# fishmingyu/HyperGef

Measured on AMD Instinct MI355X. Metric: aggregated edges/sec (fused V->E->V aggregation), higher is better.
Workload: dtype f32; 1 GPU; cora-shape x1024 block-diagonal batch, F=32; op=H*H^T*X (aggr_proto), feat_len=32, variant=auto, resolved_variant=fused

## Files before the change

hypergef_amd/_lib.py:

```python
import ctypes
import os

_HERE = os.path.dirname(os.path.abspath(__file__))
LIB_PATH = os.environ.get("HG_AGGR_LIB") or os.path.join(_HERE, "lib", "libhgaggr.so")

HG_OK = 0
HG_ERR_INVALID = -1
HG_ERR_WORKSPACE = -4
HG_ERR_UNSUPPORTED = -5
HG_VARIANT_AUTO = 0
HG_VARIANT_PULL = 1
HG_VARIANT_PUSH_ATOMIC = 2
HG_VARIANT_FUSED = 3
HG_PLAN_HOST_ONLY = 1
HG_PLAN_NO_XCD_REMAP = 2
HG_PLAN_DFS_ORDER = 4
HG_PLAN_NO_HUB_PASS = 8
HG_PLAN_NO_ROW_STREAM = 16

VARIANTS = {"auto": HG_VARIANT_AUTO, "pull": HG_VARIANT_PULL, "push_atomic": HG_VARIANT_PUSH_ATOMIC,
            "fused": HG_VARIANT_FUSED}

SYMBOLS = (
    "hg_version", "hg_last_error", "hg_status_string", "hg_balance_schedule", "hg_mtx_read", "hg_free",
    "hg_plan_create_host", "hg_plan_create_device", "hg_plan_destroy", "hg_plan_get_info",
    "hg_plan_get_vertex_csr", "hg_plan_get_vertex_csr_device", "hg_plan_get_schedule", "hg_plan_prepare", "hg_plan_auto_variant", "hg_plan_bind_scales", "hg_plan_tune_f32",
    "hg_plan_workspace_bytes",
    "hg_aggr_fused_f32", "hg_aggr_fused_bf16", "hg_linear_pack_f32", "hg_linear_pack_ex_f32", "hg_linear_pack_floats", "hg_linear_rows_f32", "hg_linear_wgrad_workspace_bytes", "hg_linear_wgrad_f32", "hg_aggr_linear_workspace_bytes", "hg_aggr_linear_f32", "hg_aggr_linear_res_f32", "hg_aggr_linear_res_dev_f32",
    "hg_gather_rows_f32", "hg_aggr_push_groups_f32", "hg_gather_max_f32",
    "hg_scatter_record_f32",
    "hg_aggr_incidence_workspace_bytes", "hg_aggr_incidence_f32", "hg_incidence_dot_f32", "hg_plan_get_incidence_perm",
)


class HgError(RuntimeError):
    def __init__(self, status, message):
        super().__init__("libhgaggr: %s (status %d)" % (message, status))
        self.status = status


class PlanOpts(ctypes.Structure):
    _fields_ = [("short_max", ctypes.c_int32), ("split_len", ctypes.c_int32),
                ("panel_rows", ctypes.c_int32), ("panel_nnz", ctypes.c_int32),
                ("flags", ctypes.c_int32), ("t_big", ctypes.c_int32),
                ("fused_tile_bytes", ctypes.c_int32), ("fused_steps", ctypes.c_int32)]


class TuneInfo(ctypes.Structure):
    _fields_ = [("variant", ctypes.c_int32), ("pull_hop_kernels", ctypes.c_int32), ("us", ctypes.c_float * 10),
                ("reserved", ctypes.c_int32)]


class FusedInfo(ctypes.Structure):
    _fields_ = [("cap", ctypes.c_int32), ("t_big", ctypes.c_int32), ("vdeg_max", ctypes.c_int32),
                ("panels", ctypes.c_int32), ("n_mat", ctypes.c_int32), ("n_hub", ctypes.c_int32),
                ("slots", ctypes.c_int64), ("member_entries", ctypes.c_int64),
                ("n_split", ctypes.c_int32), ("fixups", ctypes.c_int32),
                ("hub_rounds", ctypes.c_int32), ("hub_workgroups", ctypes.c_int32),
                ("hub_entries", ctypes.c_int64), ("hub_pairs", ctypes.c_int64),
                ("partial_rows", ctypes.c_int64),
                ("record_words_max", ctypes.c_int32), ("stream_steps_max", ctypes.c_int32),
                ("lds_bytes", ctypes.c_int32), ("reserved", ctypes.c_int32)]

    def as_dict(self):
        return {name: getattr(self, name) for name, _ in self._fields_}


class PlanInfo(ctypes.Structure):
    _fields_ = [("N", ctypes.c_int32), ("M", ctypes.c_int32), ("nnz", ctypes.c_int64),
                ("short_max", ctypes.c_int32), ("split_len", ctypes.c_int32),
                ("panel_rows", ctypes.c_int32), ("panel_nnz", ctypes.c_int32),
                ("flags", ctypes.c_int32),
                ("panels", ctypes.c_int32 * 2), ("tasks", ctypes.c_int32 * 2),
                ("partials", ctypes.c_int32 * 2), ("fixups", ctypes.c_int32 * 2),
                ("max_len", ctypes.c_int32 * 2), ("device_bytes", ctypes.c_int64)]

    def as_dict(self):
        out = {}
        for name, _ in self._fields_:
            v = getattr(self, name)
            out[name] = list(v) if hasattr(v, "__len__") else v
        return out


_lib = None


def lib():
    global _lib
    if _lib is not None:
        return _lib
    if not os.path.exists(LIB_PATH):
        raise ImportError(
            "%s not found: build it with `python -c 'import __graft_entry__ as g; g.build()'` "
            "(or `make -C hypergef_amd/csrc`). There is no CPU fallback." % LIB_PATH)
    L = ctypes.CDLL(LIB_PATH)
    vp, i32, i64, sz = ctypes.c_void_p, ctypes.c_int32, ctypes.c_int64, ctypes.c_size_t
    L.hg_version.restype = ctypes.c_int
    L.hg_last_error.restype = ctypes.c_char_p
    L.hg_status_string.restype = ctypes.c_char_p
    L.hg_status_string.argtypes = [ctypes.c_int]
    L.hg_balance_schedule.restype = ctypes.c_int
    L.hg_balance_schedule.argtypes = [i32, i32, vp, ctypes.POINTER(i64), ctypes.POINTER(i64),
                                      vp, vp, vp, vp]
    L.hg_mtx_read.restype = ctypes.c_int
    L.hg_mtx_read.argtypes = [ctypes.c_char_p, ctypes.POINTER(i32), ctypes.POINTER(i32), ctypes.POINTER(i64),
                              ctypes.POINTER(ctypes.POINTER(i32)), ctypes.POINTER(ctypes.POINTER(i32)),
                              ctypes.POINTER(ctypes.POINTER(i32)), ctypes.POINTER(ctypes.POINTER(i32))]
    L.hg_free.restype = None
    L.hg_free.argtypes = [vp]
    L.hg_plan_create_host.restype = ctypes.c_int
    L.hg_plan_create_host.argtypes = [ctypes.POINTER(vp), i32, i32, vp, vp, ctypes.POINTER(PlanOpts)]
    L.hg_plan_create_device.restype = ctypes.c_int
    L.hg_plan_create_device.argtypes = [ctypes.POINTER(vp), i32, i32, i64, vp, vp,
                                        ctypes.POINTER(PlanOpts), vp]
    L.hg_plan_destroy.restype = None
    L.hg_plan_destroy.argtypes = [vp]
    L.hg_plan_get_info.restype = ctypes.c_int
    L.hg_plan_get_info.argtypes = [vp, ctypes.POINTER(PlanInfo)]
    L.hg_plan_get_vertex_csr.restype = ctypes.c_int
    L.hg_plan_get_vertex_csr.argtypes = [vp, vp, vp]
    L.hg_plan_get_vertex_csr_device.restype = ctypes.c_int
    L.hg_plan_get_vertex_csr_device.argtypes = [vp, ctypes.POINTER(vp), ctypes.POINTER(vp)]
    L.hg_plan_get_schedule.restype = ctypes.c_int
    L.hg_plan_get_schedule.argtypes = [vp, i32, vp, vp, vp]
    L.hg_plan_prepare.restype = ctypes.c_int
    L.hg_plan_prepare.argtypes = [vp, i32, ctypes.POINTER(FusedInfo)]
    L.hg_plan_tune_f32.restype = ctypes.c_int
    L.hg_plan_tune_f32.argtypes = [vp, i32, vp, vp, vp, vp, vp, vp, vp, vp, sz, i32, vp, ctypes.POINTER(TuneInfo)]
    L.hg_linear_pack_f32.restype = ctypes.c_int
    L.hg_linear_pack_f32.argtypes = [i32, i32, vp, vp, vp]
    L.hg_linear_pack_ex_f32.restype = ctypes.c_int
    L.hg_linear_pack_ex_f32.argtypes = [i32, i32, vp, vp, i32, vp]
    L.hg_linear_pack_floats.restype = sz
    L.hg_linear_pack_floats.argtypes = [i32, i32, i32]
    L.hg_linear_wgrad_workspace_bytes.restype = sz
    L.hg_linear_wgrad_workspace_bytes.argtypes = [i64, i32, i32]
    L.hg_linear_wgrad_f32.restype = ctypes.c_int
    L.hg_linear_wgrad_f32.argtypes = [i64, i32, i32, vp, vp, vp, vp, sz, vp]
    L.hg_linear_rows_f32.restype = ctypes.c_int
    L.hg_linear_rows_f32.argtypes = [i64, i32, i32, vp, vp, vp, vp]
    L.hg_aggr_linear_workspace_bytes.restype = sz
    L.hg_aggr_linear_workspace_bytes.argtypes = [vp, i32]
    L.hg_aggr_linear_f32.restype = ctypes.c_int
    L.hg_aggr_linear_f32.argtypes = [vp, i32, i32, vp, vp, vp, vp, vp, vp, vp, vp, vp, sz, i32, vp]
    L.hg_aggr_linear_res_f32.restype = ctypes.c_int
    L.hg_aggr_linear_res_f32.argtypes = [vp, i32, i32, vp, vp, vp, vp, vp, vp, vp, vp, ctypes.c_float, ctypes.c_float,
                                         i32, vp, vp, vp, sz, i32, vp]
    L.hg_aggr_linear_res_dev_f32.restype = ctypes.c_int
    L.hg_aggr_linear_res_dev_f32.argtypes = [vp, i32, i32, vp, vp, vp, vp, vp, vp, vp, vp, ctypes.c_float, vp,
                                             i32, vp, vp, vp, sz, i32, vp]
    L.hg_plan_bind_scales.restype = ctypes.c_int
    L.hg_plan_bind_scales.argtypes = [vp, i32, vp, vp, vp, vp]
    L.hg_plan_auto_variant.restype = ctypes.c_int
    L.hg_plan_auto_variant.argtypes = [vp, i32]
    L.hg_plan_workspace_bytes.restype = sz
    L.hg_plan_workspace_bytes.argtypes = [vp, i32]
    L.hg_aggr_fused_f32.restype = ctypes.c_int
    L.hg_aggr_fused_f32.argtypes = [vp, i32, vp, vp, vp, vp, vp, vp, vp, vp, sz, i32, vp]
    L.hg_aggr_fused_bf16.restype = ctypes.c_int
    L.hg_aggr_fused_bf16.argtypes = [vp, i32, vp, vp, vp, vp, vp, vp, vp, vp, sz, i32, vp]
    L.hg_gather_rows_f32.restype = ctypes.c_int
    L.hg_gather_rows_f32.argtypes = [vp, i32, i32, vp, vp, vp, vp, vp, vp, vp, sz, vp]
    L.hg_gather_max_f32.restype = ctypes.c_int
    L.hg_gather_max_f32.argtypes = [i32, i32, vp, vp, vp, vp, vp, vp, vp, vp]
    L.hg_scatter_record_f32.restype = ctypes.c_int
    L.hg_scatter_record_f32.argtypes = [i32, i32, i32, vp, vp, vp, vp, vp]
    if hasattr(L, "hg_aggr_incidence_f32"):
        L.hg_aggr_incidence_workspace_bytes.restype = sz
        L.hg_aggr_incidence_workspace_bytes.argtypes = [vp, i32]
        L.hg_aggr_incidence_f32.restype = ctypes.c_int
        L.hg_aggr_incidence_f32.argtypes = [vp, i32, vp, vp, vp, vp, vp, vp, vp, vp, vp, vp, vp, sz, vp]
        L.hg_incidence_dot_f32.restype = ctypes.c_int
        L.hg_incidence_dot_f32.argtypes = [vp, i32, vp, vp, vp, vp, vp, vp]
        L.hg_plan_get_incidence_perm.restype = ctypes.c_int
        L.hg_plan_get_incidence_perm.argtypes = [vp, vp]
    L.hg_aggr_push_groups_f32.restype = ctypes.c_int
    L.hg_aggr_push_groups_f32.argtypes = [i32, i32, i32, i64, vp, vp, vp, vp, vp, vp,
                                          vp, vp, vp, vp, vp, vp]
    _lib = L
    return L


def check(status):
    if status != HG_OK:
        msg = lib().hg_last_error()
        raise HgError(status, (msg or b"").decode() or lib().hg_status_string(status).decode())
```

hypergef_amd/csrc/hg_api.hip:

```cpp
#include <hip/hip_runtime.h>

#include <cstdio>
#include <cstring>
#include <algorithm>
#include <new>
#include <string>

#include "hg_kernels.h"

namespace {

int hip_fail(const char *what, hipError_t e) {
  hg::set_error(std::string(what) + ": " + hipGetErrorString(e));
  return HG_ERR_HIP;
}

#define HG_HIP(call)                                  \
  do {                                                \
    hipError_t e_ = (call);                           \
    if (e_ != hipSuccess) return hip_fail(#call, e_); \
  } while (0)

size_t round256(size_t x) { return (x + 255) & ~(size_t)255; }

bool aligned16(const void *p) { return (reinterpret_cast<uintptr_t>(p) & 15) == 0; }
bool aligned_lane(const void *p, bool bf16) { return (reinterpret_cast<uintptr_t>(p) & (bf16 ? 7 : 15)) == 0; }
bool rows_whole_64(const void *base, int32_t F, bool bf16 = false) {
  return ((int64_t)F * (bf16 ? 2 : 4)) % 64 == 0 && (reinterpret_cast<uintptr_t>(base) & 63) == 0;
}

int resolve_opts(const hg_plan_opts *in, hg::Opts &o) {
  if (in) {
    if (in->short_max > 0) o.short_max = in->short_max;
    if (in->split_len > 0) o.split_len = in->split_len;
    if (in->panel_rows > 0) {
      o.panel_rows = in->panel_rows;
      o.panel_rows_auto = false;
    }
    if (in->panel_nnz > 0) o.panel_nnz = in->panel_nnz;
    o.flags = in->flags;
    if (in->t_big > 0) o.t_big = in->t_big;
    if (in->fused_tile_bytes > 0) {
      o.fused_tile_bytes = in->fused_tile_bytes;
      o.fused_tile_auto = false;
    }
    if (in->fused_steps > 0) o.fused_steps = in->fused_steps;
  }
  if (o.short_max > o.panel_nnz || o.split_len < o.short_max || o.panel_rows > 4096 ||
      o.panel_nnz > 16384 || o.fused_tile_bytes > 131072) {
    hg::set_error("hg_plan_opts: need short_max <= panel_nnz <= 16384, split_len >= short_max, panel_rows <= 4096, fused_tile_bytes <= 131072");
    return HG_ERR_INVALID;
  }
  if ((size_t)(4 * o.panel_rows + 1 + o.panel_nnz) * sizeof(int32_t) > (size_t)160 * 1024) {
    hg::set_error("hg_plan_opts: panel_rows / panel_nnz need more than 160 KiB of LDS per workgroup");
    return HG_ERR_INVALID;
  }
  return HG_OK;
}

template <typename T>
int upload(const std::vector<T> &h, T **d, int64_t &bytes) {
  *d = nullptr;
  if (h.empty()) return HG_OK;
  const size_t n = h.size() * sizeof(T);
  hipError_t e = hipMalloc(reinterpret_cast<void **>(d), n);
  if (e != hipSuccess) {
    hg::set_error(std::string("hipMalloc(plan): ") + hipGetErrorString(e));
    return e == hipErrorOutOfMemory ? HG_ERR_NOMEM : HG_ERR_HIP;
  }
  HG_HIP(hipMemcpy(*d, h.data(), n, hipMemcpyHostToDevice));
  bytes += (int64_t)n;
  return HG_OK;
}

int sched_upload(hg::Sched &s, int64_t &bytes) {
  int rc;
  if ((rc = upload(s.panels, &s.d_panels, bytes)) != HG_OK) return rc;
  if ((rc = upload(s.tasks, &s.d_tasks, bytes)) != HG_OK) return rc;
  return upload(s.fixups, &s.d_fixups, bytes);
}

void sched_free(hg::Sched &s) {
  if (s.d_panels) (void)hipFree(s.d_panels);
  if (s.d_tasks) (void)hipFree(s.d_tasks);
  if (s.d_fixups) (void)hipFree(s.d_fixups);
  s.d_panels = nullptr;
  s.d_tasks = nullptr;
  s.d_fixups = nullptr;
}

int plan_upload(hg_plan *p) {
  HG_HIP(hipGetDevice(&p->device));
  int rc;
  if ((rc = upload(p->ptr_v, &p->d_ptr_v, p->device_bytes)) != HG_OK) return rc;
  if ((rc = upload(p->ind_v, &p->d_ind_v, p->device_bytes)) != HG_OK) return rc;
  for (int h = 0; h < 2; h++)
    if ((rc = sched_upload(p->sched[h], p->device_bytes)) != HG_OK) return rc;
  if (p->has_lat)
    for (int h = 0; h < 2; h++)
      if ((rc = sched_upload(p->sched_lat[h], p->device_bytes)) != HG_OK) return rc;
  return HG_OK;
}

int fused_upload(hg::FusedSched &f, int64_t &bytes) {
  int rc;
#define UP(v, d) if ((rc = upload(f.v, &f.d, bytes)) != HG_OK) return rc
  UP(prow, d_prow);
  UP(mat_ptr, d_mat_ptr);
  UP(mat_ind, d_mat_ind);
  UP(mat_eid, d_mat_eid);
  UP(rec, d_rec);
  UP(rec_tab, d_rec_tab);
  UP(eid_all, d_eid_all);
  UP(fixups, d_fixups);
  UP(hub.vslot0, hub.d_vslot0);
  UP(hub.rec, hub.d_rec);
  UP(hub.rec_tab, hub.d_rec_tab);
  UP(hub.wg_first, hub.d_wg_first);
  UP(mat_stream.rec, mat_stream.d_rec);
  UP(mat_stream.rec_tab, mat_stream.d_rec_tab);
  UP(mat_stream.fixups, mat_stream.d_fixups);
#undef UP
  return sched_upload(f.mat_sched, bytes);
}

void fused_free(hg::FusedSched &f) {
  void *ptrs[] = {f.d_prow, f.d_mat_ptr, f.d_mat_ind, f.d_mat_eid, f.d_rec, f.d_rec_tab, f.d_eid_all, f.d_bsA,
                  f.d_bsB, f.d_bsD, f.d_fixups, f.hub.d_vslot0, f.hub.d_rec, f.hub.d_rec_tab, f.hub.d_wg_first, f.mat_stream.d_rec, f.mat_stream.d_rec_tab,
                  f.mat_stream.d_fixups};
  for (void *q : ptrs)
    if (q) (void)hipFree(q);
  sched_free(f.mat_sched);
}

bool wide_rows_ok(const hg_plan *p, int32_t F) {
  return (F % 4 == 0 || F > 8) && p->N < (1 << 24) && p->M < (1 << 24) && F < (1 << 22) && (int64_t)p->N * F * 4 < ((int64_t)1 << 31) &&
         (int64_t)p->M * F * 4 < ((int64_t)1 << 31);
}
bool plan_vec4(const hg_plan *p, int32_t F) { return F % 4 == 0 || wide_rows_ok(p, F); }

void fused_caps(const hg_plan *p, int32_t F, bool vec4, int32_t &cap, int32_t &mem_cap, int32_t tile_bytes = 0) {
  const int row_bytes = hg::fused_tile_row_floats(F, vec4) * 4;
  const int c = std::max(16, std::min(256, (tile_bytes > 0 ? tile_bytes : p->opts.fused_tile_bytes) / row_bytes));
  cap = c / 16 * 16;
  mem_cap = cap * 4;
  if (p->opts.fused_steps > 0) {
    const int32_t ng = 256 / (hg::fused_tile_row_floats(F, vec4) / (vec4 ? 4 : 1));
    mem_cap = std::max(p->opts.t_big, std::min(mem_cap, p->opts.fused_steps * ng));
  }
}

double small_graph_cost(const hg::FusedSched &f) {
  int32_t max_rows = 0;
  for (const hg::FPanel &pn : f.panels) max_rows = std::max(max_rows, pn.nrows);
  const int launches = 1 + (f.n_mat > 0 ? 1 : 0) + (f.fixups.empty() ? 0 : 1);
  return 5.0 * launches + 0.08 * f.max_steps + 0.4 * ((max_rows + f.ng - 1) / std::max(1, f.ng));
}

bool lin_caps(const hg_plan *p, int32_t F, bool vec4, int32_t &cap, int32_t &mem_cap, int32_t &rows_cap) {
  if (!vec4 || F != 128 || !p->opts.fused_tile_auto || p->opts.fused_steps > 0 || p->nnz <= (1 << 18)) return false;
  const int pct = 150;
  fused_caps(p, F, vec4, cap, mem_cap);
  const int32_t ng = 256 / (hg::fused_tile_row_floats(F, vec4) / 4);
  rows_cap = std::min(cap, 4 * ng);
  cap = std::max(cap, (rows_cap * pct / 100 + 7) / 8 * 8);
  mem_cap = cap * 4;
  return true;
}

int get_fused(const hg_plan *cp, int32_t F, bool vec4, const hg::FusedSched **out, bool lin = false) {
  hg_plan *p = const_cast<hg_plan *>(cp);
  int32_t cap, mem_cap, rows_cap = 0;
  if (lin && !lin_caps(p, F, vec4, cap, mem_cap, rows_cap)) lin = false;
  if (!lin) fused_caps(p, F, vec4, cap, mem_cap);
  const int32_t row_floats = hg::fused_tile_row_floats(F, vec4);
  const int32_t ng = 256 / (row_floats / (vec4 ? 4 : 1));
  const bool allow_hub = vec4 && F % 4 == 0 && F >= 16 && p->N < (1 << 24) && p->M < (1 << 24) && (int64_t)p->N * F * 4 < ((int64_t)1 << 31) &&
                         (int64_t)p->M * F * 4 < ((int64_t)1 << 31);
  const int64_t key = ((((int64_t)cap * 1000000 + mem_cap) * 1000 + ng) * 2 + (allow_hub ? 1 : 0)) * 1024 + rows_cap;
  std::lock_guard<std::mutex> lock(p->fused_mu);
  auto it = p->fused.find(key);
  if (it == p->fused.end()) {
    hg::FusedSched f;
    try {
      hg::build_fused(p->N, p->M, p->ptr_t.data(), p->ind_t.data(), p->ptr_v.data(), p->ind_v.data(),
                      p->opts, cap, mem_cap, ng, row_floats, allow_hub, f, rows_cap);
      if (p->nnz <= (1 << 18)) {
        double best = small_graph_cost(f);
        const int32_t tiles[3] = {p->opts.fused_tile_bytes, p->opts.fused_tile_bytes / 2, p->opts.fused_tile_bytes / 4};
        for (int t = 0; t < (p->opts.fused_tile_auto ? 3 : 1); t++) {
          int32_t c2, m2;
          fused_caps(p, F, vec4, c2, m2, tiles[t]);
          if (t > 0 && c2 == cap) continue;
          for (int mode = 0; mode < 4; mode++) {
            if (t == 0 && mode == 0) continue;
            hg::Opts o = p->opts;
            if (mode == 1) {
              if (p->sched[0].max_len * 4 > m2 || p->sched[0].max_len <= o.t_big) continue;
              o.t_big = p->sched[0].max_len;
            } else if (mode >= 2) {
              o.slot_chunk = std::max(o.t_big, mode == 2 ? 8 : 16);
              if (p->sched[0].max_len <= o.slot_chunk || (mode == 3 && o.t_big >= 16)) continue;
            }
            hg::FusedSched alt;
            hg::build_fused(p->N, p->M, p->ptr_t.data(), p->ind_t.data(), p->ptr_v.data(), p->ind_v.data(), o, c2, m2,
                            ng, row_floats, allow_hub, alt);
            if (alt.invalid) continue;
            const double c = small_graph_cost(alt);
            if (c < best) {
              best = c;
              f = std::move(alt);
            }
          }
        }
        const int32_t lanes = row_floats / (vec4 ? 4 : 1);
        if (p->opts.fused_tile_auto && vec4 && F % 4 == 0 && (lanes == 8 || lanes == 16) && p->nnz <= 16384 && p->N <= 4096 &&
            wide_rows_ok(p, F)) {
          for (int32_t tile : {16384, 32768, 65536}) {
            int32_t c2, m2;
            fused_caps(p, F, vec4, c2, m2, tile);
            for (int mode = 1; mode < 4; mode++) {
              hg::Opts o = p->opts;
              if (mode == 1) {
                if (p->sched[0].max_len * 4 > m2) continue;
                o.t_big = std::max(o.t_big, p->sched[0].max_len);
              } else {
                o.slot_chunk = std::max(o.t_big, mode == 2 ? 8 : 16);
                if (p->sched[0].max_len <= o.slot_chunk) continue;
              }
              hg::FusedSched alt;
              hg::build_fused(p->N, p->M, p->ptr_t.data(), p->ind_t.data(), p->ptr_v.data(), p->ind_v.data(), o, c2, m2,
                              4 * ng, row_floats, false, alt);
              if (alt.invalid || alt.n_mat > 0 || !alt.fixups.empty()) continue;
              const double c = small_graph_cost(alt) + 0.3;
              if (c < best) {
                best = c;
                f = std::move(alt);
              }
            }
          }
        }
      }
    } catch (const std::bad_alloc &) {
      hg::set_error("fused schedule: host allocation failed");
      return HG_ERR_NOMEM;
    }
    for (const hg::FPanel &pn : f.panels) {
      if (pn.nrows <= 0 || pn.nrows > f.rows_cap || pn.nslots > f.cap || pn.npm > f.mem_cap ||
          pn.nvs > f.vslot_cap || pn.r0 < 0 || (size_t)(pn.r0 + pn.nrows) > f.prow.size()) {
        hg::set_error("fused schedule: internal error, panel exceeds its LDS budget");
        return HG_ERR_INVALID;
      }
    }
    const size_t lds_need = std::max((size_t)f.cap * (row_floats + 4) * 4 + (size_t)f.max_rec_words * 4 +
                                         (size_t)(2 * f.cap + f.rows_cap) * 4 + 16,
                                     f.hub.K > 0 ? hg::hub_pass_lds_bytes(f.hub.cap, row_floats, f.hub.max_rec_words) : 0);
    if (lds_need > (size_t)160 * 1024) {
      hg::set_error("fused schedule: fused_tile_bytes = " + std::to_string(p->opts.fused_tile_bytes) + " needs " +
                    std::to_string(lds_need) + " bytes of LDS per workgroup at this feature width (limit 163840)");
      return HG_ERR_INVALID;
    }
    int rc = (p->opts.flags & HG_PLAN_HOST_ONLY) ? HG_OK : fused_upload(f, p->device_bytes);
    if (rc != HG_OK) {
      fused_free(f);
      return rc;
    }
    it = p->fused.emplace(key, std::move(f)).first;
  }
  p->fused_by_width[((int64_t)F * 2 + (vec4 ? 1 : 0)) * 2 + (lin ? 1 : 0)] = &it->second;
  *out = &it->second;
  return HG_OK;
}

struct Carve {
  size_t xe, part[2], total;
};
Carve carve(const hg_plan *p, int32_t F) {
  Carve c;
  c.xe = 0;
  size_t off = round256((size_t)p->M * F * sizeof(float));
  for (int h = 0; h < 2; h++) {
    c.part[h] = off;
    off += round256((size_t)std::max(std::max(p->sched[h].nslots, p->sched_lat[h].nslots), p->stream_nslots[h]) * F * sizeof(float) + 16);
  }
  c.total = off;
  return c;
}
struct FusedCarve {
  size_t mat_part, part, total;
};
FusedCarve fused_carve(const hg::FusedSched &f, int32_t F) {
  FusedCarve c;
  c.mat_part = round256((size_t)f.n_mat * F * sizeof(float));
  c.part = c.mat_part + round256((size_t)std::max(f.mat_sched.nslots, f.mat_stream.nslots) * F * sizeof(float));
  c.total = c.part + round256((size_t)f.n_part * F * sizeof(float) + 16);
  return c;
}
size_t workspace_need(const hg_plan *cp, int32_t F, bool pull_only = false) {
  hg_plan *p = const_cast<hg_plan *>(cp);
  size_t need = carve(p, F).total;
  if (pull_only) return need;
  std::lock_guard<std::mutex> lock(p->fused_mu);
  for (const auto &kv : p->fused_by_width)
    if (kv.first / 4 == F) need = std::max(need, fused_carve(*kv.second, F).total);
  return need;
}

int pick_variant_uncached(const hg_plan *plan, int32_t F, bool vec4, int32_t *variant,
                          const hg::FusedSched **f);
int get_row_stream(const hg_plan *cp, int hop, int32_t ng, const hg::RowStream **out);

int pick_variant(const hg_plan *plan, int32_t F, bool vec4, int32_t *variant,
                 const hg::FusedSched **f) {
  hg_plan *mp = const_cast<hg_plan *>(plan);
  const int64_t key = (int64_t)F * 2 + (vec4 ? 1 : 0);
  {
    std::lock_guard<std::mutex> lock(mp->auto_mu);
    auto it = mp->auto_choice.find(key);
    if (it != mp->auto_choice.end()) {
      *variant = it->second;
      return *variant == HG_VARIANT_FUSED ? get_fused(plan, F, vec4, f) : HG_OK;
    }
  }
  int rc = pick_variant_uncached(plan, F, vec4, variant, f);
  if (rc == HG_OK) {
    std::lock_guard<std::mutex> lock(mp->auto_mu);
    mp->auto_choice[key] = *variant;
  }
  return rc;
}

int pick_variant_uncached(const hg_plan *plan, int32_t F, bool vec4, int32_t *variant,
                          const hg::FusedSched **f) {
  *variant = HG_VARIANT_PULL;
  const bool small = plan->nnz <= (1 << 18);
  if (!small && plan->small_nnz_frac < 0.2) return HG_OK;
  int32_t cap, mem_cap;
  fused_caps(plan, F, vec4, cap, mem_cap);
  if (small) {
    int64_t n_mat = 0, n_big = 0;
    hg::classify_fused(plan->N, plan->M, plan->ptr_t.data(), plan->ptr_v.data(), plan->ind_v.data(), plan->opts,
                       cap, mem_cap, &n_mat, &n_big);
    if (n_big > 0) return HG_OK;
  }
  int rc = get_fused(plan, F, vec4, f);
  if (rc != HG_OK) return rc;
  const hg::FusedSched &fs = **f;
  const int64_t mat_nnz = fs.mat_ptr.empty() ? 0 : fs.mat_ptr.back();
  if (small && (fs.n_mat > 0 || !fs.fixups.empty())) return HG_OK;
  const bool work_ok = small || fs.pmem_entries + fs.hub.stream_entries + mat_nnz <= 5 * plan->nnz;
  const bool pieces_ok = small || (int64_t)fs.n_split * 16 <= plan->N;
  if (work_ok && pieces_ok) *variant = HG_VARIANT_FUSED;
  return HG_OK;
}

int run_sched(const hg_plan *p, const hg::Sched &s, int32_t F, const int32_t *ptr,
              const int32_t *ind, const void *src, const float *scaleA, const float *scaleB,
              const int32_t *scale_map, const int32_t *dst_map, void *dst, float *partial,
              hipStream_t stream, bool nt_dst = false, bool src_bf16 = false, bool dst_bf16 = false,
              const float *w = nullptr, const int32_t *wperm = nullptr) {
  hg::WeightedGatherArgs a;
  a.nt_dst = nt_dst ? 1 : 0;
  a.w = w;
  a.wperm = wperm;
  a.scale_map = scale_map;
  a.dst_map = dst_map;
  a.ptr = ptr;
  a.ind = ind;
  a.src = src;
  a.dst = dst;
  a.scaleA = scaleA;
  a.scaleB = scaleB;
  a.partial = partial;
  a.panels = s.d_panels;
  a.tasks = s.d_tasks;
  a.npanels = (int32_t)s.panels.size();
  a.ntasks = (int32_t)s.tasks.size();
  a.n_task_blocks = (a.ntasks + 3) / 4;
  a.F = F;
  a.panel_rows = p->opts.panel_rows;
  a.panel_nnz = p->opts.panel_nnz;
  a.xcd_remap = (p->opts.flags & HG_PLAN_NO_XCD_REMAP) ? 0 : 1;
  const bool vec4 = (F % 4 == 0) && aligned_lane(src, src_bf16) && aligned_lane(dst, dst_bf16) && aligned16(partial);
  if (w && (src_bf16 || dst_bf16)) {
    hg::set_error("weighted row gather: fp32 rows only");
    return HG_ERR_UNSUPPORTED;
  }
  hipError_t e = w ? hg::launch_gather_weighted(a, (int)s.fixups.size(), s.n_fix_l1, s.d_fixups, vec4, stream)
                   : hg::launch_gather(a, (int)s.fixups.size(), s.n_fix_l1, s.d_fixups, vec4, stream, src_bf16, dst_bf16);
  if (e != hipSuccess) return hip_fail("gather_rows launch", e);
  return HG_OK;
}

int get_row_stream(const hg_plan *cp, int hop, int32_t ng, const hg::RowStream **out) {
  hg_plan *p = const_cast<hg_plan *>(cp);
  std::lock_guard<std::mutex> lock(p->stream_mu);
  const int64_t key = (int64_t)hop * 1024 + ng;
  auto it = p->row_streams.find(key);
  if (it == p->row_streams.end()) {
    hg::RowStream rs;
    try {
      if (hop == 0) hg::build_row_stream(p->M, p->ptr_t.data(), p->ind_t.data(), nullptr, ng, p->N, rs);
      else hg::build_row_stream(p->N, p->ptr_v.data(), p->ind_v.data(), nullptr, ng, p->M, rs);
    } catch (const std::bad_alloc &) {
      hg::set_error("row stream schedule: host allocation failed");
      return HG_ERR_NOMEM;
    }
    if (rs.nslots > p->stream_nslots[hop]) {
      hg::set_error("row stream schedule: internal error, more partial rows than the workspace layout reserves");
      return HG_ERR_INVALID;
    }
    int rc;
    if ((rc = upload(rs.rec, &rs.d_rec, p->device_bytes)) != HG_OK) return rc;
    if ((rc = upload(rs.rec_tab, &rs.d_rec_tab, p->device_bytes)) != HG_OK) return rc;
    if ((rc = upload(rs.fixups, &rs.d_fixups, p->device_bytes)) != HG_OK) return rc;
    it = p->row_streams.emplace(key, std::move(rs)).first;
  }
  *out = &it->second;
  return HG_OK;
}

int get_incidence_perm(const hg_plan *cp, bool upload_it, const int32_t **d_perm) {
  hg_plan *p = const_cast<hg_plan *>(cp);
  std::lock_guard<std::mutex> lock(p->perm_mu);
  if (!p->perm_built) {
    try {
      p->perm.assign((size_t)p->nnz, 0);
      std::vector<int32_t> cursor(p->ptr_v.begin(), p->ptr_v.end() - 1);
      for (int32_t e = 0; e < p->M; e++)
        for (int32_t q = p->ptr_t[e]; q < p->ptr_t[e + 1]; q++) p->perm[cursor[p->ind_t[q]]++] = q;
    } catch (const std::bad_alloc &) {
      hg::set_error("incidence permutation: host allocation failed");
      return HG_ERR_NOMEM;
    }
    p->perm_built = true;
  }
  if (upload_it && !p->d_perm && p->nnz > 0) {
    int rc = upload(p->perm, &p->d_perm, p->device_bytes);
    if (rc != HG_OK) {
      if (p->d_perm) (void)hipFree(p->d_perm);
      p->d_perm = nullptr;
      return rc;
    }
  }
  if (d_perm) *d_perm = p->d_perm;
  return HG_OK;
}

int run_hop(const hg_plan *p, int hop, int32_t F, const int32_t *ptr, const int32_t *ind,
            const void *src, const float *scaleA, const float *scaleB, void *dst,
            float *partial, hipStream_t stream, bool src_bf16 = false, bool dst_bf16 = false) {
  const bool lanes16 = F % 4 == 0 || F > 8;
  const int64_t nsrc = hop == 0 ? p->N : p->M, sb = nsrc * F * (src_bf16 ? 2 : 4);
  const bool nt_out = rows_whole_64(dst, F, dst_bf16) && (hop == 1 || (int64_t)p->M * F * 4 >= ((int64_t)192 << 20));
  int kind = 0;
  {
    hg_plan *mp = const_cast<hg_plan *>(p);
    std::lock_guard<std::mutex> lock(mp->auto_mu);
    auto it = mp->hop_kernel.find(F);
    if (it != mp->hop_kernel.end()) kind = hop == 0 ? it->second % 3 : (it->second / 3) % 3;
  }
  if (kind == 0 && lanes16 && F < (1 << 22) && nsrc < (1 << 24) && sb > 0 && sb < ((int64_t)1 << 31) && !(p->opts.flags & HG_PLAN_NO_ROW_STREAM)) {
    const int32_t ng = 256 / (hg::fused_tile_row_floats(F, true) / 4);
    const hg::RowStream *rs = nullptr;
    int rc = get_row_stream(p, hop, ng, &rs);
    if (rc != HG_OK) return rc;
    hg::StreamArgs sa;
    sa.rec = rs->d_rec;
    sa.rec_tab = rs->d_rec_tab;
    sa.nrec = (int32_t)rs->rec_tab.size();
    sa.ng = rs->ng;
    sa.cap = rs->cap;
    sa.max_rec_words = rs->max_rec_words;
    sa.src = src;
    sa.src_bytes = (int32_t)sb;
    sa.nrows_src = (int32_t)nsrc;
    sa.scaleA = scaleA;
    sa.scaleB = scaleB;
    sa.dst = dst;
    sa.partial = partial;
    sa.F = F;
    sa.xcd_remap = (p->opts.flags & HG_PLAN_NO_XCD_REMAP) ? 0 : 1;
    sa.nt_dst = nt_out;
    if (sa.nrec == 0) return HG_OK;
    if (hg::stream_rows_ok(sa, true)) {
      hipError_t e = hg::launch_stream_rows(sa, stream, src_bf16, dst_bf16);
      if (e == hipSuccess)
        e = hg::launch_fixups(rs->d_fixups, (int)rs->fixups.size(), rs->n_fix_l1, F, partial, dst, scaleA, scaleB,
                              nullptr, true, stream, nt_out, dst_bf16);
      if (e != hipSuccess) return hip_fail("stream_rows launch", e);
      return HG_OK;
    }
  }
  return run_sched(p, (kind == 2 && p->has_lat) ? p->sched_lat[hop] : p->sched[hop], F, ptr, ind, src, scaleA, scaleB,
                   nullptr, nullptr, dst, partial, stream, nt_out, src_bf16, dst_bf16);
}

enum { kSizeAny = 0, kSizePull = 1, kSizeLater = 2 };
int check_call(const hg_plan *plan, int32_t F, const void *workspace, size_t workspace_bytes, int size_mode = kSizeAny) {
  if (!plan) {
    hg::set_error("null plan");
    return HG_ERR_INVALID;
  }
  if (plan->opts.flags & HG_PLAN_HOST_ONLY) {
    hg::set_error("plan was built with HG_PLAN_HOST_ONLY and holds no device schedule");
    return HG_ERR_INVALID;
  }
  if (F <= 0) {
    hg::set_error("feature width must be positive");
    return HG_ERR_INVALID;
  }
  if ((int64_t)std::max(plan->N, plan->M) * F >= ((int64_t)1 << 40)) {
    hg::set_error("feature matrix too large");
    return HG_ERR_INVALID;
  }
  const size_t need = size_mode == kSizeLater ? 0 : workspace_need(plan, F, size_mode == kSizePull);
  if (need > 0 && (!workspace || workspace_bytes < need)) {
    hg::set_error("workspace too small: need " + std::to_string(need) + " bytes, got " +
                  std::to_string(workspace_bytes));
    return HG_ERR_WORKSPACE;
  }
  if (workspace && (reinterpret_cast<uintptr_t>(workspace) & 255)) {
    hg::set_error("workspace must be 256-byte aligned");
    return HG_ERR_INVALID;
  }
  return HG_OK;
}

int plan_build(hg_plan **out, int32_t N, int32_t M, const int32_t *csrptr_t,
               const int32_t *colind_t, const hg_plan_opts *opts) {
  if (!out) {
    hg::set_error("hg_plan_create: null output pointer");
    return HG_ERR_INVALID;
  }
  *out = nullptr;
  hg::Opts o;
  int rc = resolve_opts(opts, o);
  if (rc != HG_OK) return rc;
  if ((rc = hg::validate_csr(M, N, csrptr_t, colind_t)) != HG_OK) return rc;
  hg_plan *p = new (std::nothrow) hg_plan();
  if (!p) {
    hg::set_error("hg_plan_create: host allocation failed");
    return HG_ERR_NOMEM;
  }
  try {
    p->N = N;
    p->M = M;
    p->nnz = csrptr_t[M];
    p->opts = o;
    p->ptr_t.assign(csrptr_t, csrptr_t + M + 1);
    p->ind_t.assign(colind_t, colind_t + p->nnz);
    hg::transpose_csr(M, N, csrptr_t, colind_t, p->ptr_v, p->ind_v);
    hg::build_sched(M, csrptr_t, o, p->sched[0]);
    hg::build_sched(N, p->ptr_v.data(), o, p->sched[1]);
    if (p->nnz <= (1 << 18) && o.short_max > hg::kLatShortMax) {
      hg::Opts ol = o;
      ol.short_max = hg::kLatShortMax;
      hg::build_sched(M, csrptr_t, ol, p->sched_lat[0]);
      hg::build_sched(N, p->ptr_v.data(), ol, p->sched_lat[1]);
      p->has_lat = true;
    }
    int64_t small = 0;
    for (int32_t e = 0; e < M; e++) {
      const int32_t len = csrptr_t[e + 1] - csrptr_t[e];
      if (len <= o.t_big) small += len;
    }
    p->small_nnz_frac = p->nnz > 0 ? (double)small / (double)p->nnz : 0.0;
    for (int h = 0; h < 2; h++) {
      const std::vector<int32_t> &ptr = h ? p->ptr_v : p->ptr_t;
      int64_t ns = 0;
      for (size_t r = 0; r + 1 < ptr.size(); r++) {
        const int64_t len = ptr[r + 1] - ptr[r];
        if (len > hg::kRowStreamChunk) {
          const int64_t k = (len + hg::kRowStreamChunk - 1) / hg::kRowStreamChunk;
          ns += k;
          if (k > 32) {
            int64_t fan = 1;
            while (fan * fan < k) fan++;
            ns += (k + fan - 1) / fan;
          }
        }
      }
      p->stream_nslots[h] = (int32_t)std::min<int64_t>(ns, 0x7fffffff);
    }
  } catch (const std::bad_alloc &) {
    delete p;
    hg::set_error("hg_plan_create: host allocation failed");
    return HG_ERR_NOMEM;
  }
  if (!(o.flags & HG_PLAN_HOST_ONLY)) {
    rc = plan_upload(p);
    if (rc != HG_OK) {
      hg_plan_destroy(p);
      return rc;
    }
  }
  *out = p;
  return HG_OK;
}

}

extern "C" {

int hg_plan_create_host(hg_plan **out, int32_t N, int32_t M, const int32_t *csrptr_t_host,
                        const int32_t *colind_t_host, const hg_plan_opts *opts) {
  return plan_build(out, N, M, csrptr_t_host, colind_t_host, opts);
}

int hg_plan_create_device(hg_plan **out, int32_t N, int32_t M, int64_t nnz,
                          const int32_t *csrptr_t_dev, const int32_t *colind_t_dev,
                          const hg_plan_opts *opts, hg_stream_t stream) {
  if (!out || N < 0 || M < 0 || nnz < 0 || !csrptr_t_dev || (nnz > 0 && !colind_t_dev)) {
    hg::set_error("hg_plan_create_device: bad argument");
    return HG_ERR_INVALID;
  }
  hipStream_t s = static_cast<hipStream_t>(stream);
  std::vector<int32_t> ptr, ind;
  try {
    ptr.resize((size_t)M + 1);
    ind.resize((size_t)nnz);
  } catch (const std::bad_alloc &) {
    hg::set_error("hg_plan_create_device: host allocation failed");
    return HG_ERR_NOMEM;
  }
  HG_HIP(hipMemcpyAsync(ptr.data(), csrptr_t_dev, ptr.size() * sizeof(int32_t),
                        hipMemcpyDeviceToHost, s));
  if (nnz > 0)
    HG_HIP(hipMemcpyAsync(ind.data(), colind_t_dev, ind.size() * sizeof(int32_t),
                          hipMemcpyDeviceToHost, s));
  HG_HIP(hipStreamSynchronize(s));
  if (ptr[M] != nnz) {
    hg::set_error("hg_plan_create_device: csrptr_t[M] != nnz");
    return HG_ERR_INVALID;
  }
  return plan_build(out, N, M, ptr.data(), ind.data(), opts);
}

void hg_plan_destroy(hg_plan *p) {
  if (!p) return;
  if (p->d_ptr_v) (void)hipFree(p->d_ptr_v);
  if (p->d_ind_v) (void)hipFree(p->d_ind_v);
  for (int h = 0; h < 2; h++) sched_free(p->sched[h]);
  for (int h = 0; h < 2; h++) sched_free(p->sched_lat[h]);
  for (auto &kv : p->fused) fused_free(kv.second);
  for (auto &kv : p->row_streams) {
    void *ptrs[] = {kv.second.d_rec, kv.second.d_rec_tab, kv.second.d_fixups};
    for (void *q : ptrs)
      if (q) (void)hipFree(q);
  }
  if (p->d_perm) (void)hipFree(p->d_perm);
  delete p;
}

int hg_plan_get_info(const hg_plan *p, hg_plan_info *info) {
  if (!p || !info) {
    hg::set_error("hg_plan_get_info: null argument");
    return HG_ERR_INVALID;
  }
  std::memset(info, 0, sizeof(*info));
  info->N = p->N;
  info->M = p->M;
  info->nnz = p->nnz;
  info->short_max = p->opts.short_max;
  info->split_len = p->opts.split_len;
  info->panel_rows = p->opts.panel_rows;
  info->panel_nnz = p->opts.panel_nnz;
  info->flags = p->opts.flags;
  for (int h = 0; h < 2; h++) {
    info->panels[h] = (int32_t)p->sched[h].panels.size();
    info->tasks[h] = (int32_t)p->sched[h].tasks.size();
    info->partials[h] = p->sched[h].nslots;
    info->fixups[h] = (int32_t)p->sched[h].fixups.size();
    info->max_len[h] = p->sched[h].max_len;
  }
  info->device_bytes = p->device_bytes;
  return HG_OK;
}

int hg_plan_get_vertex_csr(const hg_plan *p, int32_t *ptr_v_host, int32_t *ind_v_host) {
  if (!p || !ptr_v_host || (p->nnz > 0 && !ind_v_host)) {
    hg::set_error("hg_plan_get_vertex_csr: null argument");
    return HG_ERR_INVALID;
  }
  std::memcpy(ptr_v_host, p->ptr_v.data(), p->ptr_v.size() * sizeof(int32_t));
  if (p->nnz > 0) std::memcpy(ind_v_host, p->ind_v.data(), p->ind_v.size() * sizeof(int32_t));
  return HG_OK;
}

int hg_plan_get_vertex_csr_device(const hg_plan *p, const int32_t **ptr_v_dev,
                                  const int32_t **ind_v_dev) {
  if (!p || !ptr_v_dev || !ind_v_dev || (p->opts.flags & HG_PLAN_HOST_ONLY)) {
    hg::set_error("hg_plan_get_vertex_csr_device: null argument or host-only plan");
    return HG_ERR_INVALID;
  }
  *ptr_v_dev = p->d_ptr_v;
  *ind_v_dev = p->d_ind_v;
  return HG_OK;
}

int hg_plan_get_schedule(const hg_plan *p, int32_t hop, int32_t *panels, int32_t *tasks,
                         int32_t *fixups) {
  if (!p || (hop != 0 && hop != 1)) {
    hg::set_error("hg_plan_get_schedule: bad argument");
    return HG_ERR_INVALID;
  }
  const hg::Sched &s = p->sched[hop];
  static_assert(sizeof(hg::Panel) == 16 && sizeof(hg::Task) == 16 && sizeof(hg::Fixup) == 16, "quad layout");
  if (panels && !s.panels.empty()) std::memcpy(panels, s.panels.data(), s.panels.size() * sizeof(hg::Panel));
  if (tasks && !s.tasks.empty()) std::memcpy(tasks, s.tasks.data(), s.tasks.size() * sizeof(hg::Task));
  if (fixups && !s.fixups.empty()) std::memcpy(fixups, s.fixups.data(), s.fixups.size() * sizeof(hg::Fixup));
  return HG_OK;
}

static int gather_bound_scales(hg::FusedSched *f, const float *degE, const float *degV, const float *W, hipStream_t stream) {
  const size_t ns = f->eid_all.size(), nr = f->prow.size();
  if (!f->d_bsA && ns > 0) {
    HG_HIP(hipMalloc(reinterpret_cast<void **>(&f->d_bsA), ns * sizeof(float)));
    HG_HIP(hipMalloc(reinterpret_cast<void **>(&f->d_bsB), ns * sizeof(float)));
  }
  if (!f->d_bsD && nr > 0) HG_HIP(hipMalloc(reinterpret_cast<void **>(&f->d_bsD), nr * sizeof(float)));
  hipError_t e = hg::launch_bind_scales((int64_t)ns, f->d_eid_all, degE, W, f->d_bsA, f->d_bsB, (int64_t)nr,
                                        f->d_prow, degV, f->d_bsD, stream);
  if (e != hipSuccess) return hip_fail("bind_scales launch", e);
  return HG_OK;
}

int hg_plan_bind_scales(const hg_plan *cp, int32_t F, const float *degE, const float *degV,
                        const float *W, hg_stream_t stream) {
  if (!cp || F <= 0 || (cp->opts.flags & HG_PLAN_HOST_ONLY)) {
    hg::set_error("hg_plan_bind_scales: bad argument or host-only plan");
    return HG_ERR_INVALID;
  }
  const hg::FusedSched *cf = nullptr;
  int rc = get_fused(cp, F, plan_vec4(cp, F), &cf);
  if (rc != HG_OK) return rc;
  hg::FusedSched *f = const_cast<hg::FusedSched *>(cf);
  std::lock_guard<std::mutex> lock(const_cast<hg_plan *>(cp)->fused_mu);
  for (const auto &kv : cp->fused_by_width)
    if (kv.first / 4 == F && (kv.first & 1) && kv.second != cf) {
      hg::FusedSched *fl = const_cast<hg::FusedSched *>(kv.second);
      fl->bound_degE = fl->bound_W = fl->bound_degV = nullptr;
      fl->bound_W_is_one = false;
    }
  if (!degE && !degV && !W) {
    f->bound_degE = f->bound_W = f->bound_degV = nullptr;
    f->bound_W_is_one = false;
    return HG_OK;
  }
  if ((rc = gather_bound_scales(f, degE, degV, W, static_cast<hipStream_t>(stream))) != HG_OK) return rc;
  bool w_one = false;
  if (W && cp->M > 0) {
    int32_t *d_flag = nullptr, h_flag = 1;
    HG_HIP(hipMalloc(reinterpret_cast<void **>(&d_flag), sizeof(int32_t)));
    hipStream_t st = static_cast<hipStream_t>(stream);
    hipError_t e2 = hipMemcpyAsync(d_flag, &h_flag, sizeof(int32_t), hipMemcpyHostToDevice, st);
    if (e2 == hipSuccess) e2 = hg::launch_all_ones(cp->M, W, d_flag, st);
    if (e2 == hipSuccess) e2 = hipMemcpyAsync(&h_flag, d_flag, sizeof(int32_t), hipMemcpyDeviceToHost, st);
    if (e2 == hipSuccess) e2 = hipStreamSynchronize(st);
    (void)hipFree(d_flag);
    if (e2 != hipSuccess) return hip_fail("bind_scales: all-ones check", e2);
    w_one = h_flag != 0;
  }
  f->bound_degE = degE;
  f->bound_W = W;
  f->bound_degV = degV;
  f->bound_W_is_one = w_one;
  return HG_OK;
}

int hg_plan_auto_variant(const hg_plan *p, int32_t F) {
  if (!p || F <= 0) {
    hg::set_error("hg_plan_auto_variant: bad argument");
    return HG_ERR_INVALID;
  }
  int32_t variant = HG_VARIANT_PULL;
  const hg::FusedSched *f = nullptr;
  int rc = pick_variant(p, F, plan_vec4(p, F), &variant, &f);
  return rc != HG_OK ? rc : variant;
}

int hg_plan_prepare(const hg_plan *p, int32_t F, hg_fused_info *info) {
  if (!p || F <= 0) {
    hg::set_error("hg_plan_prepare: bad argument");
    return HG_ERR_INVALID;
  }
  const hg::FusedSched *f = nullptr;
  int rc = get_fused(p, F, plan_vec4(p, F), &f);
  if (rc != HG_OK) return rc;
  if (!(p->opts.flags & (HG_PLAN_HOST_ONLY | HG_PLAN_NO_ROW_STREAM)) && (F % 4 == 0 || F > 8)) {
    const int32_t ng = 256 / (hg::fused_tile_row_floats(F, true) / 4);
    for (int hop = 0; hop < 2; hop++) {
      const int64_t nsrc = hop == 0 ? p->N : p->M;
      if (nsrc >= (1 << 24) || nsrc * F * 4 >= ((int64_t)1 << 31)) continue;
      const hg::RowStream *rs = nullptr;
      if ((rc = get_row_stream(p, hop, ng, &rs)) != HG_OK) return rc;
    }
  }
  if (info) {
    info->cap = f->cap;
    info->t_big = f->t_big;
    info->vdeg_max = f->vdeg_max;
    info->panels = (int32_t)f->panels.size();
    info->n_mat = f->n_mat;
    info->n_hub = f->hub.K;
    info->member_entries = f->pmem_entries;
    int64_t slots = 0;
    for (const auto &pn : f->panels) slots += pn.nslots;
    info->slots = slots;
    info->n_split = f->n_split;
    info->fixups = (int32_t)f->fixups.size();
    info->hub_rounds = (int32_t)f->hub.rec_tab.size();
    info->hub_workgroups = f->hub.K > 0 ? f->hub.nwg : 0;
    info->hub_entries = f->hub.stream_entries;
    info->hub_pairs = f->hub.pairs;
    info->partial_rows = f->n_part;
    info->record_words_max = f->max_rec_words;
    info->stream_steps_max = f->max_steps;
    info->lds_bytes = (int32_t)((size_t)f->cap * hg::fused_tile_row_floats(F, plan_vec4(p, F)) * 4 + (size_t)f->max_rec_words * 4 + 16);
    info->reserved = 0;
  }
  return HG_OK;
}

__attribute__((visibility("default"))) int hg_debug_fused_shape(const hg_plan *p, int32_t F, int32_t lin, int64_t *out9) {
  const hg::FusedSched *f = nullptr;
  int rc = get_fused(p, F, plan_vec4(p, F), &f, lin != 0);
  if (rc != HG_OK) return rc;
  int64_t rows = 0, padded = 0, slots = 0;
  for (const auto &pn : f->panels) {
    rows += pn.nrows;
    padded += (pn.nrows + 15) / 16 * 16;
    slots += pn.nslots;
  }
  const int64_t v[9] = {(int64_t)f->panels.size(), rows, padded, f->pmem_entries, slots, f->cap, f->rows_cap, f->n_mat,
                        f->stream_entries / std::max(1, f->ng) * 100000 + f->max_rec_words};
  for (int i = 0; i < 9; i++) out9[i] = v[i];
  return HG_OK;
}

size_t hg_plan_workspace_bytes(const hg_plan *p, int32_t F) {
  if (!p || F <= 0) return 0;
  int32_t variant = HG_VARIANT_PULL;
  const hg::FusedSched *f = nullptr;
  (void)pick_variant(p, F, plan_vec4(p, F), &variant, &f);
  return workspace_need(p, F);
}

int hg_gather_rows_f32(const hg_plan *plan, int32_t hop, int32_t F, const int32_t *csrptr_t,
                       const int32_t *colind_t, const float *src, const float *scaleA,
                       const float *scaleB, float *dst, void *workspace, size_t workspace_bytes,
                       hg_stream_t stream) {
  int rc = check_call(plan, F, workspace, workspace_bytes, kSizePull);
  if (rc != HG_OK) return rc;
  if ((hop != 0 && hop != 1) || !src || !dst || (hop == 0 && (!csrptr_t || (plan->nnz > 0 && !colind_t)))) {
    hg::set_error("hg_gather_rows_f32: bad argument");
    return HG_ERR_INVALID;
  }
  const Carve c = carve(plan, F);
  float *partial = reinterpret_cast<float *>(static_cast<char *>(workspace) + c.part[hop]);
  const int32_t *ptr = hop == 0 ? csrptr_t : plan->d_ptr_v;
  const int32_t *ind = hop == 0 ? colind_t : plan->d_ind_v;
  return run_hop(plan, hop, F, ptr, ind, src, scaleA, scaleB, dst, partial,
                 static_cast<hipStream_t>(stream));
}

int hg_aggr_push_groups_f32(int32_t N, int32_t M, int32_t F, int64_t n_group,
                            const int32_t *group_key, const int32_t *group_row,
                            const int32_t *group_st, const int32_t *group_ed,
                            const int32_t *csrptr_t, const int32_t *colind_t, const float *X,
                            const float *degE, const float *degV, const float *W, float *Y,
                            hg_stream_t stream) {
  if (N < 0 || M < 0 || F <= 0 || n_group < 0 || !X || !Y || !colind_t) {
    hg::set_error("hg_aggr_push_groups_f32: bad argument");
    return HG_ERR_INVALID;
  }
  if (group_key ? (!group_row || !group_st || !group_ed) : (!csrptr_t || n_group != M)) {
    hg::set_error("hg_aggr_push_groups_f32: need all four group arrays, or csrptr_t with n_group == M");
    return HG_ERR_INVALID;
  }
  hipStream_t s = static_cast<hipStream_t>(stream);
  HG_HIP(hipMemsetAsync(Y, 0, (size_t)N * F * sizeof(float), s));
  hg::PushArgs a;
  a.n_group = n_group;
  a.group_key = group_key;
  a.group_row = group_row;
  a.group_st = group_st;
  a.group_ed = group_ed;
  a.csrptr_t = csrptr_t;
  a.colind_t = colind_t;
  a.X = X;
  a.degE = degE;
  a.degV = degV;
  a.W = W;
  a.Y = Y;
  a.F = F;
  hipError_t e = hg::launch_push(a, s);
  if (e != hipSuccess) return hip_fail("push_groups launch", e);
  return HG_OK;
}

int hg_gather_max_f32(int32_t M, int32_t F, const int32_t *csrptr_t, const int32_t *colind_t,
                      const float *X, const float *degE, const float *W, float *Xe, int32_t *record,
                      hg_stream_t stream) {
  if (M < 0 || F <= 0 || !csrptr_t || !X || !Xe || !record || (int64_t)M * F >= ((int64_t)1 << 39)) {
    hg::set_error("hg_gather_max_f32: bad argument");
    return HG_ERR_INVALID;
  }
  hipError_t e = hg::launch_gather_max(M, F, csrptr_t, colind_t, X, degE, W, Xe, record,
                                       static_cast<hipStream_t>(stream));
  if (e != hipSuccess) return hip_fail("gather_max launch", e);
  return HG_OK;
}

int hg_scatter_record_f32(int32_t N, int32_t M, int32_t F, const float *T, const int32_t *record,
                          const float *degV, float *Y, hg_stream_t stream) {
  if (N < 0 || M < 0 || F <= 0 || !T || !record || !Y) {
    hg::set_error("hg_scatter_record_f32: bad argument");
    return HG_ERR_INVALID;
  }
  hipStream_t s = static_cast<hipStream_t>(stream);
  HG_HIP(hipMemsetAsync(Y, 0, (size_t)N * F * sizeof(float), s));
  hipError_t e = hg::launch_scatter_record(M, F, T, record, degV, Y, s);
  if (e != hipSuccess) return hip_fail("scatter_record launch", e);
  return HG_OK;
}

struct LinReq {
  const float *Wlin;
  int32_t F_out;
  float *Y;
  bool done;
  hg::LinEpilogue epi;
};

static int aggr_impl(const hg_plan *plan, int32_t F, const int32_t *csrptr_t,
                     const int32_t *colind_t, const void *X, const float *degE,
                     const float *degV, const float *W, void *Y, void *workspace,
                     size_t workspace_bytes, int32_t variant, hg_stream_t stream, LinReq *lin, bool bf16 = false) {
  const char *fn = bf16 ? "hg_aggr_fused_bf16" : "hg_aggr_fused_f32";
  if (variant == HG_VARIANT_PUSH_ATOMIC) {
    if (!plan) {
      hg::set_error("null plan");
      return HG_ERR_INVALID;
    }
    if (bf16) {
      hg::set_error("hg_aggr_fused_bf16: the push kernels are fp32 only");
      return HG_ERR_UNSUPPORTED;
    }
    return hg_aggr_push_groups_f32(plan->N, plan->M, F, plan->M, nullptr, nullptr, nullptr, nullptr,
                                   csrptr_t, colind_t, static_cast<const float *>(X), degE, degV, W,
                                   static_cast<float *>(Y), stream);
  }
  if (variant != HG_VARIANT_AUTO && variant != HG_VARIANT_PULL && variant != HG_VARIANT_FUSED) {
    hg::set_error(std::string(fn) + ": unknown variant");
    return HG_ERR_UNSUPPORTED;
  }
  int rc = check_call(plan, F, workspace, workspace_bytes, kSizeLater);
  if (rc != HG_OK) return rc;
  if (!csrptr_t || (plan->nnz > 0 && !colind_t) || !X || !Y) {
    hg::set_error(std::string(fn) + ": null array");
    return HG_ERR_INVALID;
  }
  if (bf16 && (lin || F % 4 != 0 || !aligned_lane(X, true) || !aligned_lane(Y, true))) {
    hg::set_error("hg_aggr_fused_bf16: F must be a multiple of 4 and X, Y 8-byte aligned");
    return HG_ERR_UNSUPPORTED;
  }
  hipStream_t s = static_cast<hipStream_t>(stream);
  const Carve c = carve(plan, F);
  char *ws = static_cast<char *>(workspace);
  float *Xe = reinterpret_cast<float *>(ws + c.xe);
  const bool aligned = (F % 4 == 0) && aligned_lane(X, bf16) && aligned_lane(Y, bf16) && aligned16(Xe);
  const bool vec4 = aligned || wide_rows_ok(plan, F);
  const hg::FusedSched *f = nullptr;
  if (variant == HG_VARIANT_AUTO) {
    if ((rc = pick_variant(plan, F, vec4, &variant, &f)) != HG_OK) return rc;
  }
  if (variant == HG_VARIANT_FUSED) {
    if (!f && (rc = get_fused(plan, F, vec4, &f)) != HG_OK) return rc;
    if (lin && aligned && f->fixups.empty()) {
      const hg::FusedSched *fl = nullptr;
      if ((rc = get_fused(plan, F, vec4, &fl, true)) != HG_OK) return rc;
      if (fl != f && fl->fixups.empty()) {
        const bool dflt_bound = (degE || degV || W) && f->bound_degE == degE && f->bound_W == W && f->bound_degV == degV;
        if (dflt_bound && !(fl->bound_degE == degE && fl->bound_W == W && fl->bound_degV == degV)) {
          hg::FusedSched *m = const_cast<hg::FusedSched *>(fl);
          std::lock_guard<std::mutex> lock(const_cast<hg_plan *>(plan)->fused_mu);
          if ((rc = gather_bound_scales(m, degE, degV, W, s)) != HG_OK) return rc;
          (void)hipStreamSynchronize(s);
          m->bound_degE = degE;
          m->bound_W = W;
          m->bound_degV = degV;
          m->bound_W_is_one = f->bound_W_is_one;
        }
        f = fl;
      }
    }
    const FusedCarve fc = fused_carve(*f, F);
    if (fc.total > 0 && (!workspace || fc.total > workspace_bytes)) {
      hg::set_error("workspace too small for the fused schedule: need " + std::to_string(fc.total) + " bytes, got " +
                    std::to_string(workspace_bytes) +
                    " (hg_plan_workspace_bytes covers it once hg_plan_prepare has built the schedule)");
      return HG_ERR_WORKSPACE;
    }
    float *partial = reinterpret_cast<float *>(ws + fc.part);
    const bool bound = (degE || degV || W) && f->bound_degE == degE && f->bound_W == W && f->bound_degV == degV;
    if (bound && W && f->bound_W_is_one) W = nullptr;
    const int64_t xb = (int64_t)plan->N * F * (bf16 ? 2 : 4), mb = (int64_t)f->n_mat * F * 4;
    const int32_t x_bytes = xb < ((int64_t)1 << 31) ? (int32_t)xb : 0;
    const int32_t mat_bytes = mb < ((int64_t)1 << 31) ? (int32_t)mb : 0;
    if (f->n_mat > 0) {
      hg::StreamArgs sa;
      sa.rec = f->mat_stream.d_rec;
      sa.rec_tab = f->mat_stream.d_rec_tab;
      sa.nrec = (int32_t)f->mat_stream.rec_tab.size();
      sa.ng = f->mat_stream.ng;
      sa.cap = f->mat_stream.cap;
      sa.max_rec_words = f->mat_stream.max_rec_words;
      sa.src = X;
      sa.src_bytes = x_bytes;
      sa.nrows_src = plan->N;
      sa.scaleA = degE;
      sa.scaleB = W;
      sa.dst = Xe;
      sa.partial = reinterpret_cast<float *>(ws + fc.mat_part);
      sa.F = F;
      sa.xcd_remap = (plan->opts.flags & HG_PLAN_NO_XCD_REMAP) ? 0 : 1;
      if (hg::stream_rows_ok(sa, vec4)) {
        hipError_t e = hg::launch_stream_rows(sa, s, bf16, false);
        if (e == hipSuccess)
          e = hg::launch_fixups(f->mat_stream.d_fixups, (int)f->mat_stream.fixups.size(), f->mat_stream.n_fix_l1, F,
                                sa.partial, Xe, degE, W, f->d_mat_eid, vec4, s);
        if (e != hipSuccess) return hip_fail("stream_rows launch", e);
      } else {
        rc = run_sched(plan, f->mat_sched, F, f->d_mat_ptr, f->d_mat_ind, X, degE, W, f->d_mat_eid,
                       nullptr, Xe, reinterpret_cast<float *>(ws + fc.mat_part), s, false, bf16);
        if (rc != HG_OK) return rc;
      }
    }
    if (f->hub.K > 0) {
      hg::HubArgs h;
      h.rec = f->hub.d_rec;
      h.rec_tab = f->hub.d_rec_tab;
      h.wg_first = f->hub.d_wg_first;
      h.vslot0 = f->hub.d_vslot0;
      h.nwg = f->hub.nwg;
      h.ng = f->hub.ng;
      h.cap = f->hub.cap;
      h.max_rec_words = f->hub.max_rec_words;
      h.X = X;
      h.Xe_mat = f->n_mat > 0 ? Xe : nullptr;
      h.degE = degE;
      h.W = W;
      h.partial = partial;
      h.F = F;
      h.x_bytes = x_bytes;
      h.mat_bytes = mat_bytes;
      h.nrows_x = plan->N;
      h.nrows_mat = f->n_mat;
      h.n_heavy = f->hub.n_heavy;
      for (int q = 0; q < hg::kHubHeavy; q++) h.hslot0[q] = f->hub.hslot0[q];
      hipError_t e = hg::launch_hub_pass(h, vec4, s, bf16);
      if (e != hipSuccess) return hip_fail("hub_pass launch", e);
    }
    hg::FusedArgs a;
    a.npanels = (int32_t)f->panels.size();
    a.X = X;
    a.Xe_mat = f->n_mat > 0 ? Xe : nullptr;
    a.degE = degE;
    a.W = W;
    a.degV = degV;
    a.Y = Y;
    a.partial = partial;
    a.F = F;
    a.cap = f->cap;
    a.rows_cap = f->rows_cap;
    a.xcd_remap = (plan->opts.flags & HG_PLAN_NO_XCD_REMAP) ? 0 : 1;
    a.rec = f->d_rec;
    a.rec_tab = f->d_rec_tab;
    a.eid_all = f->d_eid_all;
    a.max_rec_words = f->max_rec_words;
    a.ng = f->ng;
    a.x_bytes = x_bytes;
    a.mat_bytes = mat_bytes;
    a.nrows_x = plan->N;
    a.nrows_mat = f->n_mat;
    a.y_nt = rows_whole_64(Y, F, bf16);
    a.reverse_runs = f->n_mat > 0 && !f->mat_ptr.empty() && (int64_t)f->mat_ptr.back() * 4 >= plan->nnz;
    a.bsA = bound ? f->d_bsA : nullptr;
    a.bsB = bound ? f->d_bsB : nullptr;
    a.bsD = bound ? f->d_bsD : nullptr;
    if (lin && f->fixups.empty() && aligned) {
      a.Wlin = lin->Wlin;
      a.F_out = lin->F_out;
      a.epi = lin->epi;
      if (hg::fused_linear_ok(a)) {
        a.Y = lin->Y;
        lin->done = true;
      } else {
        a.Wlin = nullptr;
      }
    }
    hipError_t e = hg::launch_fused(a, vec4, s, bf16);
    if (e != hipSuccess) return hip_fail("fused_panel launch", e);
    if (!f->fixups.empty()) {
      e = hg::launch_fixups(f->d_fixups, (int)f->fixups.size(), f->n_fix_l1, F, partial, Y, degV, nullptr, nullptr, vec4, s,
                            rows_whole_64(Y, F, bf16), bf16);
      if (e != hipSuccess) return hip_fail("fixup launch", e);
    }
    return HG_OK;
  }
  if (c.total > 0 && (!workspace || workspace_bytes < c.total)) {
    hg::set_error("workspace too small: need " + std::to_string(c.total) + " bytes, got " + std::to_string(workspace_bytes));
    return HG_ERR_WORKSPACE;
  }
  rc = run_hop(plan, 0, F, csrptr_t, colind_t, X, degE, W, Xe,
               reinterpret_cast<float *>(ws + c.part[0]), s, bf16, false);
  if (rc != HG_OK) return rc;
  return run_hop(plan, 1, F, plan->d_ptr_v, plan->d_ind_v, Xe, degV, nullptr, Y,
                 reinterpret_cast<float *>(ws + c.part[1]), s, false, bf16);
}

int hg_aggr_fused_f32(const hg_plan *plan, int32_t F, const int32_t *csrptr_t,
                      const int32_t *colind_t, const float *X, const float *degE,
                      const float *degV, const float *W, float *Y, void *workspace,
                      size_t workspace_bytes, int32_t variant, hg_stream_t stream) {
  return aggr_impl(plan, F, csrptr_t, colind_t, X, degE, degV, W, Y, workspace, workspace_bytes, variant,
                   stream, nullptr);
}

int hg_aggr_fused_bf16(const hg_plan *plan, int32_t F, const int32_t *csrptr_t,
                       const int32_t *colind_t, const uint16_t *X, const float *degE,
                       const float *degV, const float *W, uint16_t *Y, void *workspace,
                       size_t workspace_bytes, int32_t variant, hg_stream_t stream) {
  if (variant == HG_VARIANT_PUSH_ATOMIC) {
    hg::set_error("hg_aggr_fused_bf16: HG_VARIANT_PUSH_ATOMIC is fp32 only");
    return HG_ERR_UNSUPPORTED;
  }
  return aggr_impl(plan, F, csrptr_t, colind_t, X, degE, degV, W, Y, workspace, workspace_bytes, variant,
                   stream, nullptr, true);
}

int hg_plan_tune_f32(const hg_plan *plan, int32_t F, const int32_t *csrptr_t, const int32_t *colind_t,
                     const float *X, const float *degE, const float *degV, const float *W, float *Y,
                     void *workspace, size_t workspace_bytes, int32_t iters, hg_stream_t stream,
                     hg_tune_info *info) {
  int rc = check_call(plan, F, workspace, workspace_bytes);
// ... 321 lines not shown
```

hypergef_amd/csrc/hg_fused.cpp:

```cpp
#include <algorithm>
#include <numeric>

#include "hg_internal.h"

namespace hg {

void pack_records(FusedSched &f, int32_t ng, int32_t idle);
static void build_hub_pass(int32_t N, int32_t M, const int32_t *ptr_t, const int32_t *ind_t, const int32_t *ptr_v,
                           const std::vector<uint8_t> &is_mat, const std::vector<int32_t> &mat_id,
                           const std::vector<int32_t> &hub_of, const std::vector<int32_t> &parts,
                           int32_t t_big, FusedSched &f, std::vector<Fixup> &finals);

void classify_fused(int32_t N, int32_t M, const int32_t *ptr_t, const int32_t *ptr_v, const int32_t *ind_v,
                    const Opts &o, int32_t cap, int32_t mem_cap, int64_t *n_mat, int64_t *n_big) {
  (void)ind_v;
  const int32_t t_big = std::max(1, std::min(o.t_big, mem_cap));
  const int32_t vdeg_max = std::max(1, std::min(std::min(cap, cap * 2), mem_cap / t_big));
  *n_mat = 0;
  for (int32_t e = 0; e < M; e++)
    if (ptr_t[e + 1] - ptr_t[e] > t_big) (*n_mat)++;
  *n_big = 0;
  for (int32_t v = 0; v < N; v++)
    if (ptr_v[v + 1] - ptr_v[v] > vdeg_max) (*n_big)++;
}

static void hub_geometry(int32_t ng_panel, int32_t row_floats, int32_t tile_bytes, HubPass &h) {
  h.bs = 1024;
  h.ng = ng_panel * 4;
  h.R = kHubRows;
  h.cap = std::max(16, std::min(1024, tile_bytes / (row_floats * 4))) / 16 * 16;
  h.cap = std::max(h.cap, (h.ng + 15) / 16 * 16);
  h.mem_cap = std::min(h.cap * 4, 16 * h.ng);
  h.pair_cap = std::max(h.ng * h.R, std::min(h.cap * 8, 8192));
}

constexpr int32_t kHubRecWords = 6144;
static int32_t hub_rec_bound(const HubPass &h, int32_t entries, int32_t longest, int32_t nslots, int32_t npairs) {
  return 16 + h.ng + ((entries + h.ng - 1) / h.ng + longest + 1) * h.ng + nslots + (h.ng * h.R + 1) / 2 + (npairs + 1) / 2 + 4;
}

struct SlotRange {
  int32_t m0, m1;
  uint32_t hmask;
};
struct PackedStream {
  int32_t steps = 0, steps_x = 0;
  std::vector<int32_t> stream, newid, gslots;
};
static void pack_stream(const std::vector<SlotRange> &slots, const int32_t *mem, int32_t ng, int32_t idle_x,
                        int32_t idle_m, uint32_t row_mask, PackedStream &out) {
  const int32_t ns = (int32_t)slots.size();
  std::vector<int32_t> order_x, mats;
  for (int32_t k = 0; k < ns; k++) {
    const bool mat = slots[k].m1 - slots[k].m0 == 1 && ((uint32_t)mem[slots[k].m0] & 0x80000000u);
    (mat ? mats : order_x).push_back(k);
  }
  std::stable_sort(order_x.begin(), order_x.end(), [&](int32_t a, int32_t b) {
    return (slots[a].m1 - slots[a].m0) > (slots[b].m1 - slots[b].m0);
  });
  std::vector<int32_t> load((size_t)ng, 0);
  std::vector<std::vector<int32_t>> members((size_t)ng), mmembers((size_t)ng);
  for (int32_t k : order_x) {
    int32_t best = 0;
    for (int32_t g = 1; g < ng; g++)
      if (load[g] < load[best]) best = g;
    members[best].push_back(k);
    load[best] += slots[k].m1 - slots[k].m0;
  }
  out.steps_x = 0;
  for (int32_t g = 0; g < ng; g++) out.steps_x = std::max(out.steps_x, load[g]);
  for (size_t i = 0; i < mats.size(); i++) mmembers[i % (size_t)ng].push_back(mats[i]);
  const int32_t mat_steps = ((int32_t)mats.size() + ng - 1) / ng;
  out.steps = out.steps_x + mat_steps;
  out.stream.assign((size_t)out.steps * ng, idle_x);
  for (size_t i = (size_t)out.steps_x * ng; i < out.stream.size(); i++) out.stream[i] = idle_m;
  out.newid.assign((size_t)ns, 0);
  out.gslots.assign((size_t)ng, 0);
  int32_t next = 0;
  auto emit = [&](int32_t g, int32_t k, int32_t &s) {
    out.newid[k] = next++;
    for (int32_t p = slots[k].m0; p < slots[k].m1; p++, s++) {
      const uint32_t w = (uint32_t)mem[p];
      const uint32_t mat = (w & 0x80000000u) ? 0x40000000u : 0u;
      const uint32_t last = (p + 1 == slots[k].m1) ? (0x80000000u | (slots[k].hmask << 24)) : 0u;
      out.stream[(size_t)s * ng + g] = (int32_t)((w & row_mask) | mat | last);
    }
  };
  for (int32_t g = 0; g < ng; g++) {
    out.gslots[g] = next;
    int32_t s = 0;
    for (int32_t k : members[g]) emit(g, k, s);
    s = out.steps_x;
    for (int32_t k : mmembers[g]) emit(g, k, s);
  }
}

void build_fused(int32_t N, int32_t M, const int32_t *ptr_t, const int32_t *ind_t,
                 const int32_t *ptr_v, const int32_t *ind_v, const Opts &o, int32_t cap,
                 int32_t mem_cap, int32_t ng, int32_t row_floats, bool allow_hub, FusedSched &f,
                 int32_t rows_cap) {
  f = FusedSched();
  f.cap = cap;
  f.rows_cap = rows_cap > 0 ? std::min(rows_cap, cap) : cap;
  f.mem_cap = mem_cap;
  f.vslot_cap = cap * 2;
  f.t_big = std::max(1, std::min(o.t_big, f.mem_cap));
  f.vdeg_max = std::max(1, std::min(std::min(cap, f.vslot_cap), f.mem_cap / f.t_big));
  const int64_t nnz = ptr_t[M];

  const int32_t chunk = o.slot_chunk > 0 ? std::max(o.slot_chunk, f.t_big) : 0;
  auto nsub = [&](int32_t e) { return chunk > 0 ? std::max(1, (ptr_t[e + 1] - ptr_t[e] + chunk - 1) / chunk) : 1; };
  std::vector<uint8_t> is_mat((size_t)M, 0);
  std::vector<int32_t> mat_id((size_t)M, -1);
  f.mat_ptr.push_back(0);
  for (int32_t e = 0; e < M; e++)
    if (chunk == 0 && ptr_t[e + 1] - ptr_t[e] > f.t_big) {
      is_mat[e] = 1;
      mat_id[e] = f.n_mat++;
      f.mat_eid.push_back(e);
      f.mat_ind.insert(f.mat_ind.end(), ind_t + ptr_t[e], ind_t + ptr_t[e + 1]);
      f.mat_ptr.push_back((int32_t)f.mat_ind.size());
    }
  build_sched(f.n_mat, f.mat_ptr.data(), o, f.mat_sched);
  if (allow_hub) build_row_stream(f.n_mat, f.mat_ptr.data(), f.mat_ind.data(), f.mat_eid.data(), ng, N, f.mat_stream);

  std::vector<uint8_t> big((size_t)N, 0);
  std::vector<int32_t> cand;
  for (int32_t v = 0; v < N; v++) {
    int64_t w = ptr_v[v + 1] - ptr_v[v];
    if (chunk > 0) {
      w = 0;
      for (int32_t p = ptr_v[v]; p < ptr_v[v + 1]; p++) w += nsub(ind_v[p]);
      if (w > std::min(f.vdeg_max, f.mem_cap / chunk)) {
        f.invalid = true;
        return;
      }
    }
    if (w > f.vdeg_max) {
      big[v] = 2;
      cand.push_back(v);
    }
  }
  std::vector<int32_t> hub_of((size_t)N, -1), parts;
  HubPass &hp = f.hub;
  hub_geometry(ng, row_floats, o.hub_tile_bytes, hp);
  const int32_t kHubMinDeg = o.hub_min_deg;
  allow_hub = allow_hub && hub_rec_bound(hp, f.t_big, f.t_big, 1, hp.ng * hp.R) <= kHubRecWords;
  if (allow_hub && !(o.flags & HG_PLAN_NO_HUB_PASS) && nnz >= o.hub_min_nnz && !cand.empty()) {
    auto deg = [&](int32_t v) { return ptr_v[v + 1] - ptr_v[v]; };
    std::stable_sort(cand.begin(), cand.end(), [&](int32_t a, int32_t b) { return deg(a) > deg(b); });
    const int32_t vmax = hp.ng * hp.R;
    int64_t top = 0;
    for (size_t i = 0; i < cand.size() && (int32_t)i < vmax && deg(cand[i]) >= kHubMinDeg; i++) top += deg(cand[i]);
    if (top * 5 >= nnz) {
      auto listed_twice = [&](int32_t v) {
        for (int32_t p = ptr_v[v] + 1; p < ptr_v[v + 1]; p++)
          if (ind_v[p] == ind_v[p - 1]) return true;
        return false;
      };
      int64_t heavy_sum = 0;
      for (size_t i = 0; i < cand.size() && hp.n_heavy < kHubHeavy && deg(cand[i]) >= kHubMinDeg &&
                         (int64_t)deg(cand[i]) * 512 >= nnz; i++) {
        if (listed_twice(cand[i])) continue;
        heavy_sum += deg(cand[i]);
        std::rotate(cand.begin() + hp.n_heavy, cand.begin() + i, cand.begin() + i + 1);
        hp.n_heavy++;
      }
      const int64_t wmax = std::max<int64_t>(1, (top - heavy_sum) / (2 * (int64_t)hp.ng));
      int32_t nv = 0;
      for (size_t i = 0; i < cand.size() && deg(cand[i]) >= kHubMinDeg; i++) {
        const bool heavy = (int32_t)i < hp.n_heavy;
        const int32_t p = heavy ? 0 : (int32_t)std::min<int64_t>(64, (deg(cand[i]) + wmax - 1) / wmax);
        if (nv + p > vmax) break;
        nv += p;
        hub_of[cand[i]] = hp.K++;
        hp.vid.push_back(cand[i]);
        parts.push_back(p);
        big[cand[i]] = 1;
      }
      hp.nv = nv;
    }
  }

  std::vector<int32_t> order;
  order.reserve((size_t)N);
  {
    std::vector<uint8_t> vis((size_t)N, 0), seen((size_t)M, 0);
    struct Frame {
      int32_t v, ep, up;
    };
    std::vector<Frame> st;
    for (int32_t root = 0; root < N; root++) {
      if (vis[root] || big[root]) continue;
      vis[root] = 1;
      st.push_back(Frame{root, ptr_v[root], -1});
      while (!st.empty()) {
        Frame &fr = st.back();
        bool descended = false;
        while (!descended && fr.ep < ptr_v[fr.v + 1]) {
          const int32_t e = ind_v[fr.ep];
          if (fr.up < 0) {
            if (seen[e] || is_mat[e]) {
              fr.ep++;
              continue;
            }
            seen[e] = 1;
            fr.up = ptr_t[e];
          }
          while (fr.up < ptr_t[e + 1]) {
            const int32_t u = ind_t[fr.up++];
            if (!vis[u] && !big[u]) {
              vis[u] = 1;
              st.push_back(Frame{u, ptr_v[u], -1});
              descended = true;
              break;
            }
          }
          if (!descended) {
            fr.ep++;
            fr.up = -1;
          }
        }
        if (!descended) {
          order.push_back(st.back().v);
          st.pop_back();
        }
      }
    }
  }

  std::vector<int32_t> stamp((size_t)M, -1), slot_of((size_t)M, 0);
  FPanel cur{};
  auto open_panel = [&]() {
    cur = FPanel{};
    cur.r0 = (int32_t)f.prow.size();
    cur.sbase = (int32_t)f.soff.size();
    cur.pm0 = (int32_t)f.pmem.size();
    cur.eid0 = (int32_t)f.slot_eid.size();
    cur.v0 = (int32_t)f.pvs.size();
    f.soff.push_back(0);
  };
  auto close_panel = [&]() {
    cur.nrows = (int32_t)f.prow.size() - cur.r0;
    if (cur.nrows > 0) {
      cur.npm = (int32_t)f.pmem.size() - cur.pm0;
      cur.nvs = (int32_t)f.pvs.size() - cur.v0;
      f.panels.push_back(cur);
    } else {
      f.soff.pop_back();
    }
  };
  struct Cand {
    float frac;
    int32_t shared, v;
    bool operator<(const Cand &o) const {
      return frac != o.frac ? frac < o.frac : (shared != o.shared ? shared < o.shared : v > o.v);
    }
  };
  const bool greedy = !(o.flags & HG_PLAN_DFS_ORDER);
  std::vector<Cand> heap;
  std::vector<int32_t> score(greedy ? (size_t)N : 0, 0), touched;
  std::vector<uint8_t> done(greedy ? (size_t)N : 0, 0);
  size_t next_in_order = 0;
  auto reset_candidates = [&]() {
    for (const int32_t u : touched) score[u] = 0;
    touched.clear();
    heap.clear();
  };
  auto next_vertex = [&]() -> int32_t {
    if (greedy) {
      while (!heap.empty()) {
        std::pop_heap(heap.begin(), heap.end());
        const Cand c = heap.back();
        heap.pop_back();
        if (!done[c.v] && score[c.v] == c.shared) return c.v;
      }
      while (next_in_order < order.size() && done[order[next_in_order]]) next_in_order++;
    }
    return next_in_order < order.size() ? order[next_in_order++] : -1;
  };
  auto add_row = [&](int32_t v, int32_t p0, int32_t p1, int32_t dest, bool feed_greedy) {
    int32_t pid = (int32_t)f.panels.size();
    int32_t new_slots = 0, new_mem = 0, deg = 0;
    for (int32_t p = p0; p < p1; p++) {
      const int32_t e = ind_v[p];
      deg += nsub(e);
      if (stamp[e] != pid) {
        new_slots += nsub(e);
        new_mem += is_mat[e] ? 1 : (ptr_t[e + 1] - ptr_t[e]);
      }
    }
    const int32_t rows = (int32_t)f.prow.size() - cur.r0;
    const int32_t cur_mem = (int32_t)f.pmem.size() - cur.pm0;
    const int32_t cur_vs = (int32_t)f.pvs.size() - cur.v0;
    if (rows > 0 && (rows == f.rows_cap || cur.nslots + new_slots > f.cap ||
                     cur_mem + new_mem > f.mem_cap || cur_vs + deg > f.vslot_cap)) {
      close_panel();
      open_panel();
// ... 367 lines not shown
```

hypergef_amd/csrc/hg_internal.h:

```cpp
#pragma once
#include <cstdint>
#include <map>
#include <mutex>
#include <string>
#include <vector>

#include "hg_aggr.h"

namespace hg {

struct Panel {
  int32_t row0, nrows, nnz0, nnz_cnt;
};

struct Task {
  int32_t row, beg, end, slot;
};

struct Fixup {
  int32_t row, first, count, pad;
};

struct Sched {
  int32_t nrows = 0;
  int32_t max_len = 0;
  std::vector<Panel> panels;
  std::vector<Task> tasks;
  std::vector<Fixup> fixups;
  int32_t n_fix_l1 = 0;
  int32_t nslots = 0;
  Panel *d_panels = nullptr;
  Task *d_tasks = nullptr;
  Fixup *d_fixups = nullptr;
};

struct FPanel {
  int32_t r0, nrows, sbase, nslots, pm0, npm, eid0, v0, nvs, pad0, pad1, pad2;
};

struct FRec {
  int64_t off;
  int32_t len;
  int32_t off_prow, pad;
  int32_t nrows, nslots;
  int32_t slot_base, row_base;
};

constexpr int kHubRows = 12;
constexpr int kHubChunk = 4;
constexpr int kHubHeavy = 4;

struct HubRec {
  int64_t off;
  int32_t len;
  int32_t nslots, off_eid;
  int32_t pad;
};

struct HubPass {
  int32_t K = 0;
  int32_t n_heavy = 0;
  int32_t hslot0[kHubHeavy] = {};
  int32_t nv = 0;
  int32_t bs = 1024, ng = 0, R = kHubRows;
  int32_t cap = 0, mem_cap = 0, pair_cap = 0;
  int32_t nwg = 0;
  int32_t max_rec_words = 0, max_steps = 0;
  int64_t stream_entries = 0;
  int64_t pairs = 0;
  std::vector<int32_t> vid;
  std::vector<int32_t> vslot0;
  std::vector<int32_t> rec;
  std::vector<HubRec> rec_tab;
  std::vector<int32_t> wg_first;
  int32_t *d_vslot0 = nullptr, *d_rec = nullptr, *d_wg_first = nullptr;
  HubRec *d_rec_tab = nullptr;
};

constexpr int kLatShortMax = 8;
constexpr int kRowStreamChunk = 64;

struct SRec {
  int64_t off;
  int32_t len, nslots, off_sidx, pad;
};
struct RowStream {
  int32_t ng = 0, cap = 0, max_rec_words = 0, max_steps = 0;
  int32_t nslots = 0;
  int64_t entries = 0;
  std::vector<int32_t> rec;
  std::vector<SRec> rec_tab;
  std::vector<Fixup> fixups;
  int32_t n_fix_l1 = 0;
  int32_t *d_rec = nullptr;
  SRec *d_rec_tab = nullptr;
  Fixup *d_fixups = nullptr;
};

struct FusedSched {
  int32_t cap = 0;
  int32_t rows_cap = 0;
  int32_t mem_cap = 0;
  int32_t vslot_cap = 0;
  int32_t t_big = 0;
  int32_t vdeg_max = 0;
  int32_t n_mat = 0;
  int32_t n_split = 0;
  bool invalid = false;
  std::vector<FPanel> panels;
  std::vector<int32_t> soff, pmem, slot_eid;
  std::vector<int32_t> prow, pend;
  std::vector<uint16_t> pvs;
  std::vector<int32_t> mat_ptr, mat_ind, mat_eid;
  Sched mat_sched;
  RowStream mat_stream;
  HubPass hub;
  int32_t n_part = 0;
  std::vector<Fixup> fixups;
  int32_t n_fix_l1 = 0;
  Fixup *d_fixups = nullptr;
  int32_t *d_prow = nullptr;
  int32_t *d_mat_ptr = nullptr, *d_mat_ind = nullptr, *d_mat_eid = nullptr;
  int64_t pmem_entries = 0;
  int32_t ng = 0;
  std::vector<int32_t> rec;
  std::vector<FRec> rec_tab;
  int32_t max_rec_words = 0;
  int32_t max_steps = 0;
  int64_t stream_entries = 0;
  int32_t *d_rec = nullptr;
  FRec *d_rec_tab = nullptr;
  std::vector<int32_t> eid_all;
  int32_t *d_eid_all = nullptr;
  float *d_bsA = nullptr, *d_bsB = nullptr, *d_bsD = nullptr;
  const float *bound_degE = nullptr, *bound_W = nullptr, *bound_degV = nullptr;
  bool bound_W_is_one = false;
};

struct Opts {
  int32_t short_max = 32;
  int32_t split_len = 512;
  int32_t panel_rows = 128;
  bool panel_rows_auto = true;
  int32_t panel_nnz = 1024;
  int32_t flags = 0;
  int32_t t_big = 8;
  int32_t fused_tile_bytes = 16384;
  bool fused_tile_auto = true;
  int32_t slot_chunk = 0;
  int32_t fused_steps = 0;
  int64_t hub_min_nnz = 1 << 20;
  int32_t hub_min_deg = 256;
  int32_t hub_tile_bytes = 80 * 1024;
};

void set_error(const std::string &msg);

int balance_schedule(int32_t nrow, int32_t ngs, const int32_t *csrptr,
                     int64_t *n_key, int64_t *n_group, int32_t *key,
                     int32_t *row, int32_t *st, int32_t *ed);
int validate_csr(int32_t nrows, int32_t ncols, const int32_t *ptr,
                 const int32_t *ind);
void transpose_csr(int32_t nrows, int32_t ncols, const int32_t *ptr,
                   const int32_t *ind, std::vector<int32_t> &t_ptr,
                   std::vector<int32_t> &t_ind);
void build_sched(int32_t nrows, const int32_t *ptr, const Opts &o, Sched &s);
void classify_fused(int32_t N, int32_t M, const int32_t *ptr_t, const int32_t *ptr_v, const int32_t *ind_v,
                    const Opts &o, int32_t cap, int32_t mem_cap, int64_t *n_mat, int64_t *n_big);
void build_fused(int32_t N, int32_t M, const int32_t *ptr_t, const int32_t *ind_t,
                 const int32_t *ptr_v, const int32_t *ind_v, const Opts &o, int32_t cap,
                 int32_t mem_cap, int32_t ng, int32_t row_floats, bool allow_hub, FusedSched &f,
                 int32_t rows_cap = 0);
void build_row_stream(int32_t nrows, const int32_t *ptr, const int32_t *ind, const int32_t *scale_index,
                      int32_t ng, int32_t idle, RowStream &rs);
void add_fixups(int32_t row, int32_t first, int32_t count, int32_t &nslots, std::vector<Fixup> &level1,
                std::vector<Fixup> &finals);

}

struct hg_plan {
  int32_t N = 0, M = 0;
  int64_t nnz = 0;
  hg::Opts opts;
  std::vector<int32_t> ptr_t, ind_t;
  std::vector<int32_t> ptr_v, ind_v;
  int32_t *d_ptr_v = nullptr, *d_ind_v = nullptr;
  hg::Sched sched[2];
  hg::Sched sched_lat[2];
  bool has_lat = false;
  std::map<int64_t, hg::FusedSched> fused;
  std::map<int64_t, const hg::FusedSched *> fused_by_width;
  std::mutex fused_mu;
  std::map<int64_t, hg::RowStream> row_streams;
  std::mutex stream_mu;
  int32_t stream_nslots[2] = {0, 0};
  std::map<int64_t, int32_t> auto_choice;
  std::map<int32_t, int32_t> hop_kernel;
  std::mutex auto_mu;
  std::vector<int32_t> perm;
  bool perm_built = false;
  int32_t *d_perm = nullptr;
  std::mutex perm_mu;
  double small_nnz_frac = 0.0;
  int64_t device_bytes = 0;
  int device = -1;
};
```

hypergef_amd/csrc/hg_kernels.h:

```cpp
#pragma once
#include <hip/hip_runtime.h>

#include <algorithm>

#include "hg_internal.h"

namespace hg {

struct bf16 {
  uint16_t bits;
};

struct GatherArgs {
  const int32_t *ptr;
  const int32_t *ind;
  const void *src;
  void *dst;
  const float *scaleA;
  const float *scaleB;
  float *partial;
  const int32_t *scale_map;
  const int32_t *dst_map;
  const Panel *panels;
  const Task *tasks;
  int32_t npanels, ntasks, n_task_blocks;
  int32_t F;
  int32_t panel_rows, panel_nnz;
  int32_t xcd_remap;
  int32_t nt_dst = 0;
};

struct WeightedGatherArgs : GatherArgs {
  const float *w = nullptr;
  const int32_t *wperm = nullptr;
};

struct LinEpilogue {
  const float *R = nullptr;
  float ca = 1.f, cb = 0.f;
  const float *cb_dev = nullptr;
  int32_t relu = 0;
  float *T_out = nullptr;
  const void *wsplit = nullptr;
};

struct FusedArgs {
  int32_t npanels;
  const int32_t *rec;
  const FRec *rec_tab;
  const int32_t *eid_all;
  int32_t max_rec_words;
  int32_t ng;
  int32_t cap, rows_cap;
  int32_t dv_regs = 0;
  const void *X;
  const float *Xe_mat, *degE, *W, *degV;
  const float *bsA, *bsB, *bsD;
  void *Y;
  float *partial = nullptr;
  int32_t F;
  int32_t xcd_remap;
  int32_t x_bytes;
  int32_t mat_bytes;
  int32_t nrows_x;
  int32_t nrows_mat = 0;
  int32_t y_nt = 0;
  int32_t reverse_runs = 0;
  const float *Wlin = nullptr;
  int32_t F_out = 0;
  LinEpilogue epi;
};

struct LinearArgs {
  const float *T;
  const float *Wlin;
  const int32_t *rowmap;
  float *Y;
  int64_t nrows;
  int32_t F_in, F_out;
  LinEpilogue epi;
};

struct HubArgs {
  const int32_t *rec;
  const HubRec *rec_tab;
  const int32_t *wg_first;
  const int32_t *vslot0;
  int32_t nwg, ng, cap, max_rec_words;
  const void *X;
  const float *Xe_mat, *degE, *W;
  float *partial;
  int32_t F;
  int32_t x_bytes, mat_bytes, nrows_x, nrows_mat;
  int32_t n_heavy = 0;
  int32_t hslot0[kHubHeavy] = {};
};

struct StreamArgs {
  const int32_t *rec;
  const SRec *rec_tab;
  int32_t nrec, ng, cap, max_rec_words;
  const void *src;
  int32_t src_bytes, nrows_src;
  const float *scaleA, *scaleB;
  void *dst;
  float *partial;
  int32_t F, xcd_remap;
  int32_t nt_dst = 0;
};

struct PushArgs {
  int64_t n_group;
  const int32_t *group_key, *group_row, *group_st, *group_ed;
  const int32_t *csrptr_t, *colind_t;
  const float *X, *degE, *degV, *W;
  float *Y;
  int32_t F;
};

hipError_t launch_gather(const GatherArgs &a, int nfix, int nfix_l1, const Fixup *fixups, bool vec4,
                         hipStream_t stream, bool src_bf16 = false, bool dst_bf16 = false);
hipError_t launch_gather_weighted(const WeightedGatherArgs &a, int nfix, int nfix_l1, const Fixup *fixups, bool vec4,
                                  hipStream_t stream);
hipError_t launch_incidence_dot(int32_t M, int64_t nnz, int32_t F, const int32_t *ptr, const int32_t *ind, const float *A,
                                const float *B, float *out, bool vec4, hipStream_t stream);
hipError_t launch_fused(const FusedArgs &a, bool vec4, hipStream_t stream, bool xy_bf16 = false);
hipError_t launch_hub_pass(const HubArgs &a, bool vec4, hipStream_t stream, bool x_bf16 = false);
size_t hub_pass_lds_bytes(int32_t cap, int32_t row_floats, int32_t max_rec_words);
hipError_t launch_fixups(const Fixup *fixups, int nfix, int nfix_l1, int32_t F, float *partial, void *Y,
                         const float *scaleA, const float *scaleB, const int32_t *scale_map, bool vec4,
                         hipStream_t stream, bool nt_dst = false, bool Y_bf16 = false);
bool stream_rows_ok(const StreamArgs &a, bool vec4);
hipError_t launch_stream_rows(const StreamArgs &a, hipStream_t stream, bool src_bf16 = false, bool dst_bf16 = false);
bool fused_linear_ok(const FusedArgs &a);
hipError_t launch_linear(const LinearArgs &a, hipStream_t stream);
int wgrad_parts(int64_t nrows, int32_t Fa, int32_t Fb);
bool wgrad_shape_ok(int32_t Fa, int32_t Fb);
hipError_t launch_wgrad(int64_t nrows, int32_t Fa, int32_t Fb, const float *A, const float *B, float *C,
                        float *partial, hipStream_t stream);
hipError_t launch_linear_pack(int32_t F_out, int32_t F_in, const float *Wlin, float *wfrag, hipStream_t stream);
hipError_t launch_linear_pack_split(int32_t F_out, int32_t F_in, const float *Wlin, void *wsplit, hipStream_t stream);
int fused_tile_row_floats(int F, bool vec4);
hipError_t launch_push(const PushArgs &a, hipStream_t stream);
hipError_t launch_bind_scales(int64_t nslots, const int32_t *eid_all, const float *degE, const float *W,
                              float *bsA, float *bsB, int64_t nrows, const int32_t *prow, const float *degV,
                              float *bsD, hipStream_t stream);
hipError_t launch_all_ones(int64_t n, const float *W, int32_t *flag, hipStream_t stream);
hipError_t launch_gather_max(int32_t M, int32_t F, const int32_t *ptr, const int32_t *ind, const float *X,
                             const float *degE, const float *W, float *Xe, int32_t *record,
                             hipStream_t stream);
hipError_t launch_scatter_record(int32_t M, int32_t F, const float *T, const int32_t *record,
                                 const float *degV, float *Y, hipStream_t stream);

}
```

hypergef_amd/csrc/hg_kernels.hip:

```cpp
#include <hip/hip_runtime.h>

#include <atomic>
#include <type_traits>

#include "hg_kernels.h"

namespace hg {

constexpr int kRowsWaves = 7;
template <int VEC> struct Vec;
template <> struct Vec<1> {
  float x;
  __device__ __forceinline__ static Vec zero() { return Vec{0.f}; }
  __device__ __forceinline__ static Vec load(const float *p) { return Vec{*p}; }
  __device__ __forceinline__ static Vec load_buf(__amdgpu_buffer_rsrc_t r, unsigned off) {
    return Vec{__builtin_bit_cast(float, __builtin_amdgcn_raw_buffer_load_b32(r, off, 0, 0))};
  }
  __device__ __forceinline__ static Vec loadu(const float *p) { return Vec{*p}; }
  __device__ __forceinline__ void store(float *p) const { *p = x; }
  __device__ __forceinline__ void store_n(float *p, int) const { *p = x; }
  __device__ __forceinline__ void store_n_nt(float *p, int) const { __builtin_nontemporal_store(x, p); }
  __device__ __forceinline__ void add(const Vec &o) { x += o.x; }
  __device__ __forceinline__ void fma(const Vec &o, float s) { x = __builtin_fmaf(o.x, s, x); }
  __device__ __forceinline__ void mul(float s) { x *= s; }
  __device__ __forceinline__ void xor_reduce(int off) { x += __shfl_xor(x, off, 64); }
};
template <> struct Vec<4> {
  float4 v;
  __device__ __forceinline__ static Vec zero() { return Vec{make_float4(0.f, 0.f, 0.f, 0.f)}; }
  __device__ __forceinline__ static Vec load(const float *p) {
    return Vec{*reinterpret_cast<const float4 *>(p)};
  }
  __device__ __forceinline__ static Vec load_buf(__amdgpu_buffer_rsrc_t r, unsigned off) {
    typedef unsigned u4 __attribute__((ext_vector_type(4)));
    return Vec{__builtin_bit_cast(float4, (u4)__builtin_amdgcn_raw_buffer_load_b128(r, off, 0, 0))};
  }
  __device__ __forceinline__ void store(float *p) const { *reinterpret_cast<float4 *>(p) = v; }
  typedef float f4u __attribute__((ext_vector_type(4), aligned(4)));
  __device__ __forceinline__ static Vec loadu(const float *p) {
    const f4u t = *reinterpret_cast<const f4u *>(p);
    return Vec{make_float4(t.x, t.y, t.z, t.w)};
  }
  __device__ __forceinline__ void storeu(float *p) const { *reinterpret_cast<f4u *>(p) = f4u{v.x, v.y, v.z, v.w}; }
  __device__ __forceinline__ void store_n(float *p, int n) const {
    if (n >= 4) {
      storeu(p);
    } else {
      p[0] = v.x;
      if (n > 1) p[1] = v.y;
      if (n > 2) p[2] = v.z;
    }
  }
  __device__ __forceinline__ void store_nt(float *p) const {
    typedef float f4 __attribute__((ext_vector_type(4)));
    __builtin_nontemporal_store(f4{v.x, v.y, v.z, v.w}, reinterpret_cast<f4 *>(p));
  }
  __device__ __forceinline__ void store_n_nt(float *p, int n) const {
    if (n >= 4) {
      __builtin_nontemporal_store(f4u{v.x, v.y, v.z, v.w}, reinterpret_cast<f4u *>(p));
    } else {
      __builtin_nontemporal_store(v.x, p);
      if (n > 1) __builtin_nontemporal_store(v.y, p + 1);
      if (n > 2) __builtin_nontemporal_store(v.z, p + 2);
    }
  }
  __device__ __forceinline__ void add(const Vec &o) {
    v.x += o.v.x; v.y += o.v.y; v.z += o.v.z; v.w += o.v.w;
  }
  __device__ __forceinline__ void fma(const Vec &o, float s) {
    v.x = __builtin_fmaf(o.v.x, s, v.x); v.y = __builtin_fmaf(o.v.y, s, v.y);
    v.z = __builtin_fmaf(o.v.z, s, v.z); v.w = __builtin_fmaf(o.v.w, s, v.w);
  }
  __device__ __forceinline__ void mul(float s) { v.x *= s; v.y *= s; v.z *= s; v.w *= s; }
  __device__ __forceinline__ void xor_reduce(int off) {
    v.x += __shfl_xor(v.x, off, 64); v.y += __shfl_xor(v.y, off, 64);
    v.z += __shfl_xor(v.z, off, 64); v.w += __shfl_xor(v.w, off, 64);
  }
};

template <typename T, int VEC> struct Rows {
  using V = Vec<VEC>;
  __device__ __forceinline__ static V load(const float *p) { return V::load(p); }
  __device__ __forceinline__ static V load_buf(__amdgpu_buffer_rsrc_t r, unsigned off) { return V::load_buf(r, off); }
  __device__ __forceinline__ static void store(const V &v, float *p) { v.store(p); }
  __device__ __forceinline__ static void store_n(const V &v, float *p, int n) { v.store_n(p, n); }
  __device__ __forceinline__ static void store_n_nt(const V &v, float *p, int n) { v.store_n_nt(p, n); }
};
template <> struct Rows<bf16, 4> {
  using V = Vec<4>;
  typedef unsigned u2 __attribute__((ext_vector_type(2)));
  __device__ __forceinline__ static V widen(u2 u) {
    return V{make_float4(__uint_as_float(u.x << 16), __uint_as_float(u.x & 0xffff0000u), __uint_as_float(u.y << 16),
                         __uint_as_float(u.y & 0xffff0000u))};
  }
  __device__ __forceinline__ static unsigned pack(float lo, float hi) {
    return (unsigned)__builtin_bit_cast(uint16_t, (__bf16)lo) | ((unsigned)__builtin_bit_cast(uint16_t, (__bf16)hi) << 16);
  }
  __device__ __forceinline__ static u2 narrow(const V &v) { return u2{pack(v.v.x, v.v.y), pack(v.v.z, v.v.w)}; }
  __device__ __forceinline__ static V load(const bf16 *p) { return widen(*reinterpret_cast<const u2 *>(p)); }
  __device__ __forceinline__ static V load_buf(__amdgpu_buffer_rsrc_t r, unsigned off) {
    return widen(__builtin_amdgcn_raw_buffer_load_b64(r, off, 0, 0));
  }
  __device__ __forceinline__ static void store(const V &v, bf16 *p) { *reinterpret_cast<u2 *>(p) = narrow(v); }
  __device__ __forceinline__ static void store_n(const V &v, bf16 *p, int) { store(v, p); }
  __device__ __forceinline__ static void store_n_nt(const V &v, bf16 *p, int) {
    __builtin_nontemporal_store(narrow(v), reinterpret_cast<u2 *>(p));
  }
};

template <int LPR, int VEC, typename TS = float, typename TD = float, bool WT = false>
__global__ __launch_bounds__(256) void gather_rows_kernel(const std::conditional_t<WT, WeightedGatherArgs, GatherArgs> a) {
  constexpr int U = 4;
  constexpr int G = 64 / LPR;
  constexpr int NG = 256 / LPR;
  using V = Vec<VEC>;
  using RS = Rows<TS, VEC>;
  using RD = Rows<TD, VEC>;
  extern __shared__ int32_t smem[];
  const TS *src = static_cast<const TS *>(a.src);
  TD *dst = static_cast<TD *>(a.dst);

  const int tid = threadIdx.x;
  const int gl = tid & (LPR - 1);
  const int col = (blockIdx.y * LPR + gl) * VEC;
  const bool col_ok = col < a.F;
  const int64_t F = a.F;
  int b = blockIdx.x;

  if (b < a.n_task_blocks) {
    const int t = __builtin_amdgcn_readfirstlane(b * 4 + (tid >> 6));
    if (t >= a.ntasks) return;
    const Task tk = a.tasks[t];
    const int g = (tid & 63) / LPR;
    V acc = V::zero();
    for (int p = tk.beg + g; p < tk.end; p += G * U) {
      V v[U];
      float wv[U];
#pragma unroll
      for (int k = 0; k < U; k++) {
        const int q = p + k * G;
        const bool ok = col_ok && q < tk.end;
        const int64_t idx = ok ? a.ind[q] : 0;
        if constexpr (WT) wv[k] = ok ? a.w[a.wperm ? a.wperm[q] : q] : 0.f;
        v[k] = ok ? RS::load(src + idx * F + col) : V::zero();
      }
#pragma unroll
      for (int k = 0; k < U; k++) {
        if constexpr (WT) acc.fma(v[k], wv[k]);
        else acc.add(v[k]);
      }
    }
#pragma unroll
    for (int off = LPR; off < 64; off <<= 1) acc.xor_reduce(off);
    if (g == 0 && col_ok) {
      if (tk.slot < 0) {
        const int srow = a.scale_map ? a.scale_map[tk.row] : tk.row;
        const int64_t drow = a.dst_map ? a.dst_map[tk.row] : tk.row;
        if (a.scaleA) acc.mul(a.scaleA[srow]);
        if (a.scaleB) acc.mul(a.scaleB[srow]);
        if (a.nt_dst) RD::store_n_nt(acc, dst + drow * F + col, VEC);
        else RD::store(acc, dst + drow * F + col);
      } else {
        acc.store(a.partial + (int64_t)tk.slot * F + col);
      }
    }
    return;
  }

  b -= a.n_task_blocks;
  if (a.xcd_remap) {
    const int x = b & 7, i = b >> 3;
    const int cpx = a.npanels >> 3, rem = a.npanels & 7;
    b = x * cpx + (x < rem ? x : rem) + i;
  }
  const Panel pn = a.panels[b];
  int32_t *sptr = smem;
  float *sA = reinterpret_cast<float *>(smem + a.panel_rows + 1);
  float *sB = sA + a.panel_rows;
  int32_t *sdst = reinterpret_cast<int32_t *>(sB + a.panel_rows);
  int32_t *sind = sdst + a.panel_rows;

  for (int i = tid; i <= pn.nrows; i += 256) sptr[i] = a.ptr[pn.row0 + i] - pn.nnz0;
  for (int i = tid; i < pn.nrows; i += 256) {
    const int srow = a.scale_map ? a.scale_map[pn.row0 + i] : pn.row0 + i;
    if (a.scaleA) sA[i] = a.scaleA[srow];
    if (a.scaleB) sB[i] = a.scaleB[srow];
    if (a.dst_map) sdst[i] = a.dst_map[pn.row0 + i];
  }
  for (int i = tid; i < pn.nnz_cnt; i += 256) sind[i] = a.ind[pn.nnz0 + i];
  float *sw = reinterpret_cast<float *>(sind + a.panel_nnz);
  if constexpr (WT) {
    for (int i = tid; i < pn.nnz_cnt; i += 256) {
      const int q = pn.nnz0 + i;
      sw[i] = a.w[a.wperm ? a.wperm[q] : q];
    }
  }
  __syncthreads();

  const int g = tid / LPR;
  const int rpg = (pn.nrows + NG - 1) / NG;
  int r = min(g * rpg, pn.nrows);
  const int re = min(r + rpg, pn.nrows);
  if (r >= re) return;

  auto flush = [&](int row, V acc) {
    if (sptr[row + 1] > sptr[row]) {
      if (a.scaleA) acc.mul(sA[row]);
      if (a.scaleB) acc.mul(sB[row]);
    }
    const int64_t drow = a.dst_map ? sdst[row] : pn.row0 + row;
    if (col_ok) {
      if (a.nt_dst) RD::store_n_nt(acc, dst + drow * F + col, VEC);
      else RD::store(acc, dst + drow * F + col);
    }
  };

  int pos = sptr[r];
  const int stop = sptr[re];
  int row_end = sptr[r + 1];
  V acc = V::zero();

  auto issue = [&](int p0, int n, V(&v)[U]) {
#pragma unroll
    for (int k = 0; k < U; k++) {
      const int64_t idx = sind[p0 + min(k, n - 1)];
      v[k] = col_ok ? RS::load(src + idx * F + col) : V::zero();
    }
  };
  auto consume = [&](int p0, int n, const V(&v)[U]) {
#pragma unroll
    for (int k = 0; k < U; k++) {
      if (k < n) {
        while (row_end <= p0 + k) {
          flush(r, acc);
// ... 654 lines not shown
  for (int j = 0; j < NL; j++) {
    const int i = threadIdx.x + j * 256, r = i / (K / 4), c = (i % (K / 4)) * 4;
    *reinterpret_cast<float4 *>(t + r * LD + c) = v[j];
  }
  __syncthreads();
  panel_times_wt<KSTEPS>(t, nrows, a.F_out, a.Wlin, a.rowmap ? a.rowmap + row0 : nullptr, row0, a.Y,
                         threadIdx.x, bv, a.epi.relu);
}

template <int TA, int TB>
__global__ __launch_bounds__(256) __attribute__((amdgpu_waves_per_eu(TA * TB >= 16 ? 3 : TA * TB >= 8 ? 4 : 1, 8))) void wgrad_kernel(const float *A, const float *B, float *partial, int64_t N,
                                                    int64_t rows_per_wg, int lda, int ldb, int nbb, int nblocks, int nparts) {
  constexpr int FA = TA * 16, FB = TB * 16;
  int part = blockIdx.x, blk = 0;
  if (nblocks > 1) {
    const int xcd = blockIdx.x & 7, k = blockIdx.x >> 3;
    blk = k % nblocks;
    part = (k / nblocks) * 8 + xcd;
  }
  A += (blk / nbb) * FA;
  B += (blk % nbb) * FB;
  __shared__ float red[FA * FB];
  const int lane = threadIdx.x & 63, wave = threadIdx.x >> 6;
  const int kk = lane >> 4, c = lane & 15;
  const int64_t wg0 = min(N, (int64_t)part * rows_per_wg);
  const int64_t wg1 = min(N, wg0 + rows_per_wg);
  const int64_t per_wave = (rows_per_wg / 4 + 3) & ~(int64_t)3;
  const int64_t r0 = min(wg1, wg0 + wave * per_wave), r1 = min(wg1, r0 + per_wave);
  hg_f4 acc[TA][TB];
#pragma unroll
  for (int i = 0; i < TA; i++)
#pragma unroll
    for (int j = 0; j < TB; j++) acc[i][j] = hg_f4{0.f, 0.f, 0.f, 0.f};
  float a0[TA], b0[TB], a1[TA], b1[TB];
  auto load = [&](int64_t n, float (&a)[TA], float (&b)[TB]) {
    const int64_t row = min(n + kk, r1 - 1);
    typedef float f4u __attribute__((ext_vector_type(4), aligned(4)));
    typedef float f2u __attribute__((ext_vector_type(2), aligned(4)));
    auto fetch = [&](const float *p, auto &dst, auto nt) {
      constexpr int T = decltype(nt)::value;
      if constexpr (T % 4 == 0) {
#pragma unroll
        for (int q = 0; q < T / 4; q++) {
          const f4u v = *reinterpret_cast<const f4u *>(p + 4 * q);
          dst[4 * q] = v.x; dst[4 * q + 1] = v.y; dst[4 * q + 2] = v.z; dst[4 * q + 3] = v.w;
        }
      } else if constexpr (T == 2) {
        const f2u v = *reinterpret_cast<const f2u *>(p);
        dst[0] = v.x; dst[1] = v.y;
      } else {
#pragma unroll
        for (int q = 0; q < T; q++) dst[q] = p[q];
      }
    };
    fetch(A + row * lda + c * TA, a, std::integral_constant<int, TA>{});
    fetch(B + row * ldb + c * TB, b, std::integral_constant<int, TB>{});
  };
  auto step = [&](const float (&a)[TA], const float (&b)[TB]) {
#pragma unroll
    for (int i = 0; i < TA; i++)
#pragma unroll
      for (int j = 0; j < TB; j++)
        acc[i][j] = __builtin_amdgcn_mfma_f32_16x16x4f32(a[i], b[j], acc[i][j], 0, 0, 0);
  };
  float a2[TA], b2[TB];
  if (r0 < r1) {
    const int64_t rfull = r0 + ((r1 - r0) & ~(int64_t)3);
    load(r0, a0, b0);
    load(r0 + 4, a1, b1);
    int64_t n = r0;
    for (; n + 12 <= rfull; n += 12) {
      load(n + 8, a2, b2);
      __builtin_amdgcn_sched_barrier(0);
      step(a0, b0);
      __builtin_amdgcn_sched_barrier(0);
      load(n + 12, a0, b0);
      __builtin_amdgcn_sched_barrier(0);
      step(a1, b1);
      __builtin_amdgcn_sched_barrier(0);
      load(n + 16, a1, b1);
      __builtin_amdgcn_sched_barrier(0);
      step(a2, b2);
      __builtin_amdgcn_sched_barrier(0);
    }
    auto tail = [&](float (&a)[TA], float (&b)[TB], int64_t at) {
      if (at >= r1) return;
      const bool ok = at + kk < r1;
#pragma unroll
      for (int i = 0; i < TA; i++) a[i] = ok ? a[i] : 0.f;
#pragma unroll
      for (int j = 0; j < TB; j++) b[j] = ok ? b[j] : 0.f;
      step(a, b);
    };
    if (n + 8 <= rfull) {
      load(n + 8, a2, b2);
      step(a0, b0);
      step(a1, b1);
      tail(a2, b2, n + 8);
    } else if (n + 4 <= rfull) {
      step(a0, b0);
      tail(a1, b1, n + 4);
    } else {
      tail(a0, b0, n);
    }
  }
  for (int w = 0; w < 4; w++) {
    if (wave == w) {
#pragma unroll
      for (int i = 0; i < TA; i++)
#pragma unroll
        for (int j = 0; j < TB; j++)
#pragma unroll
          for (int q = 0; q < 4; q++) {
            float *d = red + (TA * (4 * kk + q) + i) * FB + TB * c + j;
            *d = w == 0 ? acc[i][j][q] : *d + acc[i][j][q];
          }
    }
    __syncthreads();
  }
  float *out = partial + ((int64_t)blk * nparts + part) * FA * FB;
  for (int i = threadIdx.x; i < FA * FB; i += 256) out[i] = red[i];
}

__global__ __launch_bounds__(256) void wgrad_reduce_kernel(const float *partial, int nparts, int n, float *out, int fa, int fb, int ldc, int nbb) {
  const int i = blockIdx.x * 256 + threadIdx.x;
  if (i >= n) return;
  const int c = blockIdx.y, nchunks = gridDim.y, z = blockIdx.z;
  partial += (int64_t)z * nparts * n;
  float s = 0.f;
  for (int p = c; p < nparts; p += nchunks) s += partial[(int64_t)p * n + i];
  if (fb > 0) out[(int64_t)((z / nbb) * fa + i / fb) * ldc + (z % nbb) * fb + (i % fb)] = s;
  else out[((int64_t)z * nchunks + c) * n + i] = s;
}

constexpr int kLinWaves8 = 8, kLinWaves16 = 6, kLinWaves32 = 5, kLinWavesStaged = 8;
constexpr int kLinWavesStaged32 = 6;
constexpr int kLinU32 = 12;
typedef unsigned hg_u4 __attribute__((ext_vector_type(4)));
typedef int hg_i4 __attribute__((ext_vector_type(4)));

__host__ __device__ inline int lin_tile_floats(int cap, int rows_cap, int tw) {
  const int rows16 = (rows_cap + 15) / 16 * 16;
  const int a = cap * tw, b = rows16 * (tw + 4);
  return a > b ? a : b;
}

template <int LPR, int VEC, int U, bool FAST, bool MAT, bool SCALED, bool LIN = false, int BS = 256, bool LINW = true, bool SPLIT = false,
          typename T = float>
__global__ __launch_bounds__(BS) __attribute__((amdgpu_waves_per_eu(LIN ? (!LINW ? (LPR >= 32 ? kLinWavesStaged32 : kLinWavesStaged) : LPR >= 32 ? kLinWaves32 : LPR == 16 ? kLinWaves16 : kLinWaves8) : 1, 8))) void fused_packed_kernel(const FusedArgs a) {
  static_assert(!LIN || BS == 256, "the linear epilogue is written for four waves");
  static_assert(!SPLIT || (LIN && !LINW && LPR == 32 && VEC == 4), "bf16x6 matrix phase: K = 128 staged instances");
  static_assert(!LIN || std::is_same_v<T, float>, "the linear epilogue takes fp32 rows");
  constexpr bool XF32 = std::is_same_v<T, float>;
  constexpr int NG = BS / LPR;
  constexpr int TW = LPR * VEC;
  using V = Vec<VEC>;
  using RX = Rows<T, VEC>;
  extern __shared__ int32_t smem[];
  const int64_t F = a.F;
  const int tid = threadIdx.x;
  const int gl = tid & (LPR - 1);
  const int lcol = gl * VEC;
  const int col = blockIdx.y * TW + lcol;
  const bool col_ok = col < a.F;
  int b = blockIdx.x;
  if (a.xcd_remap) {
    const int x = b & 7;
    int i = b >> 3;
    const int cpx = a.npanels >> 3, rem = a.npanels & 7;
    if (MAT && a.reverse_runs) i = cpx + (x < rem ? 1 : 0) - 1 - i;
    b = x * cpx + (x < rem ? x : rem) + i;
  }

  float *tile = reinterpret_cast<float *>(smem);
  int32_t *rec = smem + (LIN ? lin_tile_floats(a.cap, a.rows_cap, TW) : a.cap * TW);
  float *sA = reinterpret_cast<float *>(rec + a.max_rec_words);
  float *sB = sA + (a.degE ? a.cap : 0);
  float *sdeg = sB + (a.W ? a.cap : 0);

  const FRec rt = a.rec_tab[b];
  const int32_t *grec = a.rec + rt.off;
  const int g = tid / LPR;
  const bool dv_regs = SCALED && a.dv_regs != 0;
  [[maybe_unused]] float dv[4] = {1.f, 1.f, 1.f, 1.f};
  if constexpr (SCALED) {
    if (dv_regs) {
      const int rpg0 = (rt.nrows + NG - 1) / NG;
      const int q0 = min(g * rpg0, rt.nrows), q1 = min(q0 + rpg0, rt.nrows);
#pragma unroll
      for (int i = 0; i < 4; i++)
        if (q0 + i < q1) dv[i] = a.bsD[rt.row_base + q0 + i];
    }
  }

  const int nrec4 = rt.len >> 2;
  const hg_i4 *grec4 = reinterpret_cast<const hg_i4 *>(grec);
  const bool bound_e = SCALED && a.bsA && (a.degE || a.W) && rt.nslots > 0, bound_v = a.degV && !dv_regs && a.bsD && rt.nrows > 0;
  const bool pre = bound_e || bound_v;
  if (pre) {
    const hg_i4 rv = grec4[min(tid, nrec4 - 1)];
    float va = 1.f, vb = 1.f, vd = 1.f;
    if (bound_e) {
      const int64_t si = rt.slot_base + min(tid, rt.nslots - 1);
      if (a.degE) va = a.bsA[si];
      if (a.W) vb = a.bsB[si];
    }
    if (bound_v) vd = a.bsD[rt.row_base + min(tid, rt.nrows - 1)];
    if (tid < nrec4) reinterpret_cast<hg_i4 *>(rec)[tid] = rv;
    if (bound_e && tid < rt.nslots) {
      if (a.degE) sA[tid] = va;
      if (a.W) sB[tid] = vb;
    }
    if (bound_v && tid < rt.nrows) sdeg[tid] = vd;
  }
  for (int i = pre ? tid + BS : tid; i < nrec4; i += BS)
    reinterpret_cast<hg_i4 *>(rec)[i] = grec4[i];
  if (a.degE || a.W)
    for (int i = bound_e ? tid + BS : tid; i < rt.nslots; i += BS) {
      if (a.bsA) {
        if (a.degE) sA[i] = a.bsA[rt.slot_base + i];
        if (a.W) sB[i] = a.bsB[rt.slot_base + i];
      } else {
        const int e = a.eid_all[rt.slot_base + i];
        if (a.degE) sA[i] = e >= 0 ? a.degE[e] : 1.f;
        if (a.W) sB[i] = e >= 0 ? a.W[e] : 1.f;
      }
    }
  if (a.degV && !dv_regs)
    for (int i = bound_v ? tid + BS : tid; i < rt.nrows; i += BS) {
      if (a.bsD) {
        sdeg[i] = a.bsD[rt.row_base + i];
      } else {
        const int pr = grec[rt.off_prow + i];
        sdeg[i] = pr < 0 ? 1.f : a.degV[pr];
      }
    }
  __syncthreads();
  const int steps = rec[0], nrows = rec[1];
  const int32_t *gbase = rec + rec[4];
  const int32_t *stream = rec + rec[5];
  const uint16_t *pend = reinterpret_cast<const uint16_t *>(rec + rec[6]);
  const int32_t *prow = rec + rec[7];
  const uint16_t *pvs = reinterpret_cast<const uint16_t *>(rec + rec[9]);

  {
    [[maybe_unused]] int slot = gbase[g];
    float *tp = tile + gbase[g] * TW + lcol;
    V acc = V::zero();
    [[maybe_unused]] const unsigned row_bytes = (unsigned)a.F * 4u;
    [[maybe_unused]] const unsigned col_off = col_ok ? (unsigned)col * 4u : 0x80000000u;
    [[maybe_unused]] const unsigned xrow_bytes = (unsigned)a.F * (unsigned)sizeof(T);
    [[maybe_unused]] const unsigned xcol_off = col_ok ? (unsigned)col * (unsigned)sizeof(T) : 0x80000000u;
    [[maybe_unused]] const T *X = static_cast<const T *>(a.X);
    [[maybe_unused]] __amdgpu_buffer_rsrc_t rx, rm;
    if constexpr (FAST) {
      rx = __builtin_amdgcn_make_buffer_rsrc(const_cast<void *>(a.X), 0, a.x_bytes, 0x00020000);
      rm = __builtin_amdgcn_make_buffer_rsrc(const_cast<void *>(a.Xe_mat ? static_cast<const void *>(a.Xe_mat) : a.X), 0,
                                             a.Xe_mat ? a.mat_bytes : 0, 0x00020000);
    }
    auto block = [&](const int s0, const int send, auto full, auto matph) {
      constexpr bool FULL = decltype(full)::value;
      constexpr bool MATPH = decltype(matph)::value;
      const int idle = MATPH ? a.nrows_mat : a.nrows_x;
      int ent[U];
#pragma unroll
      for (int j = 0; j < U; j++) ent[j] = (FULL || s0 + j < send) ? stream[(s0 + j) * NG + g] : idle;
      V v[U];
#pragma unroll
      for (int j = 0; j < U; j++) {
        if (!FULL && s0 + j >= send) {
          v[j] = V::zero();
          continue;
        }
        if constexpr (FAST && !XF32 && !MATPH) {
          v[j] = RX::load_buf(rx, __umul24((unsigned)ent[j], xrow_bytes) + xcol_off);
        } else if constexpr (FAST) {
          const unsigned off = __umul24((unsigned)ent[j], row_bytes) + col_off;
          v[j] = V::load_buf(MATPH ? rm : rx, off);
        } else if constexpr (!XF32 && !MATPH) {
          const bool on = col_ok && ent[j] != idle;
          const int64_t idx = ent[j] & 0x3fffffff;
          v[j] = on ? RX::load(X + idx * F + col) : V::zero();
        } else {
          const bool on = col_ok && ent[j] != idle;
          const int64_t idx = ent[j] & 0x3fffffff;
          const float *base = MATPH ? a.Xe_mat : static_cast<const float *>(a.X);
          v[j] = on ? V::load(base + idx * F + col) : V::zero();
        }
      }
#pragma unroll
      for (int j = 0; j < U; j++) {
        acc.add(v[j]);
        if (ent[j] < 0) {
          if constexpr (SCALED) {
            if (a.degE) acc.mul(sA[slot]);
            if (a.W) acc.mul(sB[slot]);
            slot++;
          }
          acc.store(tp);
          tp += TW;
          acc = V::zero();
        }
      }
    };
    const int steps_x = MAT ? rec[8] : steps;
    if constexpr (MAT && FAST && ((LIN && !LINW && LPR >= 32) || (!LIN && VEC == 4 && BS == 256))) {
      auto mixed = [&](const int s0, auto full) {
        constexpr bool FULL = decltype(full)::value;
        int ent[U];
#pragma unroll
        for (int j = 0; j < U; j++) ent[j] = (FULL || s0 + j < steps) ? stream[(s0 + j) * NG + g] : 0;
        V v[U];
#pragma unroll
        for (int j = 0; j < U; j++) {
          if (!FULL && s0 + j >= steps) {
            v[j] = V::zero();
            continue;
          }
          const unsigned off = __umul24((unsigned)ent[j], row_bytes) + col_off;
          if (s0 + j >= steps_x) v[j] = V::load_buf(rm, off);
          else if constexpr (XF32) v[j] = V::load_buf(rx, off);
          else v[j] = RX::load_buf(rx, __umul24((unsigned)ent[j], xrow_bytes) + xcol_off);
        }
#pragma unroll
        for (int j = 0; j < U; j++) {
          acc.add(v[j]);
          if (ent[j] < 0) {
            if constexpr (SCALED) {
              if (a.degE) acc.mul(sA[slot]);
              if (a.W) acc.mul(sB[slot]);
              slot++;
            }
            acc.store(tp);
            tp += TW;
            acc = V::zero();
          }
        }
      };
      int s0 = 0;
      for (; s0 + U <= steps; s0 += U) mixed(s0, std::true_type{});
      if (s0 < steps) mixed(s0, std::false_type{});
    } else {
      int s0 = 0;
      for (; s0 + U <= steps_x; s0 += U) block(s0, steps_x, std::true_type{}, std::false_type{});
      if (s0 < steps_x) block(s0, steps_x, std::false_type{}, std::false_type{});
      if constexpr (MAT) {
        for (s0 = steps_x; s0 + U <= steps; s0 += U) block(s0, steps, std::true_type{}, std::true_type{});
        if (s0 < steps) block(s0, steps, std::false_type{}, std::true_type{});
      }
    }
  }
  __syncthreads();
  if constexpr (LIN) {
    [[maybe_unused]] float bv[BPre<TW / 4>::N];
    [[maybe_unused]] SplitB bsp[kSplitDepth];
    const LinSplit sp = lin_split(tid >> 6, a.F_out >> 4);
    if constexpr (SPLIT) {
      if (sp.active) {
#pragma unroll
        for (int t = 0; t < kSplitDepth; t++)
          bsp[t] = load_bsplit_step(static_cast<const uint4 *>(a.epi.wsplit), sp, a.F_out >> 4, a.F_out > 64 ? 2 : 1, t, tid & 63);
      }
    }
    const int rpg = (nrows + NG - 1) / NG;
    const int r0 = min(g * rpg, nrows), r1 = min(r0 + rpg, nrows);
    V rr[4];
    if (a.epi.R) {
#pragma unroll
      for (int i = 0; i < 4; i++) rr[i] = V::load(a.epi.R + (int64_t)prow[min(r0 + i, nrows - 1)] * F + col);
    }
    V outr[4];
#pragma unroll
    for (int i = 0; i < 4; i++) {
      outr[i] = V::zero();
      const int r = r0 + i;
      if (r < r1) {
        const int pb = r ? pend[r - 1] : 0, pe = pend[r];
        for (int p = pb; p < pe; p++) outr[i].add(V::load(tile + (int)pvs[p] * TW + lcol));
        if (a.degV && pe > pb) outr[i].mul(dv_regs ? dv[i] : sdeg[r]);
      }
    }
    if (a.epi.R || a.epi.ca != 1.f) {
      const float cb = a.epi.cb_dev ? *a.epi.cb_dev : a.epi.cb;
#pragma unroll
      for (int i = 0; i < 4; i++)
        if (r0 + i < r1) {
          outr[i].mul(a.epi.ca);
          if (a.epi.R) {
            rr[i].mul(cb);
            outr[i].add(rr[i]);
          }
        }
    }
    if constexpr (SPLIT) {
      const int pstride = split_plane_bytes(a.rows_cap);
      if (a.epi.T_out) {
#pragma unroll
        for (int i = 0; i < 4; i++)
          if (r0 + i < r1) outr[i].store(a.epi.T_out + (int64_t)prow[r0 + i] * TW + lcol);
      }
      __syncthreads();
#pragma unroll
      for (int i = 0; i < 4; i++)
        if (r0 + i < r1) split_store_row(reinterpret_cast<char *>(tile), pstride, r0 + i, lcol, outr[i].v);
      __syncthreads();
      if (a.F_out > 64) panel_times_wt_split<2>(tile, pstride, nrows, a.F_out, static_cast<const uint4 *>(a.epi.wsplit), prow, static_cast<float *>(a.Y), tid, bsp, a.epi.relu);
      else panel_times_wt_split<1>(tile, pstride, nrows, a.F_out, static_cast<const uint4 *>(a.epi.wsplit), prow, static_cast<float *>(a.Y), tid, bsp, a.epi.relu);
      return;
    }
    if (sp.active) load_bfrag_pre<TW / 4>(a.Wlin, sp.nt_first, tid & 63, bv);
    __syncthreads();
#pragma unroll
    for (int i = 0; i < 4; i++)
      if (r0 + i < r1) outr[i].store(tile + (r0 + i) * (TW + 4) + lcol);
    __syncthreads();
    if (a.epi.T_out) {
      constexpr int q = TW >> 2;
      for (int i = tid; i < nrows * q; i += 256) {
        const int r = i / q, c = (i - r * q) * 4;
        *reinterpret_cast<float4 *>(a.epi.T_out + (int64_t)prow[r] * TW + c) =
            *reinterpret_cast<const float4 *>(tile + r * (TW + 4) + c);
      }
    }
    panel_times_wt<TW / 4, LINW>(tile, nrows, a.F_out, a.Wlin, prow, 0, static_cast<float *>(a.Y), tid, bv, a.epi.relu);
    return;
  } else {
    const int rpg = (nrows + NG - 1) / NG;
    const int r0 = min(g * rpg, nrows), r1 = min(r0 + rpg, nrows);
    auto row = [&](const int r, const float dscale) {
      V acc = V::zero();
      const int pb = r ? pend[r - 1] : 0, pe = pend[r];
      for (int p = pb; p < pe; p++) acc.add(V::load(tile + (int)pvs[p] * TW + lcol));
      if (a.degV && pe > pb) acc.mul(dv_regs ? dscale : sdeg[r]);
      if (col_ok) {
        const int pr = prow[r];
        if constexpr (XF32) {
          float *dst = (pr < 0 ? a.partial + (int64_t)(pr & 0x7fffffff) * F : static_cast<float *>(a.Y) + (int64_t)pr * F) + col;
          if (a.y_nt && pr >= 0) acc.store_n_nt(dst, a.F - col);
          else acc.store_n(dst, a.F - col);
        } else {
          if (pr < 0) {
            acc.store_n(a.partial + (int64_t)(pr & 0x7fffffff) * F + col, a.F - col);
          } else {
            T *y = static_cast<T *>(a.Y) + (int64_t)pr * F + col;
            if (a.y_nt) RX::store_n_nt(acc, y, a.F - col);
            else RX::store_n(acc, y, a.F - col);
          }
        }
      }
    };
    if (SCALED && dv_regs) {
#pragma unroll
      for (int i = 0; i < 4; i++)
        if (r0 + i < r1) row(r0 + i, dv[i]);
    } else {
      for (int r = r0; r < r1; r++) row(r, 1.f);
    }
  }
}
// ... 341 lines not shown

constexpr size_t kLdsMax = 160 * 1024;
template <auto Kern, int BLOCK = 256, typename Args>
static hipError_t launch_lds(dim3 grid, size_t lds, hipStream_t stream, const Args &a) {
  static std::atomic<size_t> granted{64 * 1024};
  if (lds > kLdsMax) return hipErrorInvalidValue;
  if (lds > granted.load(std::memory_order_relaxed)) {
    hipError_t e = hipFuncSetAttribute(reinterpret_cast<const void *>(Kern),
                                       hipFuncAttributeMaxDynamicSharedMemorySize, (int)kLdsMax);
    if (e != hipSuccess) return e;
    granted.store(kLdsMax, std::memory_order_relaxed);
  }
  hipLaunchKernelGGL(Kern, grid, dim3(BLOCK), lds, stream, a);
  return hipGetLastError();
}

template <int LPR, int VEC, typename TD = float>
static hipError_t launch_fixups_t(const GatherArgs &a, int nfix, int nfix_l1, const Fixup *fixups, hipStream_t stream) {
  const int col_tiles = (a.F + LPR * VEC - 1) / (LPR * VEC);
  const int per_block = 256 / LPR;
  if (nfix_l1 > 0)
    hipLaunchKernelGGL((fixup_rows_kernel<LPR, VEC, TD>), dim3((nfix_l1 + per_block - 1) / per_block, col_tiles),
                       dim3(256), 0, stream, a, fixups, nfix_l1);
  if (nfix > nfix_l1)
    hipLaunchKernelGGL((fixup_rows_kernel<LPR, VEC, TD>),
                       dim3((nfix - nfix_l1 + per_block - 1) / per_block, col_tiles), dim3(256), 0, stream, a,
                       fixups + nfix_l1, nfix - nfix_l1);
  return hipGetLastError();
}

template <int LPR, int VEC, typename TS = float, typename TD = float, bool WT = false>
static hipError_t launch_gather_t(const std::conditional_t<WT, WeightedGatherArgs, GatherArgs> &a, int nfix, int nfix_l1,
                                  const Fixup *fixups, hipStream_t stream) {
  const int col_tiles = (a.F + LPR * VEC - 1) / (LPR * VEC);
  const int nblocks = a.n_task_blocks + a.npanels;
  if (nblocks > 0) {
    const size_t lds = (size_t)(4 * a.panel_rows + 1 + (WT ? 2 : 1) * a.panel_nnz) * sizeof(int32_t);
    const dim3 grid(nblocks, col_tiles);
    const hipError_t e = launch_lds<gather_rows_kernel<LPR, VEC, TS, TD, WT>>(grid, lds, stream, a);
    if (e != hipSuccess) return e;
  }
  return launch_fixups_t<LPR, VEC, TD>(a, nfix, nfix_l1, fixups, stream);
}

hipError_t launch_gather(const GatherArgs &a, int nfix, int nfix_l1, const Fixup *fixups, bool vec4,
                         hipStream_t stream, bool src_bf16, bool dst_bf16) {
  const int lanes = vec4 ? a.F / 4 : a.F;
  const int lpr = std::min(64, next_pow2(std::max(lanes, 1)));
  if ((src_bf16 || dst_bf16) && (!vec4 || (src_bf16 && dst_bf16))) return hipErrorInvalidValue;
#define HG_CASE(L)                                                                                       \
  case L:                                                                                                \
    if (src_bf16) return launch_gather_t<L, 4, bf16, float>(a, nfix, nfix_l1, fixups, stream);            \
    if (dst_bf16) return launch_gather_t<L, 4, float, bf16>(a, nfix, nfix_l1, fixups, stream);            \
    return vec4 ? launch_gather_t<L, 4>(a, nfix, nfix_l1, fixups, stream)                                \
                : launch_gather_t<L, 1>(a, nfix, nfix_l1, fixups, stream);
  switch (lpr) {
    HG_CASE(1)
    HG_CASE(2)
    HG_CASE(4)
    HG_CASE(8)
    HG_CASE(16)
    HG_CASE(32)
    HG_CASE(64)
  }
#undef HG_CASE
  return hipErrorInvalidValue;
}

hipError_t launch_gather_weighted(const WeightedGatherArgs &a, int nfix, int nfix_l1, const Fixup *fixups, bool vec4,
                                  hipStream_t stream) {
  if (!a.w) return hipErrorInvalidValue;
  const int lanes = vec4 ? a.F / 4 : a.F;
  const int lpr = std::min(64, next_pow2(std::max(lanes, 1)));
#define HG_CASE(L)                                                                                     \
  case L:                                                                                              \
    return vec4 ? launch_gather_t<L, 4, float, float, true>(a, nfix, nfix_l1, fixups, stream)          \
                : launch_gather_t<L, 1, float, float, true>(a, nfix, nfix_l1, fixups, stream);
  switch (lpr) {
    HG_CASE(1)
    HG_CASE(2)
    HG_CASE(4)
    HG_CASE(8)
    HG_CASE(16)
    HG_CASE(32)
    HG_CASE(64)
  }
#undef HG_CASE
  return hipErrorInvalidValue;
}

hipError_t launch_incidence_dot(int32_t M, int64_t nnz, int32_t F, const int32_t *ptr, const int32_t *ind, const float *A,
                                const float *B, float *out, bool vec4, hipStream_t stream) {
  if (nnz == 0) return hipSuccess;
  if (M <= 0 || F <= 0 || (vec4 && F % 4)) return hipErrorInvalidValue;
  const int lanes = vec4 ? F / 4 : F;
  const int lpr = std::min(64, next_pow2(std::max(lanes, 1)));
  const int64_t per_block = (int64_t)(256 / lpr) * kDotRun;
  const int64_t nblocks = (nnz + per_block - 1) / per_block;
  if (nblocks > 0x7fffffff) return hipErrorInvalidValue;
#define HG_CASE(L)                                                                                                   \
  case L:                                                                                                            \
    if (vec4) hipLaunchKernelGGL((incidence_dot_kernel<L, 4>), dim3((unsigned)nblocks), dim3(256), 0, stream, ptr, ind, M, \
                                 nnz, F, A, B, out);                                                                 \
    else hipLaunchKernelGGL((incidence_dot_kernel<L, 1>), dim3((unsigned)nblocks), dim3(256), 0, stream, ptr, ind, M,   \
                            nnz, F, A, B, out);                                                                      \
    return hipGetLastError();
  switch (lpr) {
    HG_CASE(1)
    HG_CASE(2)
    HG_CASE(4)
    HG_CASE(8)
    HG_CASE(16)
    HG_CASE(32)
    HG_CASE(64)
  }
#undef HG_CASE
  return hipErrorInvalidValue;
}

hipError_t launch_fixups(const Fixup *fixups, int nfix, int nfix_l1, int32_t F, float *partial, void *Y,
                         const float *scaleA, const float *scaleB, const int32_t *scale_map, bool vec4,
                         hipStream_t stream, bool nt_dst, bool Y_bf16) {
  if (nfix == 0) return hipSuccess;
  if (Y_bf16 && (!vec4 || (F & 3))) return hipErrorInvalidValue;
  GatherArgs a{};
  a.nt_dst = nt_dst ? 1 : 0;
  a.F = F;
  a.partial = partial;
  a.dst = Y;
  a.scaleA = scaleA;
  a.scaleB = scaleB;
  a.scale_map = scale_map;
  const int lanes = vec4 ? (F + 3) / 4 : F;
  const int lpr = std::min(64, next_pow2(std::max(lanes, 1)));
#define HG_CASE(L)                                                                      \
  case L:                                                                               \
    if (Y_bf16) return launch_fixups_t<L, 4, bf16>(a, nfix, nfix_l1, fixups, stream);   \
    return vec4 ? launch_fixups_t<L, 4>(a, nfix, nfix_l1, fixups, stream) : launch_fixups_t<L, 1>(a, nfix, nfix_l1, fixups, stream);
  switch (lpr) {
    HG_CASE(1)
    HG_CASE(2)
    HG_CASE(4)
    HG_CASE(8)
    HG_CASE(16)
    HG_CASE(32)
    HG_CASE(64)
  }
#undef HG_CASE
  return hipErrorInvalidValue;
}

bool stream_rows_ok(const StreamArgs &a, bool vec4) {
  return vec4 && a.nrec > 0 && a.src_bytes > 0 && a.nrows_src < (1 << 24) && a.F < (1 << 22) &&
         a.ng == 256 / (fused_tile_row_floats(a.F, true) / 4) &&
         (size_t)a.max_rec_words * 4 + (size_t)2 * a.cap * 4 <= kLdsMax;
}

template <int LPR>
static hipError_t launch_stream_t(const StreamArgs &a, hipStream_t stream, bool src_bf16, bool dst_bf16) {
  constexpr int TW = LPR * 4;
  const dim3 grid(a.nrec, (a.F + TW - 1) / TW);
  const size_t lds = (size_t)a.max_rec_words * 4 + (size_t)2 * a.cap * 4;
  if (src_bf16) return launch_lds<stream_rows_kernel<LPR, 4, 8, bf16, float>>(grid, lds, stream, a);
  if (dst_bf16) return launch_lds<stream_rows_kernel<LPR, 4, 8, float, bf16>>(grid, lds, stream, a);
  return launch_lds<stream_rows_kernel<LPR, 4, 8>>(grid, lds, stream, a);
}

hipError_t launch_stream_rows(const StreamArgs &a, hipStream_t stream, bool src_bf16, bool dst_bf16) {
  if (a.nrec == 0) return hipSuccess;
  if ((src_bf16 && dst_bf16) || ((src_bf16 || dst_bf16) && (a.F & 3))) return hipErrorInvalidValue;
  switch (fused_tile_row_floats(a.F, true) / 4) {
    case 1: return launch_stream_t<1>(a, stream, src_bf16, dst_bf16);
    case 2: return launch_stream_t<2>(a, stream, src_bf16, dst_bf16);
    case 4: return launch_stream_t<4>(a, stream, src_bf16, dst_bf16);
    case 8: return launch_stream_t<8>(a, stream, src_bf16, dst_bf16);
    case 16: return launch_stream_t<16>(a, stream, src_bf16, dst_bf16);
    case 32: return launch_stream_t<32>(a, stream, src_bf16, dst_bf16);
    case 64: return launch_stream_t<64>(a, stream, src_bf16, dst_bf16);
  }
  return hipErrorInvalidValue;
}

size_t hub_pass_lds_bytes(int32_t cap, int32_t row_floats, int32_t max_rec_words) {
  return (size_t)(cap + 1) * row_floats * 4 + (size_t)2 * max_rec_words * 4 + (size_t)2 * cap * 4 + 16;
}

template <int LPR, typename T>
static hipError_t launch_hub_t(const HubArgs &a, hipStream_t stream) {
  constexpr int TW = LPR * 4;
  if (a.ng != 1024 / LPR) return hipErrorInvalidValue;
  const bool fast = a.x_bytes > 0 && a.nrows_x < (1 << 24) && a.F < (1 << 22) &&
                    (!a.Xe_mat || (a.mat_bytes > 0 && a.nrows_mat < (1 << 24)));
  if (!fast) return hipErrorInvalidValue;
  const dim3 grid(a.nwg, (a.F + TW - 1) / TW);
  const size_t lds = hub_pass_lds_bytes(a.cap, TW, a.max_rec_words);
  if (a.cap < 1024 / LPR) return hipErrorInvalidValue;
  const int spec = (a.Xe_mat ? 1 : 0) | ((a.degE || a.W) ? 2 : 0) | (a.n_heavy > 0 ? 4 : 0);
#define HG_HUB(M, S, H) return launch_lds<hub_pass_kernel<LPR, 4, 4, M, S, H, T>, 1024>(grid, lds, stream, a)
  switch (spec) {
    case 0: HG_HUB(false, false, false);
    case 1: HG_HUB(true, false, false);
    case 2: HG_HUB(false, true, false);
    case 3: HG_HUB(true, true, false);
    case 4: HG_HUB(false, false, true);
    case 5: HG_HUB(true, false, true);
    case 6: HG_HUB(false, true, true);
    default: HG_HUB(true, true, true);
  }
#undef HG_HUB
}

hipError_t launch_hub_pass(const HubArgs &a, bool vec4, hipStream_t stream, bool x_bf16) {
  if (a.nwg == 0) return hipSuccess;
  if (!vec4) return hipErrorInvalidValue;
  if (x_bf16 && (a.F & 3)) return hipErrorInvalidValue;
  const int lpr = fused_tile_row_floats(a.F, true) / 4;
#define HG_CASE(L) \
  case L: return x_bf16 ? launch_hub_t<L, bf16>(a, stream) : launch_hub_t<L, float>(a, stream);
  switch (lpr) {
    HG_CASE(4)
    HG_CASE(8)
    HG_CASE(16)
    HG_CASE(32)
    HG_CASE(64)
  }
#undef HG_CASE
  return hipErrorInvalidValue;
}

static size_t fused_scale_floats(const FusedArgs &a) {
  return (size_t)(a.degE ? a.cap : 0) + (size_t)(a.W ? a.cap : 0) + (size_t)((a.degV && !a.dv_regs) ? a.rows_cap : 0);
}
static int fused_dv_regs(const FusedArgs &a, int ng, size_t lds_without_scales, int max_wgs) {
  if (!((a.degE || a.W) && a.degV && a.bsD && a.rows_cap <= 4 * ng)) return 0;
  const size_t common = lds_without_scales + ((size_t)(a.degE ? a.cap : 0) + (size_t)(a.W ? a.cap : 0)) * 4;
  const size_t with = common + (size_t)a.rows_cap * 4;
  const int fit_with = (int)std::min<size_t>((size_t)max_wgs, kLdsMax / with);
  const int fit_without = (int)std::min<size_t>((size_t)max_wgs, kLdsMax / common);
  return fit_without > fit_with ? 1 : 0;
}

template <int LPR, int VEC, typename T = float>
static hipError_t launch_fused_t(const FusedArgs &a, hipStream_t stream) {
  if (a.npanels == 0) return hipSuccess;
  constexpr int TW = LPR * VEC;
  constexpr bool XF32 = std::is_same_v<T, float>;
  if constexpr (VEC == 4 && (LPR == 8 || LPR == 16)) {
    if (a.ng == 1024 / LPR) {
      const bool fast = a.x_bytes > 0 && a.nrows_x < (1 << 24) && a.F < (1 << 22) && (a.F & 3) == 0;
      if (!fast || a.Wlin || a.Xe_mat) return hipErrorInvalidValue;
      const dim3 grid(a.npanels, (a.F + TW - 1) / TW);
      const size_t lds = (size_t)a.cap * TW * 4 + (size_t)a.max_rec_words * 4 + fused_scale_floats(a) * 4 + 16;
      if (a.degE || a.W) return launch_lds<fused_packed_kernel<LPR, VEC, 8, true, false, true, false, 1024, true, false, T>, 1024>(grid, lds, stream, a);
      return launch_lds<fused_packed_kernel<LPR, VEC, 8, true, false, false, false, 1024, true, false, T>, 1024>(grid, lds, stream, a);
    }
  }
  if (a.ng != 256 / LPR) return hipErrorInvalidValue;
  const int col_tiles = (a.F + TW - 1) / TW;
  FusedArgs ad = a;
  const dim3 grid(a.npanels, col_tiles);
  ad.dv_regs = a.Wlin ? 0 : fused_dv_regs(a, 256 / LPR, (size_t)a.cap * TW * 4 + (size_t)a.max_rec_words * 4 + 16, 8);
  const size_t lds_p = (size_t)a.cap * TW * 4 + (size_t)a.max_rec_words * 4 + fused_scale_floats(ad) * 4 + 16;
  if constexpr (VEC == 4) {
    const bool fast = a.x_bytes > 0 && a.nrows_x < (1 << 24) && a.F < (1 << 22) &&
                      (!a.Xe_mat || (a.mat_bytes > 0 && a.nrows_mat < (1 << 24)));
    if (a.Wlin) {
      if constexpr (XF32 && (TW == 32 || TW == 64 || TW == 128)) {
        if (!fast || a.F != TW || a.rows_cap > 4 * (256 / LPR) || (a.F_out & 15)) return hipErrorInvalidValue;
        const size_t lds_l = lds_p - (size_t)a.cap * TW * 4 + (size_t)lin_tile_floats(a.cap, a.rows_cap, TW) * 4;
        const int spec = (a.Xe_mat ? 1 : 0) | ((a.degE || a.W) ? 2 : 0);
        const int nt_all = a.F_out >> 4, nwr = nt_all >= 3 ? 1 : 4 / nt_all;
        const bool staged = a.F_out <= TW && (((a.rows_cap + 15) >> 4) + nwr - 1) / nwr <= (a.F_out > 64 ? 2 : 4);
        constexpr int UL = LPR >= 32 ? kLinU32 : 8;
        bool split = false;
        if constexpr (TW == 128) {
          const int ps = split_plane_bytes(a.rows_cap), tile_b = lin_tile_floats(a.cap, a.rows_cap, TW) * 4;
          split = a.epi.wsplit && staged && a.rows_cap > 0 && a.rows_cap <= 32 && 3 * ps <= tile_b && 2 * ps + 32 * 256 <= (int)lds_l;
        }
        if (!split) ad.epi.wsplit = nullptr;
#define HG_PKL(M, S)                                                                                                          \
  if constexpr (TW == 128)                                                                                                    \
    if (split) return launch_lds<fused_packed_kernel<LPR, VEC, UL, true, M, S, true, 256, false, true>>(grid, lds_l, stream, ad); \
  return staged ? launch_lds<fused_packed_kernel<LPR, VEC, UL, true, M, S, true, 256, false>>(grid, lds_l, stream, ad) \
                : launch_lds<fused_packed_kernel<LPR, VEC, 8, true, M, S, true, 256, true>>(grid, lds_l, stream, ad)
        switch (spec) {
          case 0: HG_PKL(false, false);
          case 1: HG_PKL(true, false);
          case 2: HG_PKL(false, true);
          default: HG_PKL(true, true);
        }
#undef HG_PKL
      } else {
        return hipErrorInvalidValue;
      }
    }
    if (fast) {
      const bool u16 = a.npanels <= 512;
      const int spec = (a.Xe_mat ? 1 : 0) | ((a.degE || a.W) ? 2 : 0);
#define HG_PK(UU, M, S) return launch_lds<fused_packed_kernel<LPR, VEC, UU, true, M, S, false, 256, true, false, T>>(grid, lds_p, stream, ad)
      if (u16) {
        switch (spec) {
          case 0: HG_PK(16, false, false);
          case 1: HG_PK(16, true, false);
          case 2: HG_PK(16, false, true);
          default: HG_PK(16, true, true);
        }
      } else {
        switch (spec) {
          case 0: HG_PK(8, false, false);
          case 1: HG_PK(8, true, false);
          case 2: HG_PK(8, false, true);
          default: HG_PK(8, true, true);
        }
      }
#undef HG_PK
    }
    if (a.F & 3) return hipErrorInvalidValue;
  }
  if (a.Wlin) return hipErrorInvalidValue;
  if constexpr (XF32 && VEC == 1 && LPR >= 8) {
    const bool fast = a.x_bytes > 0 && a.nrows_x < (1 << 24) && a.F < (1 << 22) &&
                      (!a.Xe_mat || (a.mat_bytes > 0 && a.nrows_mat < (1 << 24)));
    if (fast) {
      if (!a.Xe_mat && !a.degE && !a.W)
        return launch_lds<fused_packed_kernel<LPR, VEC, 8, true, false, false>>(grid, lds_p, stream, ad);
      return launch_lds<fused_packed_kernel<LPR, VEC, 8, true, true, true>>(grid, lds_p, stream, ad);
    }
  }
  return launch_lds<fused_packed_kernel<LPR, VEC, 8, false, true, true, false, 256, true, false, T>>(grid, lds_p, stream, ad);
}

hipError_t launch_linear_pack_split(int32_t F_out, int32_t F_in, const float *Wlin, void *wsplit, hipStream_t stream) {
  if (F_out <= 0 || F_in != 128 || (F_out & 15)) return hipErrorInvalidValue;
  const int64_t n = (int64_t)(F_out >> 4) * (F_in >> 5) * 64;
  hipLaunchKernelGGL(linear_pack_split_kernel, dim3((unsigned)((n + 255) / 256)), dim3(256), 0, stream, F_out, F_in, Wlin,
                     static_cast<uint4 *>(wsplit));
  return hipGetLastError();
}

hipError_t launch_linear_pack(int32_t F_out, int32_t F_in, const float *Wlin, float *wfrag, hipStream_t stream) {
  if (F_out <= 0 || F_in <= 0 || (F_out & 15) || (F_in & 15)) return hipErrorInvalidValue;
  const int64_t n = (int64_t)F_out * F_in;
  hipLaunchKernelGGL(linear_pack_kernel, dim3((unsigned)((n + 255) / 256)), dim3(256), 0, stream, F_out, F_in,
                     Wlin, wfrag);
  return hipGetLastError();
}

bool wgrad_blocked(int32_t Fa, int32_t Fb) { return (Fa / 16) * (Fb / 16) > 16; }
bool wgrad_shape_ok(int32_t Fa, int32_t Fb) {
  if (Fa <= 0 || Fb <= 0 || (Fa & 15) || (Fb & 15)) return false;
  if (!wgrad_blocked(Fa, Fb)) return true;
  return (Fa % 64) == 0 && (Fb % 64) == 0 && Fa <= 512 && Fb <= 512;
}
int wgrad_parts(int64_t nrows, int32_t Fa, int32_t Fb) {
  const bool blocked = wgrad_blocked(Fa, Fb);
  if (blocked) Fa = Fb = 64;
  const int tiles = (Fa / 16) * (Fb / 16);
  const int64_t cap = tiles <= 4 ? 2048 : (tiles <= 8 ? 1024 : 768);
  const int n = (int)std::max<int64_t>(1, std::min<int64_t>(cap, (nrows + 63) / 64));
  return blocked ? (n + 7) / 8 * 8 : n;
}

hipError_t launch_wgrad(int64_t nrows, int32_t Fa, int32_t Fb, const float *A, const float *B, float *C,
                        float *partial, hipStream_t stream) {
  if (!wgrad_shape_ok(Fa, Fb)) return hipErrorInvalidValue;
  const bool blocked = wgrad_blocked(Fa, Fb);
  const int32_t Ba = blocked ? 64 : Fa, Bb = blocked ? 64 : Fb;
  const int nba = Fa / Ba, nbb = Fb / Bb, nblocks = nba * nbb;
  const int nparts = wgrad_parts(nrows, Fa, Fb);
  int64_t rows_per_wg = (nrows + nparts - 1) / nparts;
  rows_per_wg = (rows_per_wg + 15) & ~(int64_t)15;
#define HG_WG(TA_, TB_)                                                                                          \
  if (Ba == 16 * TA_ && Bb == 16 * TB_) {                                                                        \
    hipLaunchKernelGGL((wgrad_kernel<TA_, TB_>), dim3(nparts * nblocks), dim3(256), 0, stream, A, B, partial, nrows, rows_per_wg, Fa, Fb, nbb, nblocks, nparts); \
  } else
  HG_WG(1, 1) HG_WG(1, 2) HG_WG(2, 1) HG_WG(2, 2) HG_WG(1, 4) HG_WG(4, 1) HG_WG(2, 4) HG_WG(4, 2) HG_WG(4, 4)
  HG_WG(1, 8) HG_WG(8, 1) HG_WG(2, 8) HG_WG(8, 2) HG_WG(1, 3) HG_WG(3, 1) HG_WG(3, 3) HG_WG(3, 4) HG_WG(4, 3)
  HG_WG(2, 3) HG_WG(3, 2) { return hipErrorInvalidValue; }
#undef HG_WG
  hipError_t e = hipGetLastError();
  if (e != hipSuccess) return e;
  const int n = Ba * Bb;
  const int mid = nparts > 64 ? 32 : 1;
  float *p2 = partial + (int64_t)nblocks * nparts * n;
  if (mid > 1) {
    hipLaunchKernelGGL(wgrad_reduce_kernel, dim3((n + 255) / 256, mid, nblocks), dim3(256), 0, stream, partial, nparts, n, p2, 0, 0, 0, nbb);
    hipLaunchKernelGGL(wgrad_reduce_kernel, dim3((n + 255) / 256, 1, nblocks), dim3(256), 0, stream, p2, mid, n, C, Ba, Bb, Fb, nbb);
  } else {
    hipLaunchKernelGGL(wgrad_reduce_kernel, dim3((n + 255) / 256, 1, nblocks), dim3(256), 0, stream, partial, nparts, n, C, Ba, Bb, Fb, nbb);
  }
  return hipGetLastError();
}

bool fused_linear_ok(const FusedArgs &a) {
  const int lpr = a.F / 4;
  return (a.F == 32 || a.F == 64 || a.F == 128) && a.F_out > 0 && (a.F_out & 15) == 0 && a.x_bytes > 0 && a.nrows_x < (1 << 24) &&
         (!a.Xe_mat || (a.mat_bytes > 0 && a.nrows_mat < (1 << 24))) &&
         a.ng == 256 / lpr && a.rows_cap <= 4 * (256 / lpr) && a.rows_cap <= a.cap;
}

hipError_t launch_linear(const LinearArgs &a, hipStream_t stream) {
  if (a.nrows == 0) return hipSuccess;
  if ((a.F_out & 15) || a.F_out <= 0) return hipErrorInvalidValue;
  const int R = a.F_in >= 128 ? 32 : 64;
  const int64_t nb = (a.nrows + R - 1) / R;
  if (nb > 0x7fffffffLL) return hipErrorInvalidValue;
  const dim3 grid((unsigned)nb), block(256);
  switch (a.F_in) {
    case 32: hipLaunchKernelGGL((linear_rows_kernel<8>), grid, block, 0, stream, a); break;
    case 64: hipLaunchKernelGGL((linear_rows_kernel<16>), grid, block, 0, stream, a); break;
    case 128: hipLaunchKernelGGL((linear_rows_kernel<32>), grid, block, 0, stream, a); break;
    default: return hipErrorInvalidValue;
  }
  return hipGetLastError();
}


int fused_tile_row_floats(int F, bool vec4);

hipError_t launch_fused(const FusedArgs &a, bool vec4, hipStream_t stream, bool xy_bf16) {
  const int lpr = fused_tile_row_floats(a.F, vec4) / (vec4 ? 4 : 1);
  if (xy_bf16 && (!vec4 || a.Wlin || (a.F & 3))) return hipErrorInvalidValue;
#define HG_CASE(L)                                              \
  case L:                                                       \
    if (xy_bf16) return launch_fused_t<L, 4, bf16>(a, stream);   \
    return vec4 ? launch_fused_t<L, 4>(a, stream) : launch_fused_t<L, 1>(a, stream);
  switch (lpr) {
    HG_CASE(1)
    HG_CASE(2)
    HG_CASE(4)
    HG_CASE(8)
    HG_CASE(16)
    HG_CASE(32)
    HG_CASE(64)
  }
#undef HG_CASE
  return hipErrorInvalidValue;
}

int fused_tile_row_floats(int F, bool vec4) {
  const int lanes = vec4 ? (F + 3) / 4 : F;
  return std::min(64, next_pow2(std::max(lanes, 1))) * (vec4 ? 4 : 1);
}

hipError_t launch_push(const PushArgs &a, hipStream_t stream) {
  const int lpr = std::min(64, next_pow2(std::max(a.F, 1)));
  const int per_block = 256 / lpr;
  const int col_tiles = (a.F + lpr - 1) / lpr;
  const int64_t nblocks = (a.n_group + per_block - 1) / per_block;
  if (nblocks == 0) return hipSuccess;
  if (nblocks > 0x7fffffffLL) return hipErrorInvalidValue;
#define HG_CASE(L)                                                                              \
  case L:                                                                                       \
    hipLaunchKernelGGL((push_tasks_kernel<L>), dim3((unsigned)nblocks, col_tiles), dim3(256), 0, \
                       stream, a);                                                              \
    break;
  switch (lpr) {
    HG_CASE(1)
    HG_CASE(2)
    HG_CASE(4)
    HG_CASE(8)
    HG_CASE(16)
    HG_CASE(32)
    HG_CASE(64)
  }
#undef HG_CASE
  return hipGetLastError();
}

__global__ __launch_bounds__(256) void gather_max_kernel(int32_t M, int32_t F, const int32_t *ptr,
                                                         const int32_t *ind, const float *X,
                                                         const float *degE, const float *W, float *Xe,
                                                         int32_t *record) {
  const int64_t t = (int64_t)blockIdx.x * 256 + threadIdx.x;
  if (t >= (int64_t)M * F) return;
  const int32_t e = (int32_t)(t / F), k = (int32_t)(t % F);
  float best = -1e5f;
  int32_t who = 0;
  for (int32_t p = ptr[e]; p < ptr[e + 1]; p++) {
    const int32_t u = ind[p];
    const float x = X[(int64_t)u * F + k];
    if (x > best) {
      best = x;
      who = u;
    }
  }
  const float degE_val = degE ? degE[e] : 1.f, W_val = W ? W[e] : 1.f;
  best *= degE_val * W_val;
  Xe[t] = best;
  record[t] = who;
}

__global__ __launch_bounds__(256) void scatter_record_kernel(int32_t M, int32_t F, const float *T,
                                                             const int32_t *record, const float *degV,
                                                             float *Y) {
  const int64_t t = (int64_t)blockIdx.x * 256 + threadIdx.x;
  if (t >= (int64_t)M * F) return;
  const int32_t k = (int32_t)(t % F);
  const int64_t v = record[t];
  atomicAdd(Y + v * F + k, T[t] * (degV ? degV[v] : 1.f));
}

__global__ __launch_bounds__(256) void bind_scales_kernel(int64_t nslots, const int32_t *eid_all,
                                                          const float *degE, const float *W, float *bsA,
                                                          float *bsB, int64_t nrows, const int32_t *prow,
                                                          const float *degV, float *bsD) {
  const int64_t t = (int64_t)blockIdx.x * 256 + threadIdx.x;
  if (t < nslots) {
    const int e = eid_all[t];
    bsA[t] = (degE && e >= 0) ? degE[e] : 1.f;
    bsB[t] = (W && e >= 0) ? W[e] : 1.f;
  }
  if (t < nrows) bsD[t] = (degV && prow[t] >= 0) ? degV[prow[t]] : 1.f;
}

hipError_t launch_bind_scales(int64_t nslots, const int32_t *eid_all, const float *degE, const float *W,
                              float *bsA, float *bsB, int64_t nrows, const int32_t *prow, const float *degV,
                              float *bsD, hipStream_t stream) {
  const int64_t n = std::max(nslots, nrows);
  if (n == 0) return hipSuccess;
  hipLaunchKernelGGL(bind_scales_kernel, dim3((unsigned)((n + 255) / 256)), dim3(256), 0, stream, nslots,
                     eid_all, degE, W, bsA, bsB, nrows, prow, degV, bsD);
  return hipGetLastError();
}

__global__ __launch_bounds__(256) void all_ones_kernel(int64_t n, const float *W, int32_t *flag) {
  int64_t i = (int64_t)blockIdx.x * 256 + threadIdx.x;
  bool ok = true;
  for (; i < n; i += (int64_t)gridDim.x * 256) ok = ok && W[i] == 1.0f;
  if (__builtin_amdgcn_ballot_w64(!ok) != 0 && (threadIdx.x & 63) == 0) *flag = 0;
}

hipError_t launch_all_ones(int64_t n, const float *W, int32_t *flag, hipStream_t stream) {
  if (n == 0) return hipSuccess;
  const unsigned blocks = (unsigned)std::min<int64_t>(1024, (n + 255) / 256);
  hipLaunchKernelGGL(all_ones_kernel, dim3(blocks), dim3(256), 0, stream, n, W, flag);
  return hipGetLastError();
}

hipError_t launch_gather_max(int32_t M, int32_t F, const int32_t *ptr, const int32_t *ind, const float *X,
                             const float *degE, const float *W, float *Xe, int32_t *record,
                             hipStream_t stream) {
  const int64_t n = (int64_t)M * F;
  if (n == 0) return hipSuccess;
  hipLaunchKernelGGL(gather_max_kernel, dim3((unsigned)((n + 255) / 256)), dim3(256), 0, stream, M, F, ptr, ind,
                     X, degE, W, Xe, record);
  return hipGetLastError();
}

hipError_t launch_scatter_record(int32_t M, int32_t F, const float *T, const int32_t *record,
                                 const float *degV, float *Y, hipStream_t stream) {
  const int64_t n = (int64_t)M * F;
  if (n == 0) return hipSuccess;
  hipLaunchKernelGGL(scatter_record_kernel, dim3((unsigned)((n + 255) / 256)), dim3(256), 0, stream, M, F, T,
                     record, degV, Y);
  return hipGetLastError();
}

}
```

include/hg_aggr.h:

```cpp
#ifndef HG_AGGR_H
#define HG_AGGR_H

#include <stddef.h>
#include <stdint.h>

#ifdef __cplusplus
extern "C" {
#endif

#define HG_AGGR_VERSION 410

#if defined(__GNUC__)
#define HG_API __attribute__((visibility("default")))
#else
#define HG_API
#endif

typedef enum hg_status {
  HG_OK = 0,
  HG_ERR_INVALID = -1,
  HG_ERR_NOMEM = -2,
  HG_ERR_HIP = -3,
  HG_ERR_WORKSPACE = -4,
  HG_ERR_UNSUPPORTED = -5
} hg_status;

typedef void *hg_stream_t;
typedef struct hg_plan hg_plan;

typedef enum hg_variant {
  HG_VARIANT_AUTO = 0,
  HG_VARIANT_PULL = 1,
  HG_VARIANT_PUSH_ATOMIC = 2,
  HG_VARIANT_FUSED = 3
} hg_variant;

typedef struct hg_plan_opts {
  int32_t short_max;
  int32_t split_len;
  int32_t panel_rows;
  int32_t panel_nnz;
  int32_t flags;
  int32_t t_big;
  int32_t fused_tile_bytes;
  int32_t fused_steps;
} hg_plan_opts;

#define HG_PLAN_HOST_ONLY 1
#define HG_PLAN_NO_XCD_REMAP 2
#define HG_PLAN_DFS_ORDER 4
#define HG_PLAN_NO_ROW_STREAM 16
#define HG_PLAN_NO_HUB_PASS 8

typedef struct hg_plan_info {
  int32_t N, M;
  int64_t nnz;
  int32_t short_max, split_len, panel_rows, panel_nnz, flags;
  int32_t panels[2];
  int32_t tasks[2];
  int32_t partials[2];
  int32_t fixups[2];
  int32_t max_len[2];
  int64_t device_bytes;
} hg_plan_info;

typedef struct hg_fused_info {
  int32_t cap;
  int32_t t_big, vdeg_max;
  int32_t panels;
  int32_t n_mat;
  int32_t n_hub;
  int64_t slots;
  int64_t member_entries;
  int32_t n_split;
  int32_t fixups;
  int32_t hub_rounds, hub_workgroups;
  int64_t hub_entries;
  int64_t hub_pairs;
  int64_t partial_rows;
  int32_t record_words_max;
  int32_t stream_steps_max;
  int32_t lds_bytes;
  int32_t reserved;
} hg_fused_info;

HG_API int hg_version(void);
HG_API const char *hg_last_error(void);
HG_API const char *hg_status_string(int status);

HG_API int hg_balance_schedule(int32_t nrow, int32_t ngs, const int32_t *csrptr_host,
                        int64_t *n_key, int64_t *n_group, int32_t *key,
                        int32_t *row, int32_t *group_st, int32_t *group_ed);

HG_API int hg_mtx_read(const char *path, int32_t *nrow, int32_t *ncol, int64_t *nnz,
                       int32_t **H_ptr, int32_t **H_ind, int32_t **HT_ptr, int32_t **HT_ind);
HG_API void hg_free(void *p);

HG_API int hg_plan_create_host(hg_plan **out, int32_t N, int32_t M,
                        const int32_t *csrptr_t_host,
                        const int32_t *colind_t_host,
                        const hg_plan_opts *opts);
HG_API int hg_plan_create_device(hg_plan **out, int32_t N, int32_t M, int64_t nnz,
                          const int32_t *csrptr_t_dev,
                          const int32_t *colind_t_dev,
                          const hg_plan_opts *opts, hg_stream_t stream);
HG_API void hg_plan_destroy(hg_plan *plan);
HG_API int hg_plan_get_info(const hg_plan *plan, hg_plan_info *info);
HG_API int hg_plan_get_vertex_csr(const hg_plan *plan, int32_t *ptr_v_host,
                           int32_t *ind_v_host);
HG_API int hg_plan_get_vertex_csr_device(const hg_plan *plan, const int32_t **ptr_v_dev,
                                  const int32_t **ind_v_dev);
HG_API int hg_plan_prepare(const hg_plan *plan, int32_t F, hg_fused_info *info);
HG_API int hg_plan_bind_scales(const hg_plan *plan, int32_t F, const float *degE,
                               const float *degV, const float *W, hg_stream_t stream);
HG_API int hg_plan_auto_variant(const hg_plan *plan, int32_t F);
typedef struct hg_tune_info {
  int32_t variant;
  int32_t pull_hop_kernels;
  float us[10];
  int32_t reserved;
} hg_tune_info;
HG_API int hg_plan_tune_f32(const hg_plan *plan, int32_t F, const int32_t *csrptr_t, const int32_t *colind_t,
                            const float *X, const float *degE, const float *degV, const float *W, float *Y,
                            void *workspace, size_t workspace_bytes, int32_t iters, hg_stream_t stream,
                            hg_tune_info *info);
HG_API int hg_plan_get_schedule(const hg_plan *plan, int32_t hop, int32_t *panels,
                                int32_t *tasks, int32_t *fixups);
HG_API size_t hg_plan_workspace_bytes(const hg_plan *plan, int32_t F);

HG_API int hg_aggr_fused_f32(const hg_plan *plan, int32_t F,
                      const int32_t *csrptr_t, const int32_t *colind_t,
                      const float *X, const float *degE, const float *degV,
                      const float *W, float *Y, void *workspace,
                      size_t workspace_bytes, int32_t variant,
                      hg_stream_t stream);

HG_API int hg_aggr_fused_bf16(const hg_plan *plan, int32_t F,
                      const int32_t *csrptr_t, const int32_t *colind_t,
                      const uint16_t *X, const float *degE, const float *degV,
                      const float *W, uint16_t *Y, void *workspace,
                      size_t workspace_bytes, int32_t variant,
                      hg_stream_t stream);

HG_API int hg_linear_pack_f32(int32_t F_out, int32_t F_in, const float *Wlin, float *wfrag,
                              hg_stream_t stream);
#define HG_LIN_RELU 1
#define HG_LIN_BF16X6 2
HG_API size_t hg_linear_pack_floats(int32_t F_out, int32_t F_in, int32_t flags);
HG_API int hg_linear_pack_ex_f32(int32_t F_out, int32_t F_in, const float *Wlin, float *wfrag, int32_t flags,
                                 hg_stream_t stream);
HG_API size_t hg_aggr_linear_workspace_bytes(const hg_plan *plan, int32_t F_in);
HG_API int hg_aggr_linear_res_f32(const hg_plan *plan, int32_t F_in, int32_t F_out,
                                  const int32_t *csrptr_t, const int32_t *colind_t, const float *X,
                                  const float *degE, const float *degV, const float *W,
                                  const float *wfrag, const float *R, float ca, float cb, int32_t relu,
                                  float *T_out, float *Y, void *workspace, size_t workspace_bytes,
                                  int32_t variant, hg_stream_t stream);
HG_API int hg_aggr_linear_res_dev_f32(const hg_plan *plan, int32_t F_in, int32_t F_out,
                                      const int32_t *csrptr_t, const int32_t *colind_t, const float *X,
                                      const float *degE, const float *degV, const float *W,
                                      const float *wfrag, const float *R, float ca, const float *cb_dev,
                                      int32_t relu, float *T_out, float *Y, void *workspace,
                                      size_t workspace_bytes, int32_t variant, hg_stream_t stream);
HG_API size_t hg_linear_wgrad_workspace_bytes(int64_t nrows, int32_t F_a, int32_t F_b);
HG_API int hg_linear_wgrad_f32(int64_t nrows, int32_t F_a, int32_t F_b, const float *A, const float *B,
                               float *C, void *workspace, size_t workspace_bytes, hg_stream_t stream);
HG_API int hg_linear_rows_f32(int64_t nrows, int32_t F_in, int32_t F_out, const float *T,
                              const float *wfrag, float *Y, hg_stream_t stream);
HG_API int hg_aggr_linear_f32(const hg_plan *plan, int32_t F_in, int32_t F_out,
                              const int32_t *csrptr_t, const int32_t *colind_t, const float *X,
                              const float *degE, const float *degV, const float *W,
                              const float *wfrag, float *Y, void *workspace, size_t workspace_bytes,
                              int32_t variant, hg_stream_t stream);

HG_API int hg_gather_rows_f32(const hg_plan *plan, int32_t hop, int32_t F,
                       const int32_t *csrptr_t, const int32_t *colind_t,
                       const float *src, const float *scaleA,
                       const float *scaleB, float *dst, void *workspace,
                       size_t workspace_bytes, hg_stream_t stream);

HG_API size_t hg_aggr_incidence_workspace_bytes(const hg_plan *plan, int32_t F);
HG_API int hg_aggr_incidence_f32(const hg_plan *plan, int32_t F, const int32_t *csrptr_t, const int32_t *colind_t,
                                 const float *X, const float *v2e_val, const float *e2v_val,
                                 const float *degE, const float *degV, const float *W,
                                 float *Xe_out, float *Y, void *workspace, size_t workspace_bytes, hg_stream_t stream);
HG_API int hg_incidence_dot_f32(const hg_plan *plan, int32_t F, const int32_t *csrptr_t, const int32_t *colind_t,
                                const float *A, const float *B, float *out, hg_stream_t stream);
HG_API int hg_plan_get_incidence_perm(const hg_plan *plan, int32_t *perm_host);

HG_API int hg_gather_max_f32(int32_t M, int32_t F, const int32_t *csrptr_t, const int32_t *colind_t,
                             const float *X, const float *degE, const float *W, float *Xe,
                             int32_t *record, hg_stream_t stream);
HG_API int hg_scatter_record_f32(int32_t N, int32_t M, int32_t F, const float *T,
                                 const int32_t *record, const float *degV, float *Y,
                                 hg_stream_t stream);

HG_API int hg_aggr_push_groups_f32(int32_t N, int32_t M, int32_t F, int64_t n_group,
                            const int32_t *group_key, const int32_t *group_row,
                            const int32_t *group_st, const int32_t *group_ed,
                            const int32_t *csrptr_t, const int32_t *colind_t,
                            const float *X, const float *degE,
                            const float *degV, const float *W, float *Y,
                            hg_stream_t stream);

#ifdef __cplusplus
}
#endif
#endif
```

Measured before the change: 32.85 billion edges/s.

## Add 32-byte-per-lane wide fused kernel variant for F=32 with half the lanes per row

Introduces a Vec8 lane type so each lane handles eight floats (two split float4 halves), halving lanes per row and doubling row groups per 256-thread block for F=32 (and optionally 64/128). The scheduler builds fused panels with the new lane-group count when the graph has enough panels, and falls back when it does not. Hub and row-stream passes keep the old 16-lane grouping. The aim is more rows in flight per block and more independent loads per lane, at the cost of higher register pressure and an extra schedule variant with cache keying and binding logic.

```diff
diff --git a/hypergef_amd/_lib.py b/hypergef_amd/_lib.py
--- a/hypergef_amd/_lib.py
+++ b/hypergef_amd/_lib.py
@@ -60,7 +60,7 @@
                 ("hub_entries", ctypes.c_int64), ("hub_pairs", ctypes.c_int64),
                 ("partial_rows", ctypes.c_int64),
                 ("record_words_max", ctypes.c_int32), ("stream_steps_max", ctypes.c_int32),
-                ("lds_bytes", ctypes.c_int32), ("reserved", ctypes.c_int32)]
+                ("lds_bytes", ctypes.c_int32), ("lane_groups", ctypes.c_int32)]
 
     def as_dict(self):
         return {name: getattr(self, name) for name, _ in self._fields_}
diff --git a/hypergef_amd/csrc/hg_api.hip b/hypergef_amd/csrc/hg_api.hip
--- a/hypergef_amd/csrc/hg_api.hip
+++ b/hypergef_amd/csrc/hg_api.hip
@@ -145,7 +145,7 @@
   cap = c / 16 * 16;
   mem_cap = cap * 4;
   if (p->opts.fused_steps > 0) {
-    const int32_t ng = 256 / (hg::fused_tile_row_floats(F, vec4) / (vec4 ? 4 : 1));
+    const int32_t ng = hg::fused_lane_groups(F, vec4, false);
     mem_cap = std::max(p->opts.t_big, std::min(mem_cap, p->opts.fused_steps * ng));
   }
 }
@@ -161,30 +161,42 @@
   if (!vec4 || F != 128 || !p->opts.fused_tile_auto || p->opts.fused_steps > 0 || p->nnz <= (1 << 18)) return false;
   const int pct = 150;
   fused_caps(p, F, vec4, cap, mem_cap);
-  const int32_t ng = 256 / (hg::fused_tile_row_floats(F, vec4) / 4);
+  const int32_t ng = hg::fused_lane_groups(F, vec4, false);
   rows_cap = std::min(cap, 4 * ng);
   cap = std::max(cap, (rows_cap * pct / 100 + 7) / 8 * 8);
   mem_cap = cap * 4;
   return true;
 }
 
-int get_fused(const hg_plan *cp, int32_t F, bool vec4, const hg::FusedSched **out, bool lin = false) {
+bool wide_lanes_ok(const hg_plan *p, int32_t F, bool vec4) {
+  return vec4 && hg::fused_wide_width(F) && wide_rows_ok(p, F) && p->N > hg::kWideMinPanels;
+}
+
+int get_fused(const hg_plan *cp, int32_t F, bool vec4, const hg::FusedSched **out, bool lin = false, bool lane16 = false) {
   hg_plan *p = const_cast<hg_plan *>(cp);
   int32_t cap, mem_cap, rows_cap = 0;
   if (lin && !lin_caps(p, F, vec4, cap, mem_cap, rows_cap)) lin = false;
   if (!lin) fused_caps(p, F, vec4, cap, mem_cap);
   const int32_t row_floats = hg::fused_tile_row_floats(F, vec4);
-  const int32_t ng = 256 / (row_floats / (vec4 ? 4 : 1));
+  const int32_t ng16 = hg::fused_lane_groups(F, vec4, false);
+  const int64_t wkey = (int64_t)F * 2 + (vec4 ? 1 : 0);
+  bool wide = !lin && !lane16 && wide_lanes_ok(p, F, vec4);
+  if (wide) {
+    std::lock_guard<std::mutex> lock(p->fused_mu);
+    if (p->wide_off.count(wkey)) wide = false;
+  }
+  if (!wide_lanes_ok(p, F, vec4)) lane16 = false;
+  const int32_t ng = hg::fused_lane_groups(F, vec4, wide);
   const bool allow_hub = vec4 && F % 4 == 0 && F >= 16 && p->N < (1 << 24) && p->M < (1 << 24) && (int64_t)p->N * F * 4 < ((int64_t)1 << 31) &&
                          (int64_t)p->M * F * 4 < ((int64_t)1 << 31);
   const int64_t key = ((((int64_t)cap * 1000000 + mem_cap) * 1000 + ng) * 2 + (allow_hub ? 1 : 0)) * 1024 + rows_cap;
-  std::lock_guard<std::mutex> lock(p->fused_mu);
+  std::unique_lock<std::mutex> lock(p->fused_mu);
   auto it = p->fused.find(key);
   if (it == p->fused.end()) {
     hg::FusedSched f;
     try {
       hg::build_fused(p->N, p->M, p->ptr_t.data(), p->ind_t.data(), p->ptr_v.data(), p->ind_v.data(),
-                      p->opts, cap, mem_cap, ng, row_floats, allow_hub, f, rows_cap);
+                      p->opts, cap, mem_cap, ng, row_floats, allow_hub, f, rows_cap, ng16);
       if (p->nnz <= (1 << 18)) {
         double best = small_graph_cost(f);
         const int32_t tiles[3] = {p->opts.fused_tile_bytes, p->opts.fused_tile_bytes / 2, p->opts.fused_tile_bytes / 4};
@@ -204,7 +216,7 @@
             }
             hg::FusedSched alt;
             hg::build_fused(p->N, p->M, p->ptr_t.data(), p->ind_t.data(), p->ptr_v.data(), p->ind_v.data(), o, c2, m2,
-                            ng, row_floats, allow_hub, alt);
+                            ng, row_floats, allow_hub, alt, 0, ng16);
             if (alt.invalid) continue;
             const double c = small_graph_cost(alt);
             if (c < best) {
@@ -214,7 +226,7 @@
           }
         }
         const int32_t lanes = row_floats / (vec4 ? 4 : 1);
-        if (p->opts.fused_tile_auto && vec4 && F % 4 == 0 && (lanes == 8 || lanes == 16) && p->nnz <= 16384 && p->N <= 4096 &&
+        if (!wide && p->opts.fused_tile_auto && vec4 && F % 4 == 0 && (lanes == 8 || lanes == 16) && p->nnz <= 16384 && p->N <= 4096 &&
             wide_rows_ok(p, F)) {
           for (int32_t tile : {16384, 32768, 65536}) {
             int32_t c2, m2;
@@ -245,6 +257,11 @@
       hg::set_error("fused schedule: host allocation failed");
       return HG_ERR_NOMEM;
     }
+    if (wide && (int64_t)f.panels.size() <= hg::kWideMinPanels) {
+      p->wide_off[wkey] = true;
+      lock.unlock();
+      return get_fused(cp, F, vec4, out, lin, lane16);
+    }
     for (const hg::FPanel &pn : f.panels) {
       if (pn.nrows <= 0 || pn.nrows > f.rows_cap || pn.nslots > f.cap || pn.npm > f.mem_cap ||
           pn.nvs > f.vslot_cap || pn.r0 < 0 || (size_t)(pn.r0 + pn.nrows) > f.prow.size()) {
@@ -267,7 +284,7 @@
     }
     it = p->fused.emplace(key, std::move(f)).first;
   }
-  p->fused_by_width[((int64_t)F * 2 + (vec4 ? 1 : 0)) * 2 + (lin ? 1 : 0)] = &it->second;
+  p->fused_by_width[(((int64_t)F * 2 + (vec4 ? 1 : 0)) * 2 + (lin ? 1 : 0)) * 2 + (lane16 ? 1 : 0)] = &it->second;
   *out = &it->second;
   return HG_OK;
 }
@@ -302,7 +319,7 @@
   if (pull_only) return need;
   std::lock_guard<std::mutex> lock(p->fused_mu);
   for (const auto &kv : p->fused_by_width)
-    if (kv.first / 4 == F) need = std::max(need, fused_carve(*kv.second, F).total);
+    if (kv.first / 8 == F) need = std::max(need, fused_carve(*kv.second, F).total);
   return need;
 }
 
@@ -461,7 +478,7 @@
     if (it != mp->hop_kernel.end()) kind = hop == 0 ? it->second % 3 : (it->second / 3) % 3;
   }
   if (kind == 0 && lanes16 && F < (1 << 22) && nsrc < (1 << 24) && sb > 0 && sb < ((int64_t)1 << 31) && !(p->opts.flags & HG_PLAN_NO_ROW_STREAM)) {
-    const int32_t ng = 256 / (hg::fused_tile_row_floats(F, true) / 4);
+    const int32_t ng = hg::fused_lane_groups(F, true, false);
     const hg::RowStream *rs = nullptr;
     int rc = get_row_stream(p, hop, ng, &rs);
     if (rc != HG_OK) return rc;
@@ -738,7 +755,7 @@
   hg::FusedSched *f = const_cast<hg::FusedSched *>(cf);
   std::lock_guard<std::mutex> lock(const_cast<hg_plan *>(cp)->fused_mu);
   for (const auto &kv : cp->fused_by_width)
-    if (kv.first / 4 == F && (kv.first & 1) && kv.second != cf) {
+    if (kv.first / 8 == F && kv.second != cf) {
       hg::FusedSched *fl = const_cast<hg::FusedSched *>(kv.second);
       fl->bound_degE = fl->bound_W = fl->bound_degV = nullptr;
       fl->bound_W_is_one = false;
@@ -789,7 +806,7 @@
   int rc = get_fused(p, F, plan_vec4(p, F), &f);
   if (rc != HG_OK) return rc;
   if (!(p->opts.flags & (HG_PLAN_HOST_ONLY | HG_PLAN_NO_ROW_STREAM)) && (F % 4 == 0 || F > 8)) {
-    const int32_t ng = 256 / (hg::fused_tile_row_floats(F, true) / 4);
+    const int32_t ng = hg::fused_lane_groups(F, true, false);
     for (int hop = 0; hop < 2; hop++) {
       const int64_t nsrc = hop == 0 ? p->N : p->M;
       if (nsrc >= (1 << 24) || nsrc * F * 4 >= ((int64_t)1 << 31)) continue;
@@ -818,14 +835,14 @@
     info->record_words_max = f->max_rec_words;
     info->stream_steps_max = f->max_steps;
     info->lds_bytes = (int32_t)((size_t)f->cap * hg::fused_tile_row_floats(F, plan_vec4(p, F)) * 4 + (size_t)f->max_rec_words * 4 + 16);
-    info->reserved = 0;
+    info->lane_groups = f->ng;
   }
   return HG_OK;
 }
 
 __attribute__((visibility("default"))) int hg_debug_fused_shape(const hg_plan *p, int32_t F, int32_t lin, int64_t *out9) {
   const hg::FusedSched *f = nullptr;
-  int rc = get_fused(p, F, plan_vec4(p, F), &f, lin != 0);
+  int rc = get_fused(p, F, plan_vec4(p, F), &f, lin != 0, lin != 0);
   if (rc != HG_OK) return rc;
   int64_t rows = 0, padded = 0, slots = 0;
   for (const auto &pn : f->panels) {
@@ -836,6 +853,24 @@
   const int64_t v[9] = {(int64_t)f->panels.size(), rows, padded, f->pmem_entries, slots, f->cap, f->rows_cap, f->n_mat,
                         f->stream_entries / std::max(1, f->ng) * 100000 + f->max_rec_words};
   for (int i = 0; i < 9; i++) out9[i] = v[i];
+  return HG_OK;
+}
+
+__attribute__((visibility("default"))) int hg_debug_fused_records(const hg_plan *p, int32_t F, int64_t *sizes4, int32_t *rec,
+                                                                  int64_t *rec_off, int32_t *slot_base, int32_t *eid) {
+  const hg::FusedSched *f = nullptr;
+  int rc = get_fused(p, F, plan_vec4(p, F), &f);
+  if (rc != HG_OK) return rc;
+  sizes4[0] = (int64_t)f->rec.size();
+  sizes4[1] = (int64_t)f->rec_tab.size();
+  sizes4[2] = (int64_t)f->eid_all.size();
+  sizes4[3] = f->ng;
+  if (rec) std::copy(f->rec.begin(), f->rec.end(), rec);
+  if (eid) std::copy(f->eid_all.begin(), f->eid_all.end(), eid);
+  for (size_t i = 0; i < f->rec_tab.size(); i++) {
+    if (rec_off) rec_off[i] = f->rec_tab[i].off;
+    if (slot_base) slot_base[i] = f->rec_tab[i].slot_base;
+  }
   return HG_OK;
 }
 
@@ -978,21 +1013,32 @@
   }
   if (variant == HG_VARIANT_FUSED) {
     if (!f && (rc = get_fused(plan, F, vec4, &f)) != HG_OK) return rc;
+    auto follow_binding = [&](const hg::FusedSched *fl) -> int {
+      const bool dflt_bound = (degE || degV || W) && f->bound_degE == degE && f->bound_W == W && f->bound_degV == degV;
+      if (dflt_bound && !(fl->bound_degE == degE && fl->bound_W == W && fl->bound_degV == degV)) {
+        hg::FusedSched *m = const_cast<hg::FusedSched *>(fl);
+        std::lock_guard<std::mutex> lock(const_cast<hg_plan *>(plan)->fused_mu);
+        int brc = gather_bound_scales(m, degE, degV, W, s);
+        if (brc != HG_OK) return brc;
+        (void)hipStreamSynchronize(s);
+        m->bound_degE = degE;
+        m->bound_W = W;
+        m->bound_degV = degV;
+        m->bound_W_is_one = f->bound_W_is_one;
+      }
+      return HG_OK;
+    };
+    if ((bf16 || lin) && f->ng != hg::fused_lane_groups(F, vec4, false) && f->ng == hg::fused_lane_groups(F, vec4, true)) {
+      const hg::FusedSched *fn = nullptr;
+      if ((rc = get_fused(plan, F, vec4, &fn, false, true)) != HG_OK) return rc;
+      if (fn != f && (rc = follow_binding(fn)) != HG_OK) return rc;
+      f = fn;
+    }
     if (lin && aligned && f->fixups.empty()) {
       const hg::FusedSched *fl = nullptr;
-      if ((rc = get_fused(plan, F, vec4, &fl, true)) != HG_OK) return rc;
+      if ((rc = get_fused(plan, F, vec4, &fl, true, true)) != HG_OK) return rc;
       if (fl != f && fl->fixups.empty()) {
-        const bool dflt_bound = (degE || degV || W) && f->bound_degE == degE && f->bound_W == W && f->bound_degV == degV;
-        if (dflt_bound && !(fl->bound_degE == degE && fl->bound_W == W && fl->bound_degV == degV)) {
-          hg::FusedSched *m = const_cast<hg::FusedSched *>(fl);
-          std::lock_guard<std::mutex> lock(const_cast<hg_plan *>(plan)->fused_mu);
-          if ((rc = gather_bound_scales(m, degE, degV, W, s)) != HG_OK) return rc;
-          (void)hipStreamSynchronize(s);
-          m->bound_degE = degE;
-          m->bound_W = W;
-          m->bound_degV = degV;
-          m->bound_W_is_one = f->bound_W_is_one;
-        }
+        if ((rc = follow_binding(fl)) != HG_OK) return rc;
         f = fl;
       }
     }
diff --git a/hypergef_amd/csrc/hg_fused.cpp b/hypergef_amd/csrc/hg_fused.cpp
--- a/hypergef_amd/csrc/hg_fused.cpp
+++ b/hypergef_amd/csrc/hg_fused.cpp
@@ -98,7 +98,8 @@
 void build_fused(int32_t N, int32_t M, const int32_t *ptr_t, const int32_t *ind_t,
                  const int32_t *ptr_v, const int32_t *ind_v, const Opts &o, int32_t cap,
                  int32_t mem_cap, int32_t ng, int32_t row_floats, bool allow_hub, FusedSched &f,
-                 int32_t rows_cap) {
+                 int32_t rows_cap, int32_t ng_lane16) {
+  if (ng_lane16 <= 0) ng_lane16 = ng;
   f = FusedSched();
   f.cap = cap;
   f.rows_cap = rows_cap > 0 ? std::min(rows_cap, cap) : cap;
@@ -122,7 +123,7 @@
       f.mat_ptr.push_back((int32_t)f.mat_ind.size());
     }
   build_sched(f.n_mat, f.mat_ptr.data(), o, f.mat_sched);
-  if (allow_hub) build_row_stream(f.n_mat, f.mat_ptr.data(), f.mat_ind.data(), f.mat_eid.data(), ng, N, f.mat_stream);
+  if (allow_hub) build_row_stream(f.n_mat, f.mat_ptr.data(), f.mat_ind.data(), f.mat_eid.data(), ng_lane16, N, f.mat_stream);
 
   std::vector<uint8_t> big((size_t)N, 0);
   std::vector<int32_t> cand;
@@ -143,7 +144,7 @@
   }
   std::vector<int32_t> hub_of((size_t)N, -1), parts;
   HubPass &hp = f.hub;
-  hub_geometry(ng, row_floats, o.hub_tile_bytes, hp);
+  hub_geometry(ng_lane16, row_floats, o.hub_tile_bytes, hp);
   const int32_t kHubMinDeg = o.hub_min_deg;
   allow_hub = allow_hub && hub_rec_bound(hp, f.t_big, f.t_big, 1, hp.ng * hp.R) <= kHubRecWords;
   if (allow_hub && !(o.flags & HG_PLAN_NO_HUB_PASS) && nnz >= o.hub_min_nnz && !cand.empty()) {
diff --git a/hypergef_amd/csrc/hg_internal.h b/hypergef_amd/csrc/hg_internal.h
--- a/hypergef_amd/csrc/hg_internal.h
+++ b/hypergef_amd/csrc/hg_internal.h
@@ -170,7 +170,7 @@
 void build_fused(int32_t N, int32_t M, const int32_t *ptr_t, const int32_t *ind_t,
                  const int32_t *ptr_v, const int32_t *ind_v, const Opts &o, int32_t cap,
                  int32_t mem_cap, int32_t ng, int32_t row_floats, bool allow_hub, FusedSched &f,
-                 int32_t rows_cap = 0);
+                 int32_t rows_cap = 0, int32_t ng_lane16 = 0);
 void build_row_stream(int32_t nrows, const int32_t *ptr, const int32_t *ind, const int32_t *scale_index,
                       int32_t ng, int32_t idle, RowStream &rs);
 void add_fixups(int32_t row, int32_t first, int32_t count, int32_t &nslots, std::vector<Fixup> &level1,
@@ -190,6 +190,7 @@
   bool has_lat = false;
   std::map<int64_t, hg::FusedSched> fused;
   std::map<int64_t, const hg::FusedSched *> fused_by_width;
+  std::map<int64_t, bool> wide_off;
   std::mutex fused_mu;
   std::map<int64_t, hg::RowStream> row_streams;
   std::mutex stream_mu;
diff --git a/hypergef_amd/csrc/hg_kernels.h b/hypergef_amd/csrc/hg_kernels.h
--- a/hypergef_amd/csrc/hg_kernels.h
+++ b/hypergef_amd/csrc/hg_kernels.h
@@ -141,6 +141,10 @@
 hipError_t launch_linear_pack(int32_t F_out, int32_t F_in, const float *Wlin, float *wfrag, hipStream_t stream);
 hipError_t launch_linear_pack_split(int32_t F_out, int32_t F_in, const float *Wlin, void *wsplit, hipStream_t stream);
 int fused_tile_row_floats(int F, bool vec4);
+int fused_lanes_per_row(int F, bool vec4, bool wide);
+inline int fused_lane_groups(int F, bool vec4, bool wide) { return 256 / fused_lanes_per_row(F, vec4, wide); }
+bool fused_wide_width(int F);
+constexpr int kWideMinPanels = 512;
 hipError_t launch_push(const PushArgs &a, hipStream_t stream);
 hipError_t launch_bind_scales(int64_t nslots, const int32_t *eid_all, const float *degE, const float *W,
                               float *bsA, float *bsB, int64_t nrows, const int32_t *prow, const float *degV,
diff --git a/hypergef_amd/csrc/hg_kernels.hip b/hypergef_amd/csrc/hg_kernels.hip
--- a/hypergef_amd/csrc/hg_kernels.hip
+++ b/hypergef_amd/csrc/hg_kernels.hip
@@ -78,8 +78,35 @@
   }
 };
 
-template <typename T, int VEC> struct Rows {
-  using V = Vec<VEC>;
+template <int HS> struct Vec8 {
+  Vec<4> lo, hi;
+  __device__ __forceinline__ static Vec8 zero() { return Vec8{Vec<4>::zero(), Vec<4>::zero()}; }
+  __device__ __forceinline__ static Vec8 load(const float *p) { return Vec8{Vec<4>::load(p), Vec<4>::load(p + HS)}; }
+  __device__ __forceinline__ static Vec8 load_buf(__amdgpu_buffer_rsrc_t r, unsigned off) {
+    return Vec8{Vec<4>::load_buf(r, off), Vec<4>::load_buf(r, off + HS * 4u)};
+  }
+  __device__ __forceinline__ void store(float *p) const { lo.store(p); hi.store(p + HS); }
+  __device__ __forceinline__ void store_n(float *p, int) const { lo.storeu(p); hi.storeu(p + HS); }
+  __device__ __forceinline__ void store_n_nt(float *p, int) const { lo.store_n_nt(p, 4); hi.store_n_nt(p + HS, 4); }
+  __device__ __forceinline__ void add(const Vec8 &o) { lo.add(o.lo); hi.add(o.hi); }
+  __device__ __forceinline__ void mul(float s) { lo.mul(s); hi.mul(s); }
+};
+#ifndef HG_WIDE_SPLIT
+#define HG_WIDE_SPLIT 1
+#endif
+#ifndef HG_WIDE_U
+#define HG_WIDE_U 4
+#endif
+#ifndef HG_WIDE_WIDTHS
+#define HG_WIDE_WIDTHS 32
+#endif
+constexpr bool kWideSplit = HG_WIDE_SPLIT != 0;
+constexpr int kWideU = HG_WIDE_U;
+template <int VEC, int LPR> struct LaneVec { using type = Vec<VEC>; };
+template <int LPR> struct LaneVec<8, LPR> { using type = Vec8<kWideSplit ? LPR * 4 : 4>; };
+
+template <typename T, int VEC, typename VT = Vec<VEC>> struct Rows {
+  using V = VT;
   __device__ __forceinline__ static V load(const float *p) { return V::load(p); }
   __device__ __forceinline__ static V load_buf(__amdgpu_buffer_rsrc_t r, unsigned off) { return V::load_buf(r, off); }
   __device__ __forceinline__ static void store(const V &v, float *p) { v.store(p); }
@@ -1040,15 +1067,16 @@
   static_assert(!SPLIT || (LIN && !LINW && LPR == 32 && VEC == 4), "bf16x6 matrix phase: K = 128 staged instances");
   static_assert(!LIN || std::is_same_v<T, float>, "the linear epilogue takes fp32 rows");
   constexpr bool XF32 = std::is_same_v<T, float>;
+  static_assert(VEC != 8 || (FAST && !LIN && BS == 256 && XF32), "32-byte lanes: the plain fp32 panel instances");
   constexpr int NG = BS / LPR;
   constexpr int TW = LPR * VEC;
-  using V = Vec<VEC>;
-  using RX = Rows<T, VEC>;
+  using V = typename LaneVec<VEC, LPR>::type;
+  using RX = Rows<T, VEC, V>;
   extern __shared__ int32_t smem[];
   const int64_t F = a.F;
   const int tid = threadIdx.x;
   const int gl = tid & (LPR - 1);
-  const int lcol = gl * VEC;
+  const int lcol = gl * (VEC == 8 && kWideSplit ? 4 : VEC);
   const int col = blockIdx.y * TW + lcol;
   const bool col_ok = col < a.F;
   int b = blockIdx.x;
@@ -1192,7 +1220,7 @@
       }
     };
     const int steps_x = MAT ? rec[8] : steps;
-    if constexpr (MAT && FAST && ((LIN && !LINW && LPR >= 32) || (!LIN && VEC == 4 && BS == 256))) {
+    if constexpr (MAT && FAST && ((LIN && !LINW && LPR >= 32) || (!LIN && VEC >= 4 && BS == 256))) {
       auto mixed = [&](const int s0, auto full) {
         constexpr bool FULL = decltype(full)::value;
         int ent[U];
@@ -1840,7 +1868,7 @@
 
 bool stream_rows_ok(const StreamArgs &a, bool vec4) {
   return vec4 && a.nrec > 0 && a.src_bytes > 0 && a.nrows_src < (1 << 24) && a.F < (1 << 22) &&
-         a.ng == 256 / (fused_tile_row_floats(a.F, true) / 4) &&
+         a.ng == fused_lane_groups(a.F, true, false) &&
          (size_t)a.max_rec_words * 4 + (size_t)2 * a.cap * 4 <= kLdsMax;
 }
 
@@ -2106,9 +2134,42 @@
 
 int fused_tile_row_floats(int F, bool vec4);
 
+template <int LPR>
+static hipError_t launch_fused_wide_t(const FusedArgs &a, hipStream_t stream) {
+  if (a.npanels == 0) return hipSuccess;
+  constexpr int TW = LPR * 8;
+  const bool fast = a.x_bytes > 0 && a.nrows_x < (1 << 24) && (!a.Xe_mat || (a.mat_bytes > 0 && a.nrows_mat < (1 << 24)));
+  if (!fast || a.Wlin || a.F != TW || a.ng != 256 / LPR) return hipErrorInvalidValue;
+  FusedArgs ad = a;
+  const dim3 grid(a.npanels, 1);
+  ad.dv_regs = fused_dv_regs(a, 256 / LPR, (size_t)a.cap * TW * 4 + (size_t)a.max_rec_words * 4 + 16, 8);
+  const size_t lds_p = (size_t)a.cap * TW * 4 + (size_t)a.max_rec_words * 4 + fused_scale_floats(ad) * 4 + 16;
+#define HG_PK(M, S) return launch_lds<fused_packed_kernel<LPR, 8, kWideU, true, M, S>>(grid, lds_p, stream, ad)
+  switch ((a.Xe_mat ? 1 : 0) | ((a.degE || a.W) ? 2 : 0)) {
+    case 0: HG_PK(false, false);
+    case 1: HG_PK(true, false);
+    case 2: HG_PK(false, true);
+    default: HG_PK(true, true);
+  }
+#undef HG_PK
+}
+
 hipError_t launch_fused(const FusedArgs &a, bool vec4, hipStream_t stream, bool xy_bf16) {
   const int lpr = fused_tile_row_floats(a.F, vec4) / (vec4 ? 4 : 1);
   if (xy_bf16 && (!vec4 || a.Wlin || (a.F & 3))) return hipErrorInvalidValue;
+  if (vec4 && fused_wide_width(a.F) && a.ng == fused_lane_groups(a.F, vec4, true)) {
+    if (xy_bf16) return hipErrorInvalidValue;
+    switch (a.F) {
+      case 32: return launch_fused_wide_t<4>(a, stream);
+#if HG_WIDE_WIDTHS & 64
+      case 64: return launch_fused_wide_t<8>(a, stream);
+#endif
+#if HG_WIDE_WIDTHS & 128
+      case 128: return launch_fused_wide_t<16>(a, stream);
+#endif
+    }
+    return hipErrorInvalidValue;
+  }
 #define HG_CASE(L)                                              \
   case L:                                                       \
     if (xy_bf16) return launch_fused_t<L, 4, bf16>(a, stream);   \
@@ -2130,6 +2191,12 @@
   const int lanes = vec4 ? (F + 3) / 4 : F;
   return std::min(64, next_pow2(std::max(lanes, 1))) * (vec4 ? 4 : 1);
 }
+
+int fused_lanes_per_row(int F, bool vec4, bool wide) {
+  const int lanes = fused_tile_row_floats(F, vec4) / (vec4 ? 4 : 1);
+  return wide && vec4 && fused_wide_width(F) ? lanes / 2 : lanes;
+}
+bool fused_wide_width(int F) { return (F == 32 || F == 64 || F == 128) && (HG_WIDE_WIDTHS & F) != 0; }
 
 hipError_t launch_push(const PushArgs &a, hipStream_t stream) {
   const int lpr = std::min(64, next_pow2(std::max(a.F, 1)));
diff --git a/include/hg_aggr.h b/include/hg_aggr.h
--- a/include/hg_aggr.h
+++ b/include/hg_aggr.h
@@ -81,7 +81,7 @@
   int32_t record_words_max;
   int32_t stream_steps_max;
   int32_t lds_bytes;
-  int32_t reserved;
+  int32_t lane_groups;
 } hg_fused_info;
 
 HG_API int hg_version(void);
```

Result: slower. 27.44 billion edges/s (-16.5%).
